# pkuyzy/TLC-GNN

Hardware: AMD Instinct MI355X
Metric: persistence-images/sec + LP-forward edges/sec, PubMed-scale, 1/2/4/8 GPU (higher is better)
Workload: dtype f64

## Files before the change

include/tlcgnn.h:

```cpp
#ifndef TLCGNN_H
#define TLCGNN_H

#include <stdint.h>

#ifdef __cplusplus
extern "C" {
#endif

#define TLC_OK                 0
#define TLC_ERR_INVALID_ARG    1
#define TLC_ERR_HIP            2
#define TLC_ERR_NO_DEVICE      3
#define TLC_ERR_UNSUPPORTED    4
#define TLC_ERR_OUT_OF_MEMORY  5

#define TLC_ST_OK              0
#define TLC_ST_MISSING_NODE    1
#define TLC_ST_DISCONNECTED    2
#define TLC_ST_ZERO_RANGE      3
#define TLC_ST_NO_TREE_EDGE    4
#define TLC_ST_TOO_LARGE       5
#define TLC_ST_NOT_CONVERGED   6
#define TLC_ST_BAD_INPUT       7

#define TLC_KEEP_ZERO_PERS   0x01u
#define TLC_INCLUDE_ROOTS    0x02u
#define TLC_NORM_EPS         0x04u
#define TLC_PI_ORD0_EXT1     0x08u
#define TLC_NO_EXT1          0x10u
#define TLC_UNREACHABLE_100  0x20u
#define TLC_DESC_MIN         0x40u
#define TLC_DESC_MAX         0x80u
#define TLC_DESC_ROOT1       0xC0u
#define TLC_DESC_MASK        0xC0u
#define TLC_NO_NORM          0x100u

typedef struct tlc_graph tlc_graph;

const char* tlc_version(void);
const char* tlc_last_error(void);
int  tlc_device_count(void);

int tlc_graph_create(int32_t n_nodes, const int32_t* h_rowptr, const int32_t* h_col, const double* h_w,
                     int device, tlc_graph** out);
int tlc_graph_destroy(tlc_graph* g);

int tlc_pd_pi_batch(tlc_graph* g, const int32_t* d_pairs, int64_t n_pairs, int hop, uint32_t flags,
                    int res, double* d_out_pi, uint8_t* d_out_status, void* stream);

int tlc_vicinity_filtration(tlc_graph* g, const int32_t* d_pairs, int64_t n_pairs, int hop, uint32_t flags,
                            const int64_t* d_node_offs, int32_t* d_out_ids, double* d_out_f,
                            int32_t* d_out_n, uint8_t* d_out_status,
                            const int64_t* d_edge_offs, int32_t* d_out_edges, int32_t* d_out_m, void* stream);

int tlc_pd_pi_batch_async(tlc_graph* g, const int32_t* d_pairs, int64_t n_pairs, int hop, uint32_t flags,
                          int res, double* d_out_pi, uint8_t* d_out_status, void* stream);
int tlc_pd_pi_batch_join(tlc_graph* g, void* stream);

int tlc_pd_pi_batch_stats(tlc_graph* g, int64_t* h_out, void* stream);

int tlc_pd_pi_batch_set_timing(tlc_graph* g, int enable);
int tlc_pd_pi_batch_timings(tlc_graph* g, double* h_ms, void* stream);
int tlc_pd_pi_batch_timing_history(tlc_graph* g, int slot, double* h_ms, int32_t cap, int32_t* n_out, void* stream);
int tlc_pd_pi_batch_sizes(tlc_graph* g, int32_t* h_n, int32_t* h_m2, int64_t cap, void* stream);
int tlc_pd_pi_algorithmic_bytes(int32_t n_nodes, const int32_t* h_rowptr, const int32_t* h_col, const int32_t* h_pairs,
                                int64_t n_pairs, int hop, int res, double* h_out_bytes);

int tlc_debug_set_option(tlc_graph* g, const char* name, int value);
int tlc_debug_dc_stats(tlc_graph* g, long long* h_out, void* stream);
int tlc_debug_chunk_counters(tlc_graph* g, long long* h_out, int32_t n, void* stream);
int tlc_debug_tier_counts(tlc_graph* g, long long* h_out, void* stream);
int tlc_debug_phase_profile(tlc_graph* g, int enable, unsigned long long* h_out, int64_t cap_u64, int32_t* n_rows);
int tlc_debug_pair_times(tlc_graph* g, unsigned long long* h_out, int64_t n_pairs);

int tlc_pd_from_filtration(int32_t n_graphs, const int64_t* d_node_offs, const int64_t* d_edge_offs,
                           const int32_t* d_edges, const double* d_f, uint32_t flags,
                           double* d_pd_up, double* d_pd_down, double* d_pd_one, double* d_ext0,
                           int32_t* d_counts, int32_t* d_edge_rank, void* stream);

int tlc_pi_raster(int32_t n_dgms, const int64_t* d_offs, const double* d_pts, int res, double* d_out,
                  void* stream);
int tlc_pi_raster_wgrad(int32_t n_dgms, int64_t n_pts, const int64_t* d_offs, const double* d_pts, int res,
                        const double* d_grad_img, double* d_grad_pts, void* stream);


int tlc_gcn_norm_csr(int32_t n_nodes, int64_t n_edges, const int64_t* d_edge_index,
                     int32_t* d_rowptr, int32_t* d_col, float* d_val, int32_t* d_nnz, void* stream);

int tlc_gemm_f32(int32_t M, int32_t N, int32_t K, const float* d_A, const float* d_B, const float* d_bias,
                 int relu, float* d_C, void* stream);

int tlc_spgemm_csr_dense_f32(int32_t M, int32_t K, int32_t N, const int32_t* d_rowptr, const int32_t* d_col, const float* d_val,
                             const float* d_B, const float* d_bias, int relu, float* d_C, void* stream);

int tlc_spmm_csr_f32(int32_t n_rows, const int32_t* d_rowptr, const int32_t* d_col, const float* d_val,
                     const float* d_X, int32_t k, const float* d_bias, int relu, float* d_Y, void* stream);

int tlc_renorm_rows_f32(int32_t n_rows, int32_t k, float* d_emb, void* stream);

int tlc_gcn2_encode_f32(int32_t n_nodes, const int32_t* d_rowptr, const int32_t* d_col, const float* d_val,
                        const float* d_x, int32_t f_in, const float* d_w1, const float* d_b1, int32_t hidden,
                        const float* d_w2, const float* d_b2, int32_t out_dim, int flags, float* d_ws, float* d_emb, void* stream);

int tlc_gcn2_encode_csr_f32(int32_t n_nodes, const int32_t* d_rowptr, const int32_t* d_col, const float* d_val,
                            const int32_t* d_xs_rowptr, const int32_t* d_xs_col, const float* d_xs_val, int32_t f_in,
                            const float* d_w1, const float* d_b1, int32_t hidden, const float* d_w2, const float* d_b2,
                            int32_t out_dim, int flags, float* d_ws, float* d_emb, void* stream);

int tlc_lp_decode_fused(int64_t n_pairs, const int32_t* d_pairs, const float* d_emb, int32_t emb_dim,
                        const double* d_pi, int32_t pi_dim, const float* d_W1, const float* d_b1,
                        const float* d_W2, const float* d_b2, float* d_prob, void* stream);
int tlc_lp_decode_fused_f32(int64_t n_pairs, const int32_t* d_pairs, const float* d_emb, int32_t emb_dim,
                            const float* d_pi, int32_t pi_dim, const float* d_W1, const float* d_b1,
                            const float* d_W2, const float* d_b2, float* d_prob, void* stream);


int tlc_gcn_norm_csr_t(int32_t n_nodes, int64_t n_edges, const int64_t* d_edge_index, const int32_t* d_rowptr,
                       int32_t* d_rowptr_t, int32_t* d_col_t, float* d_val_t, int32_t* d_nnz, void* stream);

int tlc_gemm_tn_f32(int32_t M, int32_t N, int64_t K, const float* d_A, const float* d_B, float* d_C, float* d_work, void* stream);

int tlc_lp_decode_bwd_f32(int64_t n_pairs, const int32_t* d_pairs, const float* d_emb_pre, const float* d_emb, int32_t n_nodes,
                          int32_t emb_dim, const float* d_pi, int32_t pi_dim, const float* d_W1, const float* d_b1,
                          const float* d_W2, const float* d_b2, const float* d_gprob, const int32_t* d_node_ptr,
                          const int32_t* d_node_slots, float* d_gemb, float* d_gw, float* d_work, void* stream);


int64_t tlc_nc_group_work_ints(int32_t n_nodes, int64_t n_edges);

int tlc_nc_group(int32_t n_nodes, int64_t n_edges, const int64_t* d_edge_index, int32_t* d_groups, int32_t* d_work, int32_t* d_bad,
                 void* stream);

int tlc_nc_linear_f32(int32_t M, int32_t N, int32_t K, const float* d_x, const float* d_w, const float* d_b, float* d_y, void* stream);

int tlc_nc_linear_bwd_f32(int32_t M, int32_t N, int32_t K, const float* d_x, const float* d_w, const float* d_gy, float* d_gx,
                          float* d_gw, float* d_gb, float* d_work, void* stream);

int64_t tlc_nc_curv_work_bytes(int32_t n_nodes, int64_t n_edges, int32_t C, int32_t D);

int tlc_nc_curv_fwd_f32(int32_t n_nodes, int64_t n_edges, int32_t C, int32_t D, const int32_t* d_groups, const float* d_xl,
                        const float* d_wmul, const float* d_w1, const float* d_prelu, const float* d_w2, const float* d_b2, float* d_alpha,
                        float* d_out, void* stream);

int tlc_nc_curv_bwd_f32(int32_t n_nodes, int64_t n_edges, int32_t C, int32_t D, const int32_t* d_groups, const float* d_xl,
                        const float* d_wmul, const float* d_w1, const float* d_prelu, const float* d_w2, const float* d_alpha,
                        const float* d_gout, float* d_gxl, float* d_gw1, float* d_gprelu, float* d_gw2, float* d_gb2, void* d_work,
                        int64_t work_bytes, void* stream);

#define TLC_SCORE_F32          0
#define TLC_SCORE_F64          1
#define TLC_LABEL_U8           0
#define TLC_LABEL_I64          1
#define TLC_LABEL_F32          2
#define TLC_RANK_FORCE_RADIX   0x1u
// ... 101 lines not shown
```

tlc-gnn_amd/_lib.py:

```python
import ctypes as C
import os
import subprocess

HERE = os.path.dirname(os.path.abspath(__file__))
LIB_PATH = os.path.join(HERE, "libtlcgnn_hip.so")
CSRC = os.path.join(HERE, "csrc")

OK = 0
ERRORS = {1: "TLC_ERR_INVALID_ARG", 2: "TLC_ERR_HIP", 3: "TLC_ERR_NO_DEVICE", 4: "TLC_ERR_UNSUPPORTED",
          5: "TLC_ERR_OUT_OF_MEMORY"}

ST_OK, ST_MISSING_NODE, ST_DISCONNECTED, ST_ZERO_RANGE, ST_NO_TREE_EDGE, ST_TOO_LARGE = range(6)
ST_NOT_CONVERGED, ST_BAD_INPUT = 6, 7
HKS_NMAX, HKS_LDS_NMAX, HKS_TMAX, HKS_NORMALISE = 256, 96, 8, 0x1
KEEP_ZERO_PERS, INCLUDE_ROOTS, NORM_EPS, PI_ORD0_EXT1, NO_EXT1, UNREACHABLE_100 = 0x1, 0x2, 0x4, 0x8, 0x10, 0x20
DESC_MIN, DESC_MAX, DESC_ROOT1, NO_NORM = 0x40, 0x80, 0xC0, 0x100
DESCRIPTOR_FLAG = {"sum": 0, "min": DESC_MIN, "max": DESC_MAX}

SYMBOLS = [
    "tlc_version", "tlc_last_error", "tlc_device_count", "tlc_graph_create", "tlc_graph_destroy",
    "tlc_pd_pi_batch", "tlc_pd_pi_batch_async", "tlc_pd_pi_batch_join", "tlc_vicinity_filtration", "tlc_pd_pi_batch_stats", "tlc_pd_pi_batch_set_timing",
    "tlc_pd_pi_batch_timings", "tlc_pd_pi_batch_timing_history", "tlc_pd_pi_batch_sizes", "tlc_pd_pi_algorithmic_bytes", "tlc_pd_from_filtration",
    "tlc_pi_raster", "tlc_pi_raster_wgrad", "tlc_gcn_norm_csr", "tlc_gcn_norm_csr_t", "tlc_gemm_f32", "tlc_gemm_tn_f32", "tlc_lp_decode_bwd_f32", "tlc_binary_rank_metrics", "tlc_binary_rank_metrics_work_bytes",
    "tlc_nc_group_work_ints", "tlc_nc_group", "tlc_nc_linear_f32", "tlc_nc_linear_bwd_f32", "tlc_nc_curv_work_bytes", "tlc_nc_curv_fwd_f32",
    "tlc_nc_curv_bwd_f32", "tlc_spgemm_csr_dense_f32", "tlc_spmm_csr_f32", "tlc_renorm_rows_f32", "tlc_gcn2_encode_f32", "tlc_gcn2_encode_csr_f32",
    "tlc_lp_decode_fused", "tlc_lp_decode_fused_f32", "tlc_gat_layer_fwd", "tlc_gat_layer_tiled_fwd", "tlc_gat_tile_cut", "tlc_csr_by_target", "tlc_pdgnn_forward", "tlc_pdgnn_forward_work_bytes", "tlc_scatter_f32", "tlc_edge_head_fwd",
    "tlc_complement_rows", "tlc_complement_pairs", "tlc_select_rows", "tlc_pack_vicinities", "tlc_stack_batch", "tlc_ollivier_ricci_sinkhorn",
    "tlc_near_pairs", "tlc_w2_partial_matching", "tlc_w2_inference_matching", "tlc_gat_layer_bwd", "tlc_edge_head_bwd", "tlc_pack_offsets", "tlc_vicinity_sizes", "tlc_debug_dc_stats", "tlc_debug_tier_counts", "tlc_debug_chunk_counters", "tlc_debug_phase_profile", "tlc_debug_set_option", "tlc_debug_pair_times",
    "tlc_hks_batch", "tlc_hks_batch_work_bytes",
]


class TlcError(RuntimeError):
    pass


def build(verbose=False, force=False):
    if force:
        subprocess.run(["make", "-C", CSRC, "clean"], stdout=subprocess.PIPE, stderr=subprocess.STDOUT, text=True)
    cmd = ["make", "-C", CSRC, "-j", str(min(8, os.cpu_count() or 1))]
    res = subprocess.run(cmd, stdout=subprocess.PIPE, stderr=subprocess.STDOUT, text=True)
    if verbose or res.returncode != 0:
        print(res.stdout)
    if res.returncode != 0:
        raise TlcError("building libtlcgnn_hip.so failed")
    return LIB_PATH


_lib = None


def lib():
    global _lib
    if _lib is None:
        if not os.path.exists(LIB_PATH):
            raise TlcError("libtlcgnn_hip.so is missing: run `python -c 'import __graft_entry__ as g; g.build()'` "
                           "(there is no CPU fallback for the product path)")
        try:
            import torch
        except ImportError:
            pass
        L = C.CDLL(LIB_PATH)
        L.tlc_version.restype = C.c_char_p
        L.tlc_last_error.restype = C.c_char_p
        L.tlc_graph_create.argtypes = [C.c_int32, C.c_void_p, C.c_void_p, C.c_void_p, C.c_int, C.POINTER(C.c_void_p)]
        L.tlc_graph_destroy.argtypes = [C.c_void_p]
        L.tlc_pd_pi_batch.argtypes = [C.c_void_p, C.c_void_p, C.c_int64, C.c_int, C.c_uint32, C.c_int, C.c_void_p,
                                      C.c_void_p, C.c_void_p]
        L.tlc_pd_pi_batch_async.argtypes = L.tlc_pd_pi_batch.argtypes
        L.tlc_pd_pi_batch_join.argtypes = [C.c_void_p, C.c_void_p]
        L.tlc_vicinity_filtration.argtypes = [C.c_void_p, C.c_void_p, C.c_int64, C.c_int, C.c_uint32, C.c_void_p,
                                              C.c_void_p, C.c_void_p, C.c_void_p, C.c_void_p, C.c_void_p, C.c_void_p,
                                              C.c_void_p, C.c_void_p]
        L.tlc_pd_pi_batch_stats.argtypes = [C.c_void_p, C.c_void_p, C.c_void_p]
        L.tlc_pd_pi_batch_set_timing.argtypes = [C.c_void_p, C.c_int]
        L.tlc_pd_pi_batch_timings.argtypes = [C.c_void_p, C.c_void_p, C.c_void_p]
        L.tlc_pd_pi_batch_timing_history.argtypes = [C.c_void_p, C.c_int, C.c_void_p, C.c_int32, C.c_void_p, C.c_void_p]
        L.tlc_pd_pi_batch_sizes.argtypes = [C.c_void_p, C.c_void_p, C.c_void_p, C.c_int64, C.c_void_p]
        L.tlc_pd_pi_algorithmic_bytes.argtypes = [C.c_int32, C.c_void_p, C.c_void_p, C.c_void_p, C.c_int64, C.c_int, C.c_int, C.c_void_p]
        L.tlc_pd_from_filtration.argtypes = [C.c_int32] + [C.c_void_p] * 4 + [C.c_uint32] + [C.c_void_p] * 7
        L.tlc_pi_raster.argtypes = [C.c_int32, C.c_void_p, C.c_void_p, C.c_int, C.c_void_p, C.c_void_p]
        L.tlc_pi_raster_wgrad.argtypes = [C.c_int32, C.c_int64, C.c_void_p, C.c_void_p, C.c_int, C.c_void_p, C.c_void_p, C.c_void_p]
        if hasattr(L, "tlc_gcn_norm_csr"):
            L.tlc_gcn_norm_csr.argtypes = [C.c_int32, C.c_int64] + [C.c_void_p] * 6
            L.tlc_gemm_f32.argtypes = [C.c_int32, C.c_int32, C.c_int32, C.c_void_p, C.c_void_p, C.c_void_p, C.c_int,
                                       C.c_void_p, C.c_void_p]
            L.tlc_spgemm_csr_dense_f32.argtypes = [C.c_int32, C.c_int32, C.c_int32] + [C.c_void_p] * 5 + [C.c_int, C.c_void_p, C.c_void_p]
            L.tlc_spmm_csr_f32.argtypes = [C.c_int32] + [C.c_void_p] * 4 + [C.c_int32, C.c_void_p, C.c_int, C.c_void_p,
                                                                            C.c_void_p]
            L.tlc_renorm_rows_f32.argtypes = [C.c_int32, C.c_int32, C.c_void_p, C.c_void_p]
            L.tlc_gcn2_encode_f32.argtypes = ([C.c_int32] + [C.c_void_p] * 4 + [C.c_int32, C.c_void_p, C.c_void_p, C.c_int32, C.c_void_p,
                                              C.c_void_p, C.c_int32, C.c_int, C.c_void_p, C.c_void_p, C.c_void_p])
            L.tlc_gcn2_encode_csr_f32.argtypes = ([C.c_int32] + [C.c_void_p] * 6 + [C.c_int32, C.c_void_p, C.c_void_p, C.c_int32, C.c_void_p,
                                                  C.c_void_p, C.c_int32, C.c_int, C.c_void_p, C.c_void_p, C.c_void_p])
            L.tlc_lp_decode_fused.argtypes = [C.c_int64, C.c_void_p, C.c_void_p, C.c_int32, C.c_void_p, C.c_int32,
                                              C.c_void_p, C.c_void_p, C.c_void_p, C.c_void_p, C.c_void_p, C.c_void_p]
            L.tlc_lp_decode_fused_f32.argtypes = L.tlc_lp_decode_fused.argtypes
        if hasattr(L, "tlc_gemm_tn_f32"):
            L.tlc_gcn_norm_csr_t.argtypes = [C.c_int32, C.c_int64] + [C.c_void_p] * 7
            L.tlc_gemm_tn_f32.argtypes = [C.c_int32, C.c_int32, C.c_int64] + [C.c_void_p] * 5
            L.tlc_lp_decode_bwd_f32.argtypes = ([C.c_int64, C.c_void_p, C.c_void_p, C.c_void_p, C.c_int32, C.c_int32, C.c_void_p, C.c_int32]
                                                + [C.c_void_p] * 10)
        if hasattr(L, "tlc_binary_rank_metrics"):
            L.tlc_binary_rank_metrics_work_bytes.argtypes = [C.c_void_p, C.c_int32, C.c_int, C.c_uint32]
            L.tlc_binary_rank_metrics_work_bytes.restype = C.c_int64
            L.tlc_binary_rank_metrics.argtypes = ([C.c_void_p, C.c_int, C.c_void_p, C.c_int, C.c_void_p, C.c_int32, C.c_uint32]
                                                  + [C.c_void_p] * 6 + [C.c_int64, C.c_void_p])
        if hasattr(L, "tlc_nc_group"):
            L.tlc_nc_group_work_ints.argtypes = [C.c_int32, C.c_int64]
            L.tlc_nc_group_work_ints.restype = C.c_int64
            L.tlc_nc_group.argtypes = [C.c_int32, C.c_int64] + [C.c_void_p] * 5
            L.tlc_nc_linear_f32.argtypes = [C.c_int32] * 3 + [C.c_void_p] * 5
            L.tlc_nc_linear_bwd_f32.argtypes = [C.c_int32] * 3 + [C.c_void_p] * 8
            L.tlc_nc_curv_work_bytes.argtypes = [C.c_int32, C.c_int64, C.c_int32, C.c_int32]
            L.tlc_nc_curv_work_bytes.restype = C.c_int64
            L.tlc_nc_curv_fwd_f32.argtypes = [C.c_int32, C.c_int64, C.c_int32, C.c_int32] + [C.c_void_p] * 10
            L.tlc_nc_curv_bwd_f32.argtypes = [C.c_int32, C.c_int64, C.c_int32, C.c_int32] + [C.c_void_p] * 14 + [C.c_int64, C.c_void_p]
        if hasattr(L, "tlc_gat_layer_fwd"):
            L.tlc_gat_layer_fwd.argtypes = [C.c_int32, C.c_void_p, C.c_void_p, C.c_void_p, C.c_int32, C.c_int32,
                                            C.c_void_p, C.c_void_p, C.c_void_p, C.c_void_p, C.c_float, C.c_void_p,
                                            C.c_void_p, C.c_void_p]
            L.tlc_csr_by_target.argtypes = [C.c_int32, C.c_int64] + [C.c_void_p] * 6
            L.tlc_pdgnn_forward_work_bytes.argtypes = [C.c_int32, C.c_int64, C.c_int32]
            L.tlc_pdgnn_forward_work_bytes.restype = C.c_int64
            L.tlc_pdgnn_forward.argtypes = [C.c_int32, C.c_int64, C.c_void_p, C.c_void_p, C.c_int32, C.c_void_p, C.c_int64, C.c_void_p, C.c_int32,
                                            C.c_void_p, C.c_void_p, C.c_void_p, C.c_int32, C.c_void_p, C.c_int64, C.c_void_p, C.c_void_p, C.c_void_p]
            L.tlc_gat_tile_cut.argtypes = [C.c_int32, C.c_void_p, C.c_void_p, C.c_int32, C.c_void_p, C.c_void_p, C.POINTER(C.c_int32), C.c_void_p]
            L.tlc_gat_layer_tiled_fwd.argtypes = [C.c_int32, C.c_void_p, C.c_void_p, C.c_int32, C.c_void_p, C.c_void_p, C.c_int32, C.c_int32,
                                                  C.c_void_p, C.c_void_p, C.c_void_p, C.c_void_p, C.c_float, C.c_void_p,
                                                  C.c_void_p, C.c_void_p]
            L.tlc_scatter_f32.argtypes = [C.c_int64, C.c_void_p, C.c_void_p, C.c_int32, C.c_int, C.c_int32, C.c_void_p,
                                          C.c_void_p, C.c_void_p]
            L.tlc_edge_head_fwd.argtypes = [C.c_int64, C.c_void_p, C.c_void_p, C.c_void_p, C.c_int32, C.c_void_p,
                                            C.c_void_p, C.c_int32, C.c_float, C.c_void_p, C.c_void_p, C.c_void_p,
                                            C.c_int32, C.c_void_p, C.c_void_p]
        L.tlc_complement_rows.argtypes = [C.c_int32, C.c_void_p, C.c_void_p, C.c_void_p, C.c_void_p]
        L.tlc_complement_pairs.argtypes = [C.c_int32, C.c_void_p, C.c_void_p, C.c_void_p, C.c_void_p, C.c_int64, C.c_int64,
                                           C.c_void_p, C.c_void_p]
        L.tlc_select_rows.argtypes = [C.c_int64, C.c_int32, C.c_void_p, C.c_void_p, C.c_int64, C.c_int64, C.c_uint32, C.c_void_p,
                                      C.c_void_p, C.c_void_p, C.c_void_p, C.c_void_p, C.c_void_p]
        L.tlc_pack_vicinities.argtypes = [C.c_int64] + [C.c_void_p] * 14
        L.tlc_pack_offsets.argtypes = [C.c_int64] + [C.c_void_p] * 6
        L.tlc_stack_batch.argtypes = [C.c_int64] + [C.c_void_p] * 4 + [C.c_int64, C.c_int64] + [C.c_void_p] * 3
        L.tlc_vicinity_sizes.argtypes = [C.c_void_p, C.c_void_p, C.c_int64, C.c_int, C.c_uint32, C.c_void_p, C.c_void_p, C.c_void_p]
        L.tlc_ollivier_ricci_sinkhorn.argtypes = [C.c_int32, C.c_void_p, C.c_void_p, C.c_int64, C.c_void_p, C.c_double, C.c_double,
                                                  C.c_int32, C.c_double, C.c_void_p, C.c_void_p, C.c_void_p, C.c_int64, C.c_int32,
                                                  C.c_int64, C.c_void_p]
        L.tlc_near_pairs.argtypes = [C.c_int32, C.c_void_p, C.c_void_p, C.c_void_p, C.c_int, C.c_int64, C.c_void_p, C.c_void_p,
                                     C.c_void_p, C.c_void_p]
        L.tlc_w2_partial_matching.argtypes = [C.c_int32, C.c_void_p, C.c_void_p, C.c_void_p, C.c_void_p, C.c_int, C.c_int32] + [C.c_void_p] * 7
        L.tlc_w2_inference_matching.argtypes = [C.c_int32, C.c_void_p, C.c_void_p, C.c_void_p, C.c_void_p, C.c_int, C.c_int32] + [C.c_void_p] * 9
        L.tlc_gat_layer_bwd.argtypes = [C.c_int32, C.c_void_p, C.c_void_p, C.c_void_p, C.c_int32, C.c_int32, C.c_void_p, C.c_void_p,
                                        C.c_void_p, C.c_float] + [C.c_void_p] * 9
        L.tlc_edge_head_bwd.argtypes = [C.c_int64, C.c_void_p, C.c_void_p, C.c_void_p, C.c_int32, C.c_void_p, C.c_void_p, C.c_int32,
                                        C.c_float] + [C.c_void_p] * 9
        L.tlc_hks_batch_work_bytes.argtypes = [C.c_int64, C.c_int64, C.c_int64, C.c_int32, C.POINTER(C.c_int64)]
        L.tlc_hks_batch.argtypes = ([C.c_void_p] * 3 + [C.c_int64] * 3 + [C.POINTER(C.c_double), C.c_int32, C.c_uint32, C.c_void_p, C.c_void_p,
                                    C.c_void_p, C.c_int64, C.c_void_p])
        L.tlc_debug_set_option.argtypes = [C.c_void_p, C.c_char_p, C.c_int]
        L.tlc_debug_dc_stats.argtypes = [C.c_void_p, C.c_void_p, C.c_void_p]
        L.tlc_debug_tier_counts.argtypes = [C.c_void_p, C.c_void_p, C.c_void_p]
        L.tlc_debug_chunk_counters.argtypes = [C.c_void_p, C.c_void_p, C.c_int32, C.c_void_p]
        L.tlc_debug_phase_profile.argtypes = [C.c_void_p, C.c_int, C.c_void_p, C.c_int64, C.c_void_p]
        _lib = L
    return _lib


def check(rc, what=""):
    if rc != OK:
        msg = lib().tlc_last_error().decode("utf-8", "replace")
        raise TlcError("%s: %s (%s)" % (what or "libtlcgnn_hip", ERRORS.get(rc, rc), msg))


def require_gpu():
    import torch
    if not torch.cuda.is_available():
        raise TlcError("no MI355X/HIP device visible: the TLC-GNN hot path has no CPU fallback")
    return torch


def stream_ptr(device=None):
    import torch
    return C.c_void_p(torch.cuda.current_stream(device).cuda_stream)


def on_device_of(fn):
    import functools

    @functools.wraps(fn)
    def wrapped(*args, **kwargs):
        import torch
        for a in list(args) + list(kwargs.values()):
            if isinstance(a, torch.Tensor) and a.is_cuda:
                if a.device.index != torch.cuda.current_device():
                    with torch.cuda.device(a.device):
                        return fn(*args, **kwargs)
                break
        return fn(*args, **kwargs)
    return wrapped


def ptr(t):
    if t is None:
        return None
    assert t.is_contiguous()
    return C.c_void_p(t.data_ptr())
```

tlc-gnn_amd/csrc/api.hip:

```cpp
#include <stdarg.h>
#include <stdlib.h>

#include <algorithm>
#include <new>
#include <vector>

#include "tlc_common.h"
#include <atomic>
#include <chrono>
#include "tlc_kernels.h"

static thread_local char g_err[512] = "";
void tlc_set_error(const char* fmt, ...) {
    va_list ap;
    va_start(ap, fmt);
    vsnprintf(g_err, sizeof(g_err), fmt, ap);
    va_end(ap);
}
extern "C" const char* tlc_last_error(void) { return g_err; }
extern "C" const char* tlc_version(void) { return "tlcgnn-hip 0.1.0 (gfx950)"; }
extern "C" int tlc_device_count(void) {
    int n = 0;
    if (hipGetDeviceCount(&n) != hipSuccess) return 0;
    return n;
}

#define TLC_CHUNK_PAIRS (1 << 20)
#define TLC_N_SIDE 8
#define TLC_EARLY_CAND 512
#define TLC_EARLY_SLOTS 256
#define TLC_EARLY_WG 256
#ifndef TLC_EARLY_MIN_PAIRS
#define TLC_EARLY_MIN_PAIRS 4096
#endif
#define TLC_TIMING_RING 64
#define TLC_X_REGION 4096

#define TLC_CTL_INTS (64 + TLC_SCAN_MAX_BLOCKS + 8 + 8 * 64)
struct HostSync {
    long long total_entries;
    int tier_count[TLC_N_TIERS];
    int pad[2];
    unsigned long long stats[2];
    volatile long long pub_total;
    volatile int pub_tier[TLC_N_TIERS];
    volatile int pub_tiny[TLC_TINY_BINS];
    volatile int pub_dcm;
    volatile int pub_early;
    volatile int pub_overflow;
    volatile unsigned pub_seq;
};

#define TLC_POISON 7.25

#define TLC_N_WS 4

struct ChunkCtx {
    TlcVicParams vp;
    TlcPdParams pp;
    hipStream_t s;
    int n_pairs, hop, pi_enabled;
    bool bump, use_x, early, spec, count_only, tiny_bins, pipelined;
    bool mh_front;
    bool plain, fsplit;
    int xfgrid;
    long long bump_base;
    int xgrid, vgrid, tmask;
    unsigned seq;
    size_t spec_base[TLC_N_TIERS];
    int spec_cap[TLC_N_TIERS];
    bool used[TLC_N_SIDE];
    hipEvent_t* ev_t;
    unsigned char* ev_used;
    std::chrono::steady_clock::time_point ht0;
    double ht_front;
    unsigned long long call_seq;
};

struct Workspace {
    size_t cap_pairs;
    int *hdr_n, *hdr_m2, *hdr_lu, *hdr_lv, *tier_list;
    int* dc_lists;
    int* tiny_bins;
    int* big_lists;
    hipEvent_t ev_cls;
    int prev_dcm;
    long long* edge_off;
    int* d_ctl;
    long long* d_block_sums;
    long long* d_totals;
    unsigned long long* d_stats;
    HostSync* h_sync;
    HostSync* h_sync_dev;
    unsigned pub_seq;
    size_t cap_entries;
    unsigned* A_dir;
    double* A_lw;
    size_t cap_small;
    unsigned* S_dir;
    double* S_lw;
    int vic_hop_cap;
    int* vic_scratch;
    long long vic_stride;
    int huge_slots;
    unsigned char* huge_scratch;
    size_t huge_stride;
    int* d_cand_list;
    int* d_early_list;
    unsigned* E_dir;
    double* E_lw;
    unsigned char* handoff;
    size_t cap_handoff;
    unsigned char* handoff_large;
    size_t cap_handoff_large;
    hipStream_t main;
    hipStream_t side[TLC_N_SIDE];
    hipEvent_t ev_in, ev_done;
    hipEvent_t ev_fork, ev_join[TLC_N_SIDE], ev_early, ev_scan;
    int prev_tc[TLC_N_TIERS];
    size_t x_entries_hint;
    int busy;
    int in_call;
    int n_pairs;
    ChunkCtx ctx;
    int own_early;
    int back_pending;
};

struct tlc_graph {
    int device;
    int n_nodes;
    long long nnz;
    int nw;
    int *d_rowptr, *d_col;
    double* d_w;
    Workspace ws[TLC_N_WS];
    unsigned long long next_ws;
    Workspace* last_ws;
    unsigned long long call_seq;
    Workspace* pending;
    int vic_slots;
    size_t vic_lds;
    int lds_attr_set;
    int ball_hop;
    int* d_ball_ub[2];
    long long last_stats[10];
    long long last_tc[TLC_N_TIERS];
    long long acc_tie, acc_entries;
    unsigned long long* d_phase;
    unsigned long long* d_pair_t;
    size_t cap_pair_t;
    int timing;
    hipEvent_t ev_ring[TLC_TIMING_RING][16];
    unsigned char ev_ring_used[TLC_TIMING_RING][8];
    int ev_ring_ready;
    unsigned long long ring_pos;
    hipEvent_t* ev_t;
    unsigned char* ev_used;
    int last_n_pairs;
    int ball_list_hop;
    int* d_bptr;
    int* d_bcol;
    unsigned* d_bbits;
    int* d_be_ptr;
    unsigned* d_be_pos;
    double* d_be_w;
    long long be_entries;
    long long ball_entries;
    TlcNodeRec* d_nrec;
    double* d_hh_w;
    int hh_k;
    int hh_diag;
    size_t x_lds64, x_lds512, x_lds64f, x_lds64fb;
    int opt_extract, opt_heavy, opt_tiny;
    int opt_fast_split;
    int opt_dc_inplace;
    int opt_ball_edges;
    int opt_ball_bits;
    int opt_dc_force_fail;
    int opt_plain_kernels;
    int count_only;
    int opt_n_ws;
    int opt_spec_cap;
    int opt_timing_every;
    unsigned timing_seq;
    int opt_tier_mask;
    int opt_x_region, opt_x_bump_min;
    int opt_mh_front_pos;
    int opt_main_beside_early;
    int opt_poison;
    long long last_n_hi;
    long long cnt_n_hi, cnt_pipelined, cnt_early, cnt_beyond_spec, cnt_poisoned, cnt_poison_bytes;
    long long cnt_deferred;
    long long max_busy;
    long long poison_region[3];
};

static int finish_pending(tlc_graph* g);
static int quiesce(tlc_graph* g) {
    { const int rp = finish_pending(g); if (rp != TLC_OK) return rp; }
    for (int k = 0; k < TLC_N_WS; ++k)
        if (g->ws[k].busy) { TLC_HIP_CHECK(hipEventSynchronize(g->ws[k].ev_done)); g->ws[k].busy = 0; }
    return TLC_OK;
}

static int ensure_pairs(tlc_graph* g, Workspace* ws, size_t n) {
    if (n <= ws->cap_pairs) return TLC_OK;
    hipFree(ws->hdr_n); hipFree(ws->hdr_m2); hipFree(ws->hdr_lu); hipFree(ws->hdr_lv); hipFree(ws->tier_list); hipFree(ws->edge_off);
    hipFree(ws->dc_lists); hipFree(ws->big_lists); hipFree(ws->tiny_bins);
    ws->hdr_n = ws->hdr_m2 = ws->hdr_lu = ws->hdr_lv = ws->tier_list = ws->dc_lists = ws->big_lists = ws->tiny_bins = nullptr;
    ws->edge_off = nullptr;
    ws->cap_pairs = 0;
    TLC_HIP_CHECK(hipMalloc(&ws->hdr_n, n * sizeof(int)));
    TLC_HIP_CHECK(hipMalloc(&ws->hdr_m2, n * sizeof(int)));
    TLC_HIP_CHECK(hipMalloc(&ws->hdr_lu, n * sizeof(int)));
    TLC_HIP_CHECK(hipMalloc(&ws->hdr_lv, n * sizeof(int)));
    TLC_HIP_CHECK(hipMalloc(&ws->tier_list, n * TLC_N_TIERS * sizeof(int)));
    TLC_HIP_CHECK(hipMalloc(&ws->edge_off, (n + 1) * sizeof(long long)));
    TLC_HIP_CHECK(hipMalloc(&ws->dc_lists, 3 * (n + TLC_EARLY_SLOTS) * sizeof(int)));
    TLC_HIP_CHECK(hipMalloc(&ws->big_lists, 4 * n * sizeof(int)));
    TLC_HIP_CHECK(hipMalloc(&ws->tiny_bins, (size_t)TLC_TINY_BINS * n * sizeof(int)));
    ws->cap_pairs = n;
    return TLC_OK;
}

static int ensure_arena(tlc_graph* g, Workspace* ws, size_t entries, size_t keep = 0, hipStream_t s = nullptr) {
    if (entries <= ws->cap_entries) return TLC_OK;
    size_t want = std::max(entries + entries / 4, (size_t)1 << 16);
    unsigned* old_dir = ws->A_dir;
    double* old_lw = ws->A_lw;
    ws->A_dir = nullptr; ws->A_lw = nullptr; ws->cap_entries = 0;
    if (keep == 0) { hipFree(old_dir); hipFree(old_lw); old_dir = nullptr; old_lw = nullptr; }
    TLC_HIP_CHECK(hipMalloc(&ws->A_dir, want * sizeof(unsigned)));
    TLC_HIP_CHECK(hipMalloc(&ws->A_lw, want * sizeof(double)));
    if (keep > 0) {
        TLC_HIP_CHECK(hipMemcpyAsync(ws->A_dir, old_dir, keep * sizeof(unsigned), hipMemcpyDeviceToDevice, s));
        TLC_HIP_CHECK(hipMemcpyAsync(ws->A_lw, old_lw, keep * sizeof(double), hipMemcpyDeviceToDevice, s));
        TLC_HIP_CHECK(hipDeviceSynchronize());
        hipFree(old_dir); hipFree(old_lw);
    }
    ws->cap_entries = want;
    return TLC_OK;
}


static int ensure_handoff(tlc_graph* g, Workspace* ws, size_t bytes) {
    if (bytes <= ws->cap_handoff) return TLC_OK;
    const size_t want = std::max(bytes + bytes / 4, (size_t)1 << 20);
    hipFree(ws->handoff);
    ws->handoff = nullptr; ws->cap_handoff = 0;
    TLC_HIP_CHECK(hipMalloc(&ws->handoff, want));
    ws->cap_handoff = want;
    return TLC_OK;
}

static int ensure_handoff_large(tlc_graph* g, Workspace* ws, size_t slots) {
    if (slots * tlc_handoff_slot_bytes(TLC_TIER_LARGE) <= ws->cap_handoff_large) return TLC_OK;
    const size_t bytes = (slots + slots / 4) * tlc_handoff_slot_bytes(TLC_TIER_LARGE);
    hipFree(ws->handoff_large);
    ws->handoff_large = nullptr; ws->cap_handoff_large = 0;
    TLC_HIP_CHECK(hipMalloc(&ws->handoff_large, bytes));
    ws->cap_handoff_large = bytes;
    return TLC_OK;
}

static int ensure_small(tlc_graph* g, Workspace* ws, size_t n_pairs) {
    if (n_pairs <= ws->cap_small) return TLC_OK;
    hipFree(ws->S_dir); hipFree(ws->S_lw);
    ws->S_dir = nullptr; ws->S_lw = nullptr; ws->cap_small = 0;
    TLC_HIP_CHECK(hipMalloc(&ws->S_dir, n_pairs * (2 * TLC_S_MMAX) * sizeof(unsigned)));
    TLC_HIP_CHECK(hipMalloc(&ws->S_lw, n_pairs * (2 * TLC_S_MMAX) * sizeof(double)));
    ws->cap_small = n_pairs;
// ... 141 lines not shown
    TLC_HIP_CHECK(hipMemcpyAsync(g->d_bptr, sz.data(), ((size_t)n + 1) * sizeof(int), hipMemcpyHostToDevice, s));
    if ((rc = tlc_launch_ball_list(true, n, g->nw, g->d_rowptr, g->d_col, hop, nullptr, g->d_bptr, g->d_bcol, grid, s)) != TLC_OK) return rc;
    TLC_HIP_CHECK(hipStreamSynchronize(s));
    g->ball_list_hop = hop; g->ball_entries = tot;
    {
        int* d_es = nullptr;
        int* d_bp = nullptr;
        unsigned* d_pos = nullptr;
        double* d_bw = nullptr;
        std::vector<int> es((size_t)n + 1, 0);
        bool ok = hipMalloc(&d_es, (size_t)n * sizeof(int)) == hipSuccess;
        ok = ok && tlc_launch_ball_edges(false, n, g->nw, g->d_rowptr, g->d_col, g->d_w, g->d_bptr, g->d_bcol, d_es, nullptr, nullptr, nullptr, grid, s) == TLC_OK;
        ok = ok && hipMemcpyAsync(es.data(), d_es, (size_t)n * sizeof(int), hipMemcpyDeviceToHost, s) == hipSuccess;
        ok = ok && hipStreamSynchronize(s) == hipSuccess;
        long long et = 0;
        if (ok) for (int x = 0; x < n; ++x) { const int c = es[x]; es[x] = (int)et; et += c; if (et > 0x7fffffffll) { ok = false; break; } }
        if (ok) {
            es[n] = (int)et;
            size_t fb = 0, tb = 0;
            ok = hipMemGetInfo(&fb, &tb) == hipSuccess && (size_t)et * 12 <= fb / 8;
        }
        ok = ok && hipMalloc(&d_bp, ((size_t)n + 1) * sizeof(int)) == hipSuccess;
        ok = ok && hipMalloc(&d_pos, ((size_t)et + 64) * sizeof(unsigned)) == hipSuccess;
        ok = ok && hipMalloc(&d_bw, ((size_t)et + 64) * sizeof(double)) == hipSuccess;
        ok = ok && hipMemcpyAsync(d_bp, es.data(), ((size_t)n + 1) * sizeof(int), hipMemcpyHostToDevice, s) == hipSuccess;
        ok = ok && tlc_launch_ball_edges(true, n, g->nw, g->d_rowptr, g->d_col, g->d_w, g->d_bptr, g->d_bcol, nullptr, d_bp, d_pos, d_bw, grid, s) == TLC_OK;
        ok = ok && hipStreamSynchronize(s) == hipSuccess;
        hipFree(d_es);
        if (ok) { g->d_be_ptr = d_bp; g->d_be_pos = d_pos; g->d_be_w = d_bw; g->be_entries = et; }
        else { hipFree(d_bp); hipFree(d_pos); hipFree(d_bw); (void)hipGetLastError(); }
    }
    if (g->d_be_ptr) {
        const size_t bytes = (size_t)n * (size_t)g->nw * sizeof(unsigned);
        size_t fb = 0, tb = 0;
        unsigned* d_bb = nullptr;
        bool ok = bytes <= ((size_t)1 << 30) && hipMemGetInfo(&fb, &tb) == hipSuccess && bytes <= fb / 8;
        ok = ok && hipMalloc(&d_bb, bytes) == hipSuccess;
        ok = ok && hipMemsetAsync(d_bb, 0, bytes, s) == hipSuccess;
        ok = ok && tlc_launch_ball_bits(n, g->nw, g->d_bptr, g->d_bcol, d_bb, s) == TLC_OK;
        ok = ok && hipStreamSynchronize(s) == hipSuccess;
        if (ok) g->d_bbits = d_bb;
        else { hipFree(d_bb); (void)hipGetLastError(); }
    }
    return TLC_OK;
}

extern "C" int tlc_graph_create(int32_t n_nodes, const int32_t* h_rowptr, const int32_t* h_col, const double* h_w,
                                int device, tlc_graph** out) {
    TLC_REQUIRE(out != nullptr, "out is null");
    *out = nullptr;
    TLC_REQUIRE(n_nodes > 0 && h_rowptr && h_col && h_w, "null graph arrays or n_nodes <= 0");
    int ndev = 0;
    if (hipGetDeviceCount(&ndev) != hipSuccess || ndev == 0) {
        tlc_set_error("no HIP device visible");
        return TLC_ERR_NO_DEVICE;
    }
    TLC_REQUIRE(device >= 0 && device < ndev, "device index out of range");
    const long long nnz = h_rowptr[n_nodes];
    TLC_REQUIRE(h_rowptr[0] == 0 && nnz >= 0, "rowptr must start at 0");
    for (int i = 0; i < n_nodes; ++i) TLC_REQUIRE(h_rowptr[i + 1] >= h_rowptr[i], "rowptr not monotone");
    for (long long j = 0; j < nnz; ++j) {
        TLC_REQUIRE(h_col[j] >= 0 && h_col[j] < n_nodes, "column index out of range");
        TLC_REQUIRE(h_w[j] > 0.0, "edge weights (kappa+1) must be > 0");
    }
    const int nw = (n_nodes + 31) / 32;
    const size_t lds = ((size_t)5 * ((nw + 3) & ~3) / 2 + 4 + 16) * 4;
    if (lds > 160 * 1024) {
        tlc_set_error("graph has %d nodes: the vicinity bitmaps (%zu B) exceed the 160 KiB LDS of a CU", n_nodes, lds);
        return TLC_ERR_UNSUPPORTED;
    }
    TLC_ON_DEVICE(device);
    tlc_graph* g = new (std::nothrow) tlc_graph();
    if (!g) return TLC_ERR_OUT_OF_MEMORY;
    memset(g, 0, sizeof(*g));
    g->device = device; g->n_nodes = n_nodes; g->nnz = nnz; g->nw = nw; g->vic_lds = lds;
    auto env_on = [](const char* name) { const char* v = getenv(name); return !(v && v[0] == '0'); };
    g->opt_extract = env_on("TLC_EXTRACT"); g->opt_heavy = env_on("TLC_HEAVY"); g->opt_tiny = env_on("TLC_TINY");
    g->opt_ball_edges = env_on("TLC_BALL_EDGES"); g->opt_dc_inplace = env_on("TLC_DC_INPLACE") ? 1 : 0;
    g->opt_fast_split = env_on("TLC_FAST_SPLIT") ? 1 : 0;
    g->opt_ball_bits = env_on("TLC_BALL_BITS") ? 1 : 0;
    g->opt_plain_kernels = env_on("TLC_PLAIN_KERNELS") ? 1 : 0;
    g->opt_n_ws = 3;
    g->opt_x_region = TLC_X_REGION; g->opt_x_bump_min = 1 << 20; g->opt_tier_mask = (1 << TLC_N_TIERS) - 1; g->opt_timing_every = 1;
    g->opt_mh_front_pos = 64; g->opt_main_beside_early = 1;
    int rc = TLC_OK;
    auto fail = [&](int code) { tlc_graph_destroy(g); return code; };
#define CK(e) do { if ((e) != hipSuccess) { tlc_set_error("%s failed: %s", #e, hipGetErrorString(hipGetLastError())); return fail(TLC_ERR_HIP); } } while (0)
    CK(hipMalloc(&g->d_rowptr, (size_t)(n_nodes + 1) * sizeof(int)));
    CK(hipMalloc(&g->d_col, ((size_t)nnz + 8) * sizeof(int)));
    CK(hipMalloc(&g->d_w, ((size_t)nnz + 8) * sizeof(double)));
    CK(hipMemset(g->d_col + nnz, 0, 8 * sizeof(int)));
    CK(hipMemset(g->d_w + nnz, 0, 8 * sizeof(double)));
    CK(hipMemcpy(g->d_rowptr, h_rowptr, (size_t)(n_nodes + 1) * sizeof(int), hipMemcpyHostToDevice));
    CK(hipMemcpy(g->d_col, h_col, (size_t)nnz * sizeof(int), hipMemcpyHostToDevice));
    CK(hipMemcpy(g->d_w, h_w, (size_t)nnz * sizeof(double), hipMemcpyHostToDevice));
    int prio_lo = 0, prio_hi = 0;
    hipDeviceGetStreamPriorityRange(&prio_lo, &prio_hi);
    const int prio_mid = (prio_lo + prio_hi) / 2;
    const bool eager_streams = getenv("TLC_LAZY_STREAMS") == nullptr;
    const int n_eager = 3;
    for (int i = 0; i < TLC_N_WS; ++i) {
        Workspace* ws = &g->ws[i];
        CK(hipMalloc(&ws->d_ctl, TLC_CTL_INTS * sizeof(int)));
        ws->d_stats = reinterpret_cast<unsigned long long*>(ws->d_ctl + 64 + TLC_SCAN_MAX_BLOCKS);
        CK(hipMalloc(&ws->d_block_sums, TLC_SCAN_MAX_BLOCKS * sizeof(long long)));
        CK(hipMalloc(&ws->d_totals, 2 * sizeof(long long)));
        CK(hipHostMalloc((void**)&ws->h_sync, sizeof(HostSync), hipHostMallocMapped | hipHostMallocCoherent));
        memset(ws->h_sync, 0, sizeof(HostSync));
        CK(hipHostGetDevicePointer((void**)&ws->h_sync_dev, ws->h_sync, 0));
        if (i == 0 || (eager_streams && i < n_eager)) CK(hipStreamCreateWithPriority(&ws->main, hipStreamNonBlocking, prio_mid));
        for (int k = 0; k < TLC_N_SIDE; ++k) {
            if (k == 4) {
                if (i == 0 || (eager_streams && i < n_eager)) { CK(hipStreamCreateWithPriority(&ws->side[k], hipStreamNonBlocking, prio_hi)); ws->own_early = 1; }
            }
            else if (i > 0) {
                ws->side[k] = g->ws[0].side[k];
                if (i == 2 && k == 7) ws->side[k] = g->ws[0].side[1];
            }
            else if (k == 2) ws->side[k] = nullptr;
            else {
                const int pr = k == 1 ? prio_hi : ((k == 6 || k == 7) ? prio_mid : prio_lo);
                CK(hipStreamCreateWithPriority(&ws->side[k], hipStreamNonBlocking, pr));
            }
            CK(hipEventCreateWithFlags(&ws->ev_join[k], hipEventDisableTiming));
        }
        if (i == 0) ws->side[2] = ws->side[6];
        CK(hipEventCreateWithFlags(&ws->ev_fork, hipEventDisableTiming));
        CK(hipEventCreateWithFlags(&ws->ev_early, hipEventDisableTiming));
        CK(hipEventCreateWithFlags(&ws->ev_scan, hipEventDisableTiming));
        CK(hipEventCreateWithFlags(&ws->ev_cls, hipEventDisableTiming));
        CK(hipEventCreateWithFlags(&ws->ev_in, hipEventDisableTiming));
        CK(hipEventCreateWithFlags(&ws->ev_done, hipEventDisableTiming));
    }
#undef CK
    hipDeviceProp_t prop;
    int cus = 256;
    if (hipGetDeviceProperties(&prop, device) == hipSuccess && prop.multiProcessorCount > 0) cus = prop.multiProcessorCount;
    int per_cu = (int)std::min<size_t>(28, (160 * 1024) / std::max<size_t>(lds + 64, 1));
    if (per_cu < 1) per_cu = 1;
    g->x_lds64 = tlc_extract_lds_bytes(nw, 64);
    g->x_lds512 = tlc_extract_lds_bytes(nw, 512);
    g->x_lds64f = tlc_extract_lds_bytes(nw, 64, true);
    g->x_lds64fb = tlc_extract_lds_bytes(0, 64, true);
    per_cu = std::max(per_cu, (int)std::min<size_t>(32, (160 * 1024) / std::max<size_t>(g->x_lds64 + 64, 1)));
    g->vic_slots = cus * per_cu;
    {
        std::vector<int> hidx;
        if ((rc = build_heavy_set(g, h_rowptr, h_col, h_w, &hidx)) != TLC_OK) return fail(rc);
        if ((rc = build_node_records(g, h_rowptr, h_col, h_w, hidx)) != TLC_OK) return fail(rc);
    }
    *out = g;
    return TLC_OK;
}

extern "C" int tlc_graph_destroy(tlc_graph* g) {
    if (!g) return TLC_OK;
    TlcDeviceScope scope(g->device);
    hipDeviceSynchronize();
    hipFree(g->d_rowptr); hipFree(g->d_col); hipFree(g->d_w);
    for (int i = 0; i < TLC_N_WS; ++i) {
        Workspace* ws = &g->ws[i];
        hipFree(ws->hdr_n); hipFree(ws->hdr_m2); hipFree(ws->hdr_lu); hipFree(ws->hdr_lv); hipFree(ws->tier_list); hipFree(ws->edge_off);
        hipFree(ws->dc_lists); hipFree(ws->big_lists); hipFree(ws->tiny_bins);
        hipFree(ws->d_ctl); hipFree(ws->d_block_sums); hipFree(ws->d_totals);
        if (ws->h_sync) hipHostFree(ws->h_sync);
        hipFree(ws->A_dir); hipFree(ws->A_lw); hipFree(ws->S_dir); hipFree(ws->S_lw); hipFree(ws->vic_scratch); hipFree(ws->huge_scratch);
        hipFree(ws->handoff); hipFree(ws->handoff_large);
        hipFree(ws->d_cand_list); hipFree(ws->d_early_list); hipFree(ws->E_dir); hipFree(ws->E_lw);
        if (ws->main) hipStreamDestroy(ws->main);
        for (int k = 0; k < TLC_N_SIDE; ++k) {
            const bool own = (k == 4 && ws->own_early) || (i == 0 && k != 2);
            if (own && ws->side[k]) hipStreamDestroy(ws->side[k]);
            if (ws->ev_join[k]) hipEventDestroy(ws->ev_join[k]);
        }
        for (hipEvent_t e : {ws->ev_fork, ws->ev_early, ws->ev_scan, ws->ev_in, ws->ev_done, ws->ev_cls}) if (e) hipEventDestroy(e);
    }
    hipFree(g->d_phase); hipFree(g->d_pair_t);
    hipFree(g->d_bptr); hipFree(g->d_bcol); hipFree(g->d_nrec); hipFree(g->d_hh_w);
    hipFree(g->d_be_ptr); hipFree(g->d_be_pos); hipFree(g->d_be_w); hipFree(g->d_bbits);
    hipFree(g->d_ball_ub[0]); hipFree(g->d_ball_ub[1]);
    if (g->ev_ring_ready)
        for (int r = 0; r < TLC_TIMING_RING; ++r)
            for (int k = 0; k < 16; ++k) if (g->ev_ring[r][k]) hipEventDestroy(g->ev_ring[r][k]);
    delete g;
    return TLC_OK;
}

__global__ void tlc_wait_started(const int* counter, int target, long long max_ticks) {
    if (threadIdx.x != 0) return;
    const long long t0 = wall_clock64();
    while (__hip_atomic_load(counter, __ATOMIC_RELAXED, __HIP_MEMORY_SCOPE_AGENT) < target && wall_clock64() - t0 < max_ticks)
        __builtin_amdgcn_s_sleep(8);
}

__global__ void tlc_wait_started_dev(const int* counter, const int* target, int cap, long long max_ticks) {
    if (threadIdx.x != 0) return;
    int tg = *target;
    tg = tg < cap ? tg : cap;
    const long long t0 = wall_clock64();
    while (__hip_atomic_load(counter, __ATOMIC_RELAXED, __HIP_MEMORY_SCOPE_AGENT) < tg && wall_clock64() - t0 < max_ticks)
        __builtin_amdgcn_s_sleep(8);
}

#define T0(k, st) do { if ((c.tmask >> (k)) & 1) { TLC_HIP_CHECK(hipEventRecord(c.ev_t[2 * (k)], st)); } } while (0)
#define T1(k, st) do { if ((c.tmask >> (k)) & 1) { TLC_HIP_CHECK(hipEventRecord(c.ev_t[2 * (k) + 1], st)); c.ev_used[k] = 1; } } while (0)
static inline void dc_lists_for(Workspace* ws, TlcPdParams& q, int k) {
    const size_t cap = ws->cap_pairs + TLC_EARLY_SLOTS;
    q.dc_count = ws->d_ctl + 26 + 2 * k;
    q.dc_list = ws->dc_lists + (size_t)k * cap;
}
static const int tslot[TLC_N_TIERS] = {3, 4, 5, 6, 7, 3, 4, 4};

static int front_prepare(tlc_graph* g, Workspace* ws, const int32_t* d_pairs, int n_pairs, int hop, uint32_t flags, int res,
                         double* d_out_pi, uint8_t* d_out_status, const int64_t* d_ids_off, int32_t* d_out_ids,
                         double* d_out_f, int32_t* d_out_n, const int64_t* d_edge_offs, int32_t* d_out_edges, int32_t* d_out_m,
                         int pi_enabled, hipStream_t s, bool pipelined) {
    int rc;
    ChunkCtx& c = ws->ctx;
    c.ht0 = std::chrono::steady_clock::now();
    c.s = s; c.n_pairs = n_pairs; c.hop = hop; c.pi_enabled = pi_enabled; c.call_seq = g->call_seq;
    if ((rc = ensure_pairs(g, ws, (size_t)n_pairs)) != TLC_OK) return rc;
    if ((rc = ensure_vic_scratch(g, ws, hop)) != TLC_OK) return rc;
    TLC_HIP_CHECK(hipMemsetAsync(ws->d_ctl, 0, TLC_CTL_INTS * sizeof(int), s));

    TlcVicParams& vp = c.vp;
    memset(&vp, 0, sizeof(vp));
    vp.n_nodes = g->n_nodes; vp.nw = g->nw; vp.rowptr = g->d_rowptr; vp.col = g->d_col; vp.w = g->d_w;
    vp.dbg = g->d_phase ? g->d_phase + 32 * TLC_TIER_HUGE : nullptr;
    if (g->d_phase) {
        if (g->cap_pair_t < (size_t)n_pairs) {
            hipFree(g->d_pair_t); g->d_pair_t = nullptr; g->cap_pair_t = 0;
            TLC_HIP_CHECK(hipMalloc(&g->d_pair_t, (size_t)n_pairs * 16 * sizeof(unsigned long long)));
            g->cap_pair_t = (size_t)n_pairs;
        }
        TLC_HIP_CHECK(hipMemsetAsync(g->d_pair_t, 0, (size_t)n_pairs * 16 * sizeof(unsigned long long), s));
        vp.dbg_pair_t = g->d_pair_t;
    }
    vp.pairs = d_pairs; vp.n_pairs = n_pairs; vp.hop = hop; vp.flags = flags; vp.res = res;
    vp.scratch = ws->vic_scratch; vp.scratch_stride = ws->vic_stride;
    vp.hdr_n = ws->hdr_n; vp.hdr_m2 = ws->hdr_m2; vp.hdr_lu = ws->hdr_lu; vp.hdr_lv = ws->hdr_lv;
    vp.out_pi = d_out_pi; vp.out_status = d_out_status; vp.out_n = d_out_n; vp.out_m = d_out_m;
    vp.edge_off = ws->edge_off; vp.A_dir = nullptr; vp.A_lw = nullptr;
    vp.ids_off = (const long long*)d_ids_off; vp.out_ids = d_out_ids;

    if (!g->lds_attr_set && g->vic_lds > 64 * 1024) {
        TLC_HIP_CHECK(hipFuncSetAttribute((const void*)tlc_vicinity_kernel<false, 64>, hipFuncAttributeMaxDynamicSharedMemorySize, (int)g->vic_lds));
        TLC_HIP_CHECK(hipFuncSetAttribute((const void*)tlc_vicinity_kernel<true, 64>, hipFuncAttributeMaxDynamicSharedMemorySize, (int)g->vic_lds));
        TLC_HIP_CHECK(hipFuncSetAttribute((const void*)tlc_vicinity_kernel<true, 512>, hipFuncAttributeMaxDynamicSharedMemorySize, (int)g->vic_lds));
        TLC_HIP_CHECK(hipFuncSetAttribute((const void*)tlc_vicinity_kernel<false, 512>, hipFuncAttributeMaxDynamicSharedMemorySize, (int)g->vic_lds));
        g->lds_attr_set = 1;
    }
    const int vgrid = std::min(n_pairs, g->vic_slots);
    const int tmask = (g->timing && (g->timing_seq++ % (unsigned)std::max(g->opt_timing_every, 1)) == 0) ? g->timing : 0;
    if (tmask) {
        if (!g->ev_ring_ready) {
            for (int r = 0; r < TLC_TIMING_RING; ++r)
                for (int k = 0; k < 16; ++k) TLC_HIP_CHECK(hipEventCreate(&g->ev_ring[r][k]));
            g->ev_ring_ready = 1;
        }
        const int set = (int)(g->ring_pos++ % TLC_TIMING_RING);
        g->ev_t = g->ev_ring[set];
        g->ev_used = g->ev_ring_used[set];
        memset(g->ev_used, 0, 8);
        c.ev_t = g->ev_t; c.ev_used = g->ev_used;
    }
    c.tmask = tmask; c.vgrid = vgrid;
    g->last_n_pairs = n_pairs;
    const bool plain = pi_enabled && !d_out_ids && !d_out_f && !d_out_edges;
    const bool bump = true;
    unsigned long long* d_bump_top = reinterpret_cast<unsigned long long*>(ws->d_ctl + 20);
    int* d_bump_overflow = ws->d_ctl + 22;
    bool use_x = g->opt_extract && g->x_lds512 <= (size_t)160 * 1024 && g->x_lds64 <= (size_t)160 * 1024 &&
                 (hop <= 2 || (size_t)g->nw * 12 + 16 <= (size_t)160 * 1024);
    if (use_x) {
        if ((rc = ensure_ball_lists(g, hop, s)) != TLC_OK) return rc;
        use_x = g->ball_list_hop == hop;
    }
    const bool early = pi_enabled && !d_out_ids && !d_out_f && !d_out_edges && (hop <= 2 || use_x) && n_pairs >= TLC_EARLY_MIN_PAIRS;
    const int xgrid = std::min(n_pairs, g->vic_slots);
    const bool fsplit = use_x && g->opt_fast_split && g->opt_ball_edges && g->d_be_ptr != nullptr && !(flags & TLC_INCLUDE_ROOTS);
    const int xfgrid = fsplit ? std::min(n_pairs, 8192) : 0;
    long long bump_base = 0;
    if (use_x) {
        const long long regions = (long long)xgrid + TLC_EARLY_WG + xfgrid;
        bump_base = regions * g->opt_x_region;
        const size_t want = (size_t)bump_base + std::max<size_t>(std::max<size_t>((size_t)n_pairs * 32, (size_t)g->opt_x_bump_min), ws->x_entries_hint + ws->x_entries_hint / 2);
        if (ws->cap_entries < want && (rc = ensure_arena(g, ws, want)) != TLC_OK) return rc;
        vp.small_dir = nullptr; vp.small_lw = nullptr;
        vp.bptr = g->d_bptr; vp.bcol = g->d_bcol;
        if (g->opt_ball_edges) { vp.be_ptr = g->d_be_ptr; vp.be_pos = g->d_be_pos; vp.be_w = g->d_be_w; }
        vp.nrec = g->d_nrec;
        if (g->hh_k > 0 && g->opt_heavy) { vp.hh_w = g->d_hh_w; vp.hh_k = g->hh_k; }
        vp.region_entries = g->opt_x_region; vp.bump_base = bump_base; vp.region_base_wg = 0;
    } else {
        if ((rc = ensure_small(g, ws, (size_t)n_pairs)) != TLC_OK) return rc;
        vp.small_dir = ws->S_dir; vp.small_lw = ws->S_lw;
    }
    if (bump) {
        if (ws->cap_entries == 0 &&
            (rc = ensure_arena(g, ws, std::min<size_t>((size_t)n_pairs * 128, (size_t)1 << 23))) != TLC_OK) return rc;
        vp.A_dir = ws->A_dir; vp.A_lw = ws->A_lw;
        vp.bump_top = d_bump_top; vp.bump_cap = (long long)ws->cap_entries; vp.bump_overflow = d_bump_overflow;
    }
    TlcPdParams& pp = c.pp;
    memset(&pp, 0, sizeof(pp));
    pp.hdr_n = ws->hdr_n; pp.hdr_m2 = ws->hdr_m2; pp.hdr_lu = ws->hdr_lu; pp.hdr_lv = ws->hdr_lv;
    pp.edge_off = ws->edge_off;
    pp.small_dir = use_x ? nullptr : ws->S_dir; pp.small_lw = use_x ? nullptr : ws->S_lw;
    pp.flags = flags; pp.res = res; pp.out_pi = d_out_pi; pp.out_status = d_out_status;
    pp.ids_off = (const long long*)d_ids_off; pp.out_f = d_out_f; pp.out_n = d_out_n; pp.pi_enabled = pi_enabled;
    pp.edges_off = (const long long*)d_edge_offs; pp.out_edges = d_out_edges; pp.out_m = d_out_m;
    pp.stats = ws->d_stats;
    pp.dc_force_fail = g->opt_dc_force_fail;
    pp.no_plain = g->opt_plain_kernels ? 0 : 1;
    c.bump = bump; c.use_x = use_x; c.early = early; c.bump_base = bump_base; c.xgrid = xgrid;
    c.plain = plain; c.fsplit = fsplit; c.xfgrid = xfgrid; c.pipelined = pipelined; c.spec = false;
    c.count_only = g->count_only != 0;
    return TLC_OK;
}

__global__ void tlc_fill_f64(double* p, long long n, double v) {
    for (long long i = (long long)blockIdx.x * blockDim.x + threadIdx.x; i < n; i += (long long)gridDim.x * blockDim.x) p[i] = v;
}

static int poison_chunk(tlc_graph* g, Workspace* ws, hipStream_t s) {
    const struct { double* p; size_t n; } reg[3] = {
        {ws->A_lw, ws->cap_entries},
        {ws->E_lw, ws->E_lw ? (size_t)TLC_EARLY_SLOTS * 2 * TLC_L_MMAX : 0},
        {ws->S_lw, ws->cap_small * (2 * TLC_S_MMAX)}};
    long long bytes = 0;
    for (int r = 0; r < 3; ++r) {
        const long long n = reg[r].p ? (long long)reg[r].n : 0;
        g->poison_region[r] = n * (long long)sizeof(double);
        if (n == 0) continue;
        const int grid = (int)std::min<long long>((n + 255) / 256, 4096);
        hipLaunchKernelGGL(tlc_fill_f64, dim3(grid), dim3(256), 0, s, reg[r].p, n, (double)TLC_POISON);
        TLC_HIP_CHECK(hipGetLastError());
        bytes += n * (long long)sizeof(double);
    }
    g->cnt_poisoned += 1;
    g->cnt_poison_bytes += bytes;
    return TLC_OK;
}

static int front_fast(tlc_graph* g, Workspace* ws) {
    int rc;
    ChunkCtx& c = ws->ctx;
    TlcVicParams& vp = c.vp;
    hipStream_t s = c.s;
    const int hop = c.hop, xgrid = c.xgrid, xfgrid = c.xfgrid;
    const bool early = c.early, use_x = c.use_x, fsplit = c.fsplit;
    if (early && (rc = ensure_early(g, ws, hop, s)) != TLC_OK) return rc;
    if (g->opt_poison && (rc = poison_chunk(g, ws, s)) != TLC_OK) return rc;
    g->cnt_pipelined += c.pipelined ? 1 : 0;
    g->cnt_early += early ? 1 : 0;
    if (early) {
        TLC_HIP_CHECK(hipEventRecord(ws->ev_fork, s));
        TLC_HIP_CHECK(hipStreamWaitEvent(ws->side[4], ws->ev_fork, 0));
    }
    vp.early_min_ball = (early && use_x) ? TLC_M_NMAX - 1 : 0;
    if (fsplit) {
        TlcVicParams fp = vp;
        fp.region_base_wg = xgrid + TLC_EARLY_WG;
        fp.scratch_base_slot = 0;
        fp.work_counter = nullptr;
        size_t flds = g->x_lds64f;
        if (g->opt_ball_bits && g->d_bbits) {
            fp.bbits = g->d_bbits; fp.bb_nw = g->nw; fp.nw = 0;
            flds = g->x_lds64fb;
        }
        if ((rc = tlc_launch_extract(64, xfgrid, flds, fp, s, true)) != TLC_OK) return rc;
        vp.fast_split = 1;
    }
    return TLC_OK;
}

static int front_early_chain(tlc_graph* g, Workspace* ws) {
    int rc;
    ChunkCtx& c = ws->ctx;
    TlcVicParams& vp = c.vp;
    TlcPdParams& pp = c.pp;
    hipStream_t s = c.s;
    const int n_pairs = c.n_pairs, hop = c.hop, xgrid = c.xgrid;
    const bool early = c.early, use_x = c.use_x;
    const int32_t* d_pairs = vp.pairs;
    int* d_cand_count = ws->d_ctl + 16;
    int* d_early_count = ws->d_ctl + 17;
    int* d_early_started = ws->d_ctl + 18;
    int* d_cand_started = ws->d_ctl + 19;
    if (early) {
        if ((rc = ensure_early(g, ws, hop, s)) != TLC_OK) return rc;
        hipStream_t es = ws->side[4];
        if (use_x) {
            if ((rc = tlc_launch_classify(n_pairs, d_pairs, g->n_nodes, g->d_bptr, TLC_M_NMAX - 1, TLC_EARLY_CAND, d_cand_count,
                                          ws->d_cand_list, ws->d_ctl + 32, ws->big_lists, es)) != TLC_OK) return rc;
            TLC_HIP_CHECK(hipEventRecord(ws->ev_cls, es));
        } else if ((rc = tlc_launch_select_heavy(n_pairs, d_pairs, g->n_nodes, g->d_ball_ub[(hop - 1) & 1], TLC_M_NMAX - 1, TLC_EARLY_CAND,
                                                 d_cand_count, ws->d_cand_list, es)) != TLC_OK) return rc;
        TlcVicParams ep = vp;
        ep.fill_mode = 1; ep.fill_list = ws->d_cand_list; ep.fill_count = TLC_EARLY_CAND; ep.work_count_dev = d_cand_count;
        ep.scratch_base_slot = g->vic_slots;
        ep.dbg = g->d_phase ? g->d_phase + 32 * TLC_N_TIERS : nullptr;
        ep.early_list = ws->d_early_list; ep.early_count = d_early_count; ep.early_cap = TLC_EARLY_SLOTS;
        ep.early_dir = ws->E_dir; ep.early_lw = ws->E_lw;
        ep.started = d_cand_started;
        if (use_x) {
            ep.region_base_wg = xgrid;
            if ((rc = tlc_launch_extract(512, TLC_EARLY_WG, g->x_lds512, ep, es)) != TLC_OK) return rc;
            vp.skip_threshold = TLC_M_NMAX - 1; vp.skip_count = d_cand_count; vp.skip_cap = TLC_EARLY_CAND;
            vp.big_count = ws->d_ctl + 32; vp.big_list = ws->big_lists;
        } else {
            ep.bump_top = nullptr;
            ep.out_pi = nullptr; ep.out_status = nullptr; ep.out_n = nullptr; ep.out_m = nullptr;
            ep.small_dir = nullptr; ep.small_lw = nullptr;
            hipLaunchKernelGGL((tlc_vicinity_kernel<false, 512>), dim3(TLC_EARLY_WG), dim3(512), g->vic_lds, es, ep);
            TLC_HIP_CHECK(hipGetLastError());
        }
        TLC_HIP_CHECK(hipEventRecord(ws->ev_early, es));
        TlcPdParams lp = pp;
        lp.tier_list = ws->d_early_list; lp.tier_count = TLC_EARLY_SLOTS; lp.tier_count_dev = d_early_count;
        lp.slot_entries = 2 * TLC_L_MMAX; lp.A_dir = ws->E_dir; lp.A_lw = ws->E_lw;
        lp.started = d_early_started;
        if (tlc_handoff_slot_bytes(TLC_TIER_LARGE) != 0) {
            if ((rc = ensure_handoff_large(g, ws, TLC_EARLY_SLOTS)) != TLC_OK) return rc;
            lp.handoff = ws->handoff_large; lp.handoff_stride = (long long)tlc_handoff_slot_bytes(TLC_TIER_LARGE);
            lp.handoff_cap = TLC_EARLY_SLOTS;
            dc_lists_for(ws, lp, 2);
            lp.dc_inplace = g->opt_dc_inplace;
        }
        lp.phase_cycles = g->d_phase ? g->d_phase + 32 * TLC_TIER_LARGE : nullptr;
        T0(5, es);
        if (((g->opt_tier_mask >> TLC_TIER_LARGE) & 1) && (rc = tlc_launch_pd_tier(TLC_TIER_LARGE, lp, es)) != TLC_OK) return rc;
        T1(5, es);
        TLC_HIP_CHECK(hipEventRecord(ws->ev_join[4], es));
    }
    return TLC_OK;
}

static int front_join_early(tlc_graph* g, Workspace* ws) {
    ChunkCtx& c = ws->ctx;
    hipStream_t s = c.s;
    const bool use_x = c.use_x;
    int* d_early_count = ws->d_ctl + 17;
    int* d_early_started = ws->d_ctl + 18;
    if (c.early) {
        if (g->opt_main_beside_early && c.pipelined && use_x) { TLC_HIP_CHECK(hipStreamWaitEvent(s, ws->ev_cls, 0)); }
        else TLC_HIP_CHECK(hipStreamWaitEvent(s, ws->ev_early, 0));
        if (!c.pipelined)
            hipLaunchKernelGGL(tlc_wait_started_dev, dim3(1), dim3(TLC_WAVE), 0, s, (const int*)d_early_started, (const int*)d_early_count,
                               192, 5000ll);
        TLC_HIP_CHECK(hipGetLastError());
    }
    return TLC_OK;
}

static int front_main_scan(tlc_graph* g, Workspace* ws) {
    int rc;
    ChunkCtx& c = ws->ctx;
    TlcVicParams& vp = c.vp;
    hipStream_t s = c.s;
    const int n_pairs = c.n_pairs, xgrid = c.xgrid, vgrid = c.vgrid;
    const bool early = c.early, use_x = c.use_x, fsplit = c.fsplit, plain = c.plain, pipelined = c.pipelined, bump = c.bump;
    const long long bump_base = c.bump_base;
    int* d_early_count = ws->d_ctl + 17;
    unsigned long long* d_bump_top = reinterpret_cast<unsigned long long*>(ws->d_ctl + 20);
    int* d_bump_overflow = ws->d_ctl + 22;
    vp.work_counter = ws->d_ctl + 64 + TLC_SCAN_MAX_BLOCKS + 8;
    vp.work_chunk = std::max(2, n_pairs / (pipelined ? 4096 : 8192));
    if (fsplit && early) vp.work_chunk = 1;
    T0(0, s);
    if (use_x) {
        if ((rc = tlc_launch_extract(64, xgrid, g->x_lds64, vp, s)) != TLC_OK) return rc;
    } else {
        hipLaunchKernelGGL((tlc_vicinity_kernel<false, 64>), dim3(vgrid), dim3(TLC_WAVE), g->vic_lds, s, vp);
    }
    T1(0, s);
    vp.work_counter = nullptr;
    vp.skip_count = nullptr; vp.big_count = nullptr;
    TLC_HIP_CHECK(hipGetLastError());
    if (early) TLC_HIP_CHECK(hipStreamWaitEvent(s, ws->ev_early, 0));

    const int nb = (n_pairs + TLC_SCAN_BLOCK - 1) / TLC_SCAN_BLOCK;
    T0(1, s);
    const unsigned seq = ++ws->pub_seq;
    TlcScanParams sp;
    memset(&sp, 0, sizeof(sp));
    sp.n_pairs = n_pairs; sp.hdr_n = ws->hdr_n; sp.hdr_m2 = ws->hdr_m2;
    sp.block_agg = ws->d_block_sums; sp.block_flag = ws->d_ctl + 64; sp.sync = ws->d_ctl + 10; sp.totals = ws->d_totals;
    sp.edge_off = ws->edge_off; sp.tier_count = ws->d_ctl; sp.tier_list = ws->tier_list; sp.small_arena = use_x ? 0 : 1;
    const bool mh_split = !pipelined;
    sp.mh_min_pos = mh_split ? TLC_MH_MIN_POS : 0x7fffffff;
    c.mh_front = !mh_split && plain && g->opt_mh_front_pos > 0;
    if (c.mh_front) { sp.mh_min_pos = g->opt_mh_front_pos; sp.mh_compact_only = 1; }
    sp.tiny_ok = (g->opt_tiny && plain && vp.flags == 0u && vp.res == 5) ? 1 : 0;
    sp.dcm_count = ws->d_ctl + 44; sp.h_dcm = const_cast<int*>(&ws->h_sync_dev->pub_dcm);
    static_assert(TLC_TINY_BINS <= 16, "the size-class counters of the TINY list live in d_ctl[48..63]");
    if (sp.tiny_ok) { sp.tiny_bin_count = ws->d_ctl + 48; sp.tiny_bin_list = ws->tiny_bins; sp.h_tiny_bins = const_cast<int*>(ws->h_sync_dev->pub_tiny); }
    sp.early_list = early ? ws->d_early_list : nullptr; sp.early_count = d_early_count; sp.early_cap = TLC_EARLY_SLOTS;
    sp.h_early = const_cast<int*>(&ws->h_sync_dev->pub_early);
    sp.bump_top = bump ? d_bump_top : nullptr; sp.bump_overflow = d_bump_overflow; sp.bump_base = bump_base;
    sp.h_overflow = const_cast<int*>(&ws->h_sync_dev->pub_overflow);
    sp.h_total = const_cast<long long*>(&ws->h_sync_dev->pub_total);
    sp.h_tier = const_cast<int*>(ws->h_sync_dev->pub_tier);
    sp.h_seq = const_cast<unsigned*>(&ws->h_sync_dev->pub_seq);
    sp.seq = seq;
    hipLaunchKernelGGL(tlc_scan_bin, dim3(nb), dim3(TLC_SCAN_BLOCK), 0, s, sp);
    T1(1, s);
    TLC_HIP_CHECK(hipGetLastError());
    c.seq = seq;
    c.tiny_bins = sp.tiny_bin_count != nullptr;
    return TLC_OK;
}

static int front_speculative(tlc_graph* g, Workspace* ws) {
    int rc;
    ChunkCtx& c = ws->ctx;
    TlcPdParams& pp = c.pp;
    hipStream_t s = c.s;
    const int n_pairs = c.n_pairs;
    const bool early = c.early, plain = c.plain, pipelined = c.pipelined;
    int* d_bump_overflow = ws->d_ctl + 22;
    bool (&used)[TLC_N_SIDE] = c.used;
    for (int k = 0; k < TLC_N_SIDE; ++k) used[k] = (k == 4) && early;
    TLC_HIP_CHECK(hipEventRecord(ws->ev_scan, s));
    const bool mh_split = !pipelined;
    const bool spec = plain && mh_split;
    size_t (&spec_base)[TLC_N_TIERS] = c.spec_base;
    int (&spec_cap)[TLC_N_TIERS] = c.spec_cap;
    for (int t = 0; t < TLC_N_TIERS; ++t) { spec_base[t] = 0; spec_cap[t] = 0; }
    if (spec) {
        spec_cap[TLC_TIER_MID] = std::min(n_pairs, std::max(4096, ws->prev_tc[TLC_TIER_MID] + ws->prev_tc[TLC_TIER_MID] / 4));
        spec_cap[TLC_TIER_MEDIUM] = std::min(n_pairs, std::max(2048, ws->prev_tc[TLC_TIER_MEDIUM] + ws->prev_tc[TLC_TIER_MEDIUM] / 4));
        spec_cap[TLC_TIER_MEDHI] = std::min(n_pairs, std::max(1024, ws->prev_tc[TLC_TIER_MEDHI] + ws->prev_tc[TLC_TIER_MEDHI] / 4));
        spec_cap[TLC_TIER_MEDWIDE] = 0;
        if (g->opt_spec_cap > 0)
            for (int t : {TLC_TIER_MID, TLC_TIER_MEDIUM, TLC_TIER_MEDHI}) spec_cap[t] = std::min(spec_cap[t], g->opt_spec_cap);
        spec_base[TLC_TIER_MEDHI] = (size_t)spec_cap[TLC_TIER_MID] * tlc_handoff_slot_bytes(TLC_TIER_MID);
        spec_base[TLC_TIER_MEDIUM] = spec_base[TLC_TIER_MEDHI] + (size_t)spec_cap[TLC_TIER_MEDHI] * tlc_handoff_slot_bytes(TLC_TIER_MEDHI);
        spec_base[TLC_TIER_MEDWIDE] = spec_base[TLC_TIER_MEDIUM] + (size_t)spec_cap[TLC_TIER_MEDIUM] * tlc_handoff_slot_bytes(TLC_TIER_MEDIUM);
        if ((rc = ensure_handoff(g, ws, spec_base[TLC_TIER_MEDWIDE] +
                                        (size_t)spec_cap[TLC_TIER_MEDWIDE] * tlc_handoff_slot_bytes(TLC_TIER_MEDWIDE))) != TLC_OK) return rc;
        pp.A_dir = ws->A_dir; pp.A_lw = ws->A_lw;
        {
            const int t = TLC_TIER_MEDHI;
            pp.tier_list = ws->tier_list + (size_t)t * n_pairs; pp.tier_count = n_pairs; pp.tier_count_dev = ws->d_ctl + t;
            pp.grid = spec_cap[t]; pp.handoff_cap = spec_cap[t]; pp.phase = 0;
            pp.handoff = ws->handoff + spec_base[t]; pp.handoff_stride = (long long)tlc_handoff_slot_bytes(t);
            pp.abort_flag = d_bump_overflow;
            pp.phase_cycles = g->d_phase ? g->d_phase + 32 * t : nullptr;
            pp.dc_count = nullptr; pp.dc_list = nullptr;
            if (ws->prev_dcm > 0) dc_lists_for(ws, pp, 0);
            T0(tslot[t], s);
            if (((g->opt_tier_mask >> t) & 1) && (rc = tlc_launch_pd_tier(t, pp, s)) != TLC_OK) return rc;
            T1(tslot[t], s);
            pp.dc_count = nullptr; pp.dc_list = nullptr;
        }
        pp.phase = 0;
        pp.grid = 0; pp.tier_count_dev = nullptr; pp.abort_flag = nullptr; pp.handoff = nullptr; pp.handoff_cap = 0;
    }
    c.spec = spec;
    return TLC_OK;
}

static int run_chunk_front(tlc_graph* g, Workspace* ws, const int32_t* d_pairs, int n_pairs, int hop, uint32_t flags, int res,
                     double* d_out_pi, uint8_t* d_out_status, const int64_t* d_ids_off, int32_t* d_out_ids,
                     double* d_out_f, int32_t* d_out_n, const int64_t* d_edge_offs, int32_t* d_out_edges, int32_t* d_out_m,
                     int pi_enabled, hipStream_t s, bool pipelined) {
    int rc;
    ChunkCtx& c = ws->ctx;
    if ((rc = front_prepare(g, ws, d_pairs, n_pairs, hop, flags, res, d_out_pi, d_out_status, d_ids_off, d_out_ids, d_out_f, d_out_n,
                            d_edge_offs, d_out_edges, d_out_m, pi_enabled, s, pipelined)) != TLC_OK) return rc;
    if ((rc = front_fast(g, ws)) != TLC_OK) return rc;
    if ((rc = front_early_chain(g, ws)) != TLC_OK) return rc;
    if ((rc = front_join_early(g, ws)) != TLC_OK) return rc;
    if ((rc = front_main_scan(g, ws)) != TLC_OK) return rc;
    if ((rc = front_speculative(g, ws)) != TLC_OK) return rc;
    c.ht_front = (double)std::chrono::duration_cast<std::chrono::nanoseconds>(std::chrono::steady_clock::now() - c.ht0).count() * 1e-3;
    ws->back_pending = 1;
    return TLC_OK;
}

static inline bool sizes_published(const Workspace* ws) { return ws->h_sync->pub_seq == ws->ctx.seq; }

static void account_chunk(tlc_graph* g, const int (&tc)[TLC_N_TIERS], int n_early) {
    for (int t = 0; t <= TLC_TIER_HUGE; ++t) g->last_stats[t] += tc[t];
    for (int t = 0; t < TLC_N_TIERS; ++t) g->last_tc[t] += tc[t];
    g->last_stats[TLC_TIER_MEDIUM] += tc[TLC_TIER_MEDWIDE];
    g->last_stats[TLC_TIER_MEDIUM] += tc[TLC_TIER_MEDHI];
    g->last_stats[9] += tc[TLC_TIER_MEDHI];
    g->last_stats[TLC_TIER_SMALL] += tc[TLC_TIER_TINY];
    g->last_stats[8] += tc[TLC_TIER_TINY];
    g->last_stats[TLC_TIER_LARGE] += n_early;
    g->last_stats[7] += tc[TLC_TIER_MID];
    g->last_stats[6] += 1;
}

static int wait_for_sizes(const Workspace* ws, hipStream_t s, unsigned seq) {
    const auto t0 = std::chrono::steady_clock::now();
    bool seen = false;
    for (unsigned it = 1; !(seen = (ws->h_sync->pub_seq == seq)); ++it) {
        if ((it & 0x3ff) != 0) continue;
        const auto el = std::chrono::steady_clock::now() - t0;
        if (el < std::chrono::microseconds(300)) continue;
        const hipError_t q = hipStreamQuery(s);
        if (q == hipSuccess) { seen = (ws->h_sync->pub_seq == seq); break; }
        if (q != hipErrorNotReady) { tlc_set_error(hipGetErrorString(q)); return TLC_ERR_HIP; }
        if (el > std::chrono::seconds(20)) break;
    }
    TLC_REQUIRE(seen, "size publication did not arrive");
    return TLC_OK;
}

static int run_chunk_back(tlc_graph* g, Workspace* ws) {
    int rc;
    ChunkCtx& c = ws->ctx;
    static const bool host_trace = getenv("TLC_HOST_TRACE") != nullptr;
    const auto ht0 = c.ht0;
    auto ht_us = [&]() { return (double)std::chrono::duration_cast<std::chrono::nanoseconds>(std::chrono::steady_clock::now() - ht0).count() * 1e-3; };
    const double ht_front = c.ht_front;
    double ht_seen = 0;
    TlcVicParams& vp = c.vp;
    TlcPdParams& pp = c.pp;
    hipStream_t s = c.s;
    const int n_pairs = c.n_pairs, hop = c.hop, pi_enabled = c.pi_enabled, xgrid = c.xgrid, vgrid = c.vgrid;
    const bool bump = c.bump, use_x = c.use_x, early = c.early, spec = c.spec;
    const long long bump_base = c.bump_base;
    const unsigned seq = c.seq;
    size_t (&spec_base)[TLC_N_TIERS] = c.spec_base;
    int (&spec_cap)[TLC_N_TIERS] = c.spec_cap;
    bool (&used)[TLC_N_SIDE] = c.used;
    ws->back_pending = 0;
    if ((rc = wait_for_sizes(ws, s, seq)) != TLC_OK) return rc;
    ht_seen = ht_us();
    std::atomic_thread_fence(std::memory_order_acquire);
    const long long total = ws->h_sync->pub_total;
    int tc[TLC_N_TIERS];
    for (int t = 0; t < TLC_N_TIERS; ++t) tc[t] = ws->h_sync->pub_tier[t];
    int n_hi = 0;
    if (c.mh_front) { n_hi = tc[TLC_TIER_MEDHI]; tc[TLC_TIER_MEDIUM] += n_hi; tc[TLC_TIER_MEDHI] = 0; }
    g->cnt_n_hi += n_hi;
    const bool bumped = bump && ws->h_sync->pub_overflow == 0;
    if (use_x) ws->x_entries_hint = std::max(ws->x_entries_hint, (size_t)std::max<long long>(total - (bumped ? bump_base : 0), 0));
    if ((rc = ensure_arena(g, ws, (size_t)total, bumped ? (size_t)std::min<long long>(total, (long long)ws->cap_entries) : 0, s)) != TLC_OK) return rc;
    if (tc[TLC_TIER_HUGE] > 0 && (rc = ensure_huge(g, ws)) != TLC_OK) return rc;

    const int n_early = early ? ws->h_sync->pub_early : 0;
    const int n_dcm = ws->h_sync->pub_dcm;
    ws->prev_dcm = n_dcm;
    int todo = tc[0] + tc[1] + tc[2] + tc[3] + tc[4] + tc[5] + tc[6] + tc[7];
    if (c.count_only) {
        if ((rc = tlc_launch_copy_sizes(n_pairs, ws->hdr_n, ws->hdr_m2, pp.out_n, pp.out_m, s)) != TLC_OK) return rc;
        todo = 0;
    }
    const bool spec_done = spec && bumped;
    if (spec_done)
        for (int t : {TLC_TIER_MID, TLC_TIER_MEDIUM, TLC_TIER_MEDHI}) g->cnt_beyond_spec += std::max(tc[t] - spec_cap[t], 0);
    ws->prev_tc[TLC_TIER_MID] = tc[TLC_TIER_MID]; ws->prev_tc[TLC_TIER_MEDIUM] = tc[TLC_TIER_MEDIUM]; ws->prev_tc[TLC_TIER_MEDHI] = tc[TLC_TIER_MEDHI];
    ws->prev_tc[TLC_TIER_MEDWIDE] = tc[TLC_TIER_MEDWIDE];
    if (todo > 0) {
        vp.A_dir = ws->A_dir; vp.A_lw = ws->A_lw;
        pp.A_dir = ws->A_dir; pp.A_lw = ws->A_lw;
        pp.huge_scratch = ws->huge_scratch; pp.huge_stride = (long long)ws->huge_stride;
        pp.huge_nmax = std::min(g->n_nodes, TLC_MAX_SUBGRAPH_NODES); pp.huge_mmax = (int)std::min<long long>(g->nnz / 2 + 1, TLC_MAX_SUBGRAPH_EDGES); pp.huge_slots = ws->huge_slots;
        pp.started = (int*)(ws->d_stats + 2);
        bool filled_all = false;
        if (use_x && !bumped && tc[0] + tc[1] + tc[4] + tc[5] + tc[6] + tc[7] > 0) {
            vp.fill_mode = (tc[TLC_TIER_LARGE] + tc[TLC_TIER_HUGE] > 0 || n_early > 0) ? 2 : 0; vp.fill_list = nullptr; vp.fill_count = 0;
            vp.x_fill = 1; vp.bump_top = nullptr; vp.work_count_dev = nullptr;
            if ((rc = tlc_launch_extract(64, xgrid, g->x_lds64, vp, s)) != TLC_OK) return rc;
            filled_all = true;
        }
        size_t hand_base[TLC_N_TIERS] = {0, 0, 0, 0, 0, 0, 0, 0};
        if (pi_enabled && !spec_done) {
            size_t hand_total = 0;
            for (int t = 0; t < TLC_N_TIERS; ++t) {
                if (t == TLC_TIER_LARGE) continue;
                hand_base[t] = hand_total;
                hand_total += (size_t)tc[t] * tlc_handoff_slot_bytes(t);
            }
            if ((rc = ensure_handoff(g, ws, hand_total)) != TLC_OK) return rc;
        } else if (pi_enabled) {
            hand_base[TLC_TIER_MID] = 0;
            hand_base[TLC_TIER_MEDIUM] = spec_base[TLC_TIER_MEDIUM];
            hand_base[TLC_TIER_MEDWIDE] = spec_base[TLC_TIER_MEDWIDE];
        }
        if (spec_done && tc[TLC_TIER_MEDHI] > spec_cap[TLC_TIER_MEDHI]) {
            const int t = TLC_TIER_MEDHI;
            pp.tier_list = ws->tier_list + (size_t)t * n_pairs; pp.tier_count = tc[t]; pp.tier_count_dev = nullptr;
            pp.wi_base = spec_cap[t]; pp.grid = tc[t] - spec_cap[t]; pp.handoff_cap = spec_cap[t]; pp.phase = 1;
            pp.handoff = ws->handoff + spec_base[t]; pp.handoff_stride = (long long)tlc_handoff_slot_bytes(t);
            pp.abort_flag = nullptr; pp.dc_count = nullptr; pp.dc_list = nullptr;
            pp.tier_list_hi = nullptr; pp.n_hi = 0;
            pp.phase_cycles = g->d_phase ? g->d_phase + 32 * t : nullptr;
            if (((g->opt_tier_mask >> t) & 1) && (rc = tlc_launch_pd_tier(t, pp, s)) != TLC_OK) return rc;
            pp.wi_base = 0; pp.grid = 0; pp.phase = 0; pp.handoff = nullptr; pp.handoff_cap = 0;
        }
        struct PendingSwap { bool on; int k; bool timed; TlcPdParams pp; };
        PendingSwap pend[TLC_N_TIERS];
        for (int t = 0; t < TLC_N_TIERS; ++t) pend[t].on = false;
        auto finish_pending_swaps = [&]() -> int {
            for (int t = 0; t < TLC_N_TIERS; ++t) {
                if (!pend[t].on) continue;
                pend[t].on = false;
                const int k = pend[t].k;
                hipStream_t ss = ws->side[k];
                int r = ((g->opt_tier_mask >> t) & 1) ? tlc_launch_pd_tier(t, pend[t].pp, ss) : TLC_OK;
                if (r != TLC_OK) return r;
                if (pend[t].timed) T1(tslot[t], ss);
                TLC_HIP_CHECK(hipEventRecord(ws->ev_join[k], ss));
            }
            return TLC_OK;
        };
        auto launch_side = [&](int k, int t, bool behind_s = true) -> int {
            if (bumped && !behind_s) {
                TLC_HIP_CHECK(hipStreamWaitEvent(ws->side[k], ws->ev_scan, 0));
            } else {
                TLC_HIP_CHECK(hipEventRecord(ws->ev_fork, s));
                TLC_HIP_CHECK(hipStreamWaitEvent(ws->side[k], ws->ev_fork, 0));
            }
            pp.tier_list = ws->tier_list + (size_t)t * n_pairs; pp.tier_count = tc[t];
            pp.tier_list_hi = nullptr; pp.n_hi = 0;
            if (t == TLC_TIER_MEDIUM && n_hi > 0) { pp.tier_list_hi = ws->tier_list + (size_t)TLC_TIER_MEDHI * n_pairs; pp.n_hi = n_hi; }
            const size_t hs = pi_enabled ? tlc_handoff_slot_bytes(t) : 0;
            pp.handoff = hs ? ws->handoff + hand_base[t] : nullptr;
            pp.handoff_stride = (long long)hs;
            pp.handoff_cap = (spec_done && (t == TLC_TIER_MID || t == TLC_TIER_MEDIUM || t == TLC_TIER_MEDWIDE)) ? std::min(tc[t], spec_cap[t]) : tc[t];
            pp.dc_count = nullptr; pp.dc_list = nullptr; pp.dc_inplace = 0;
            if (t == TLC_TIER_LARGE) { dc_lists_for(ws, pp, 1); pp.dc_inplace = g->opt_dc_inplace; }
            if ((t == TLC_TIER_MEDHI || t == TLC_TIER_MEDWIDE) && n_dcm > 0) dc_lists_for(ws, pp, 0);
            if (hs && t == TLC_TIER_LARGE) {
                int r2 = ensure_handoff_large(g, ws, (size_t)TLC_EARLY_SLOTS + (size_t)tc[t]);
                if (r2 != TLC_OK) return r2;
                pp.handoff = ws->handoff_large + (size_t)TLC_EARLY_SLOTS * hs;
            }
            pp.grid = 0; pp.phase = 0; pp.tier_count_dev = nullptr; pp.abort_flag = nullptr;
            pp.phase_cycles = g->d_phase ? g->d_phase + 32 * t : nullptr;
            const bool timed = !(early && t == TLC_TIER_LARGE) && !(t == TLC_TIER_MEDIUM && spec) && t != TLC_TIER_MEDWIDE;
            if (timed) T0(tslot[t], ws->side[k]);
            const bool two = hs && !(pp.flags & TLC_NO_EXT1) &&
                             (t == TLC_TIER_MEDIUM || t == TLC_TIER_MID || t == TLC_TIER_MEDHI || t == TLC_TIER_MEDWIDE);
            if (two) pp.phase = 1;
            int r = ((g->opt_tier_mask >> t) & 1) ? tlc_launch_pd_tier(t, pp, ws->side[k]) : TLC_OK;
            pp.phase = 0;
            if (r != TLC_OK) return r;
            used[k] = true;
            if (two) {
                pend[t].on = true; pend[t].k = k; pend[t].timed = timed; pend[t].pp = pp; pend[t].pp.phase = 2;
                return TLC_OK;
            }
            if (timed) T1(tslot[t], ws->side[k]);
            TLC_HIP_CHECK(hipEventRecord(ws->ev_join[k], ws->side[k]));
            return TLC_OK;
        };
        const int heavy = tc[TLC_TIER_LARGE] + tc[TLC_TIER_HUGE];
        if (pi_enabled && tc[TLC_TIER_LARGE] > 0 && (rc = ensure_handoff_large(g, ws, (size_t)TLC_EARLY_SLOTS + (size_t)tc[TLC_TIER_LARGE])) != TLC_OK) return rc;
        T0(2, s);
        for (int t = TLC_TIER_HUGE; t >= TLC_TIER_LARGE; --t) {
            if (tc[t] <= 0) continue;
            vp.fill_mode = 1; vp.fill_list = ws->tier_list + (size_t)t * n_pairs; vp.fill_count = tc[t];
            if (use_x) {
                vp.x_fill = 1; vp.bump_top = nullptr; vp.work_count_dev = nullptr;
                if ((rc = tlc_launch_extract(512, std::min(tc[t], TLC_EARLY_WG), g->x_lds512, vp, s)) != TLC_OK) return rc;
            } else if (hop <= 2)
                hipLaunchKernelGGL((tlc_vicinity_kernel<true, 512>), dim3(std::min(tc[t], g->vic_slots)), dim3(512), g->vic_lds, s, vp);
            else
                hipLaunchKernelGGL((tlc_vicinity_kernel<true, 64>), dim3(std::min(tc[t], g->vic_slots)), dim3(TLC_WAVE), g->vic_lds, s, vp);
            TLC_HIP_CHECK(hipGetLastError());
            if ((rc = launch_side(1, t)) != TLC_OK) return rc;
        }
        if (tc[TLC_TIER_LARGE] > 0) {
            hipLaunchKernelGGL(tlc_wait_started, dim3(1), dim3(TLC_WAVE), 0, s, (const int*)pp.started,
                               std::min(tc[TLC_TIER_LARGE], 192), 5000ll);
            TLC_HIP_CHECK(hipGetLastError());
        }
        auto launch_tiny_small = [&]() -> int {
            if (tc[TLC_TIER_TINY] > 0) {
                if (bumped) { TLC_HIP_CHECK(hipStreamWaitEvent(ws->side[5], ws->ev_scan, 0)); }
                else { TLC_HIP_CHECK(hipEventRecord(ws->ev_fork, s)); TLC_HIP_CHECK(hipStreamWaitEvent(ws->side[5], ws->ev_fork, 0)); }
                pp.tier_list = ws->tier_list + (size_t)TLC_TIER_TINY * n_pairs; pp.tier_count = tc[TLC_TIER_TINY];
                pp.tiny_bin_list = nullptr;
                if (c.tiny_bins) {
                    pp.tiny_bin_list = ws->tiny_bins; pp.tiny_bin_stride = n_pairs;
                    for (int b = 0; b < TLC_TINY_BINS; ++b) pp.tiny_bin_cnt[b] = ws->h_sync->pub_tiny[b];
                }
                pp.handoff = nullptr; pp.handoff_stride = 0; pp.handoff_cap = 0; pp.grid = 0; pp.phase = 0;
                pp.tier_count_dev = nullptr; pp.abort_flag = nullptr;
                pp.dc_count = nullptr; pp.dc_list = nullptr;
                pp.tier_list_hi = nullptr; pp.n_hi = 0;
                pp.phase_cycles = g->d_phase ? g->d_phase + 32 * TLC_TIER_TINY : nullptr;
                int r = ((g->opt_tier_mask >> TLC_TIER_TINY) & 1) ? tlc_launch_pd_tiny(pp, ws->side[5]) : TLC_OK;
                if (r != TLC_OK) return r;
                TLC_HIP_CHECK(hipEventRecord(ws->ev_join[5], ws->side[5]));
                used[5] = true;
            }
            if (tc[TLC_TIER_SMALL] > 0) return launch_side(0, TLC_TIER_SMALL, false);
            return TLC_OK;
        };
        auto launch_medium_mid = [&]() -> int {
            int r;
            if (tc[TLC_TIER_MEDIUM] + tc[TLC_TIER_MEDHI] + tc[TLC_TIER_MEDWIDE] + tc[TLC_TIER_MID] > 0) {
                if (!bumped && !filled_all) {
                    vp.fill_mode = (heavy > 0 || n_early > 0) ? 2 : 0; vp.fill_list = nullptr; vp.fill_count = 0;
                    hipLaunchKernelGGL((tlc_vicinity_kernel<true, 64>), dim3(vgrid), dim3(TLC_WAVE), g->vic_lds, s, vp);
                    TLC_HIP_CHECK(hipGetLastError());
                }
                T1(2, s);
                if (tc[TLC_TIER_MEDWIDE] > 0 && (r = launch_side(7, TLC_TIER_MEDWIDE, !bumped)) != TLC_OK) return r;
                if (!spec_done && tc[TLC_TIER_MEDHI] > 0 && (r = launch_side(2, TLC_TIER_MEDHI)) != TLC_OK) return r;
                if (tc[TLC_TIER_MEDIUM] > 0 && (r = launch_side(6, TLC_TIER_MEDIUM, !bumped)) != TLC_OK) return r;
                if (tc[TLC_TIER_MID] > 0 && (r = launch_side(3, TLC_TIER_MID, !bumped)) != TLC_OK) return r;
            } else {
                T1(2, s);
            }
            return TLC_OK;
        };
        if (!c.pipelined && c.tiny_bins) {
            if ((rc = launch_medium_mid()) != TLC_OK) return rc;
            if ((rc = launch_tiny_small()) != TLC_OK) return rc;
        } else {
            if ((rc = launch_tiny_small()) != TLC_OK) return rc;
            if ((rc = launch_medium_mid()) != TLC_OK) return rc;
        }
        if ((rc = finish_pending_swaps()) != TLC_OK) return rc;
    }
    for (int k = 0; k < TLC_N_SIDE; ++k)
        if (used[k]) TLC_HIP_CHECK(hipStreamWaitEvent(s, ws->ev_join[k], 0));
#undef T0
#undef T1
    if (c.call_seq == g->call_seq) { account_chunk(g, tc, n_early); g->last_n_hi += n_hi; }
    if (host_trace) {
        static std::chrono::steady_clock::time_point last_end;
        const double gap = (double)std::chrono::duration_cast<std::chrono::nanoseconds>(ht0 - last_end).count() * 1e-3;
        fprintf(stderr, "[tlc host] ws%d since-last-chunk %.0f us | front submitted %.0f | sizes seen %.0f | tiers submitted %.0f\n",
                (int)(ws - g->ws), gap, ht_front, ht_seen, ht_us());
        last_end = std::chrono::steady_clock::now();
    }
    return TLC_OK;
}

static int chunk_entries(Workspace* ws, long long* out) {
    std::vector<int> n((size_t)ws->n_pairs), m2((size_t)ws->n_pairs);
    *out = 0;
    if (ws->n_pairs <= 0) return TLC_OK;
    TLC_HIP_CHECK(hipMemcpy(n.data(), ws->hdr_n, n.size() * sizeof(int), hipMemcpyDeviceToHost));
    TLC_HIP_CHECK(hipMemcpy(m2.data(), ws->hdr_m2, m2.size() * sizeof(int), hipMemcpyDeviceToHost));
    long long e = 0;
    for (size_t k = 0; k < n.size(); ++k) if (n[k] > 0) e += m2[k];
    *out = e;
    return TLC_OK;
}

static int finish_pending(tlc_graph* g) {
    Workspace* ws = g->pending;
    if (!ws) return TLC_OK;
    g->pending = nullptr;
    int rc = run_chunk_back(g, ws);
    if (rc != TLC_OK) return rc;
    TLC_HIP_CHECK(hipEventRecord(ws->ev_done, ws->ctx.s));
    return TLC_OK;
}
// ... 211 lines not shown
    } while (0);
    if (rc == TLC_ERR_HIP) tlc_set_error("tlc_pd_from_filtration: HIP runtime call failed: %s", hipGetErrorString(hipGetLastError()));
    hipStreamSynchronize(s);
    hipFree(d_tier);
    if (huge) hipFree(huge);
    return rc;
}

extern "C" int tlc_pi_raster(int32_t n_dgms, const int64_t* d_offs, const double* d_pts, int res, double* d_out,
                             void* stream) {
    TLC_REQUIRE(n_dgms >= 0, "n_dgms < 0");
    TLC_REQUIRE(res >= 1 && res <= 8, "res must be in 1..8");
    if (n_dgms == 0) return TLC_OK;
    TLC_REQUIRE(d_offs && d_out, "null pointer");
    return tlc_launch_pi_raster(n_dgms, (const long long*)d_offs, d_pts, res, d_out, stream);
}

extern "C" int tlc_vicinity_sizes(tlc_graph* g, const int32_t* d_pairs, int64_t n_pairs, int hop, uint32_t flags, int32_t* d_n, int32_t* d_m,
                                  void* stream) {
    TLC_REQUIRE(g != nullptr, "graph handle is null");
    TLC_REQUIRE(n_pairs == 0 || (d_n && d_m), "null output");
    g->count_only = 1;
    const int rc = run_batch(g, d_pairs, n_pairs, hop, flags, 5, nullptr, nullptr, nullptr, nullptr, nullptr, d_n, nullptr, nullptr, d_m,
                             0, stream, true);
    g->count_only = 0;
    return rc;
}

extern "C" int tlc_pi_raster_wgrad(int32_t n_dgms, int64_t n_pts, const int64_t* d_offs, const double* d_pts, int res,
                                   const double* d_grad_img, double* d_grad_pts, void* stream) {
    TLC_REQUIRE(n_dgms >= 0 && n_pts >= 0, "negative count");
    TLC_REQUIRE(res >= 1 && res <= 8, "res must be in 1..8");
    if (n_pts == 0) return TLC_OK;
    TLC_REQUIRE(n_dgms > 0 && d_offs && d_pts && d_grad_img && d_grad_pts, "null pointer");
    return tlc_launch_pi_raster_wgrad(n_dgms, (long long)n_pts, (const long long*)d_offs, d_pts, res, d_grad_img, d_grad_pts, stream);
}

extern "C" int tlc_debug_phase_profile(tlc_graph* g, int enable, unsigned long long* h_out, int64_t cap_u64, int32_t* n_rows) {
    TLC_REQUIRE(g != nullptr, "null graph");
    TLC_REQUIRE(h_out == nullptr || cap_u64 >= 0, "cap_u64 < 0");
    TLC_ON_DEVICE(g->device);
    { int rc_p = finish_pending(g); if (rc_p != TLC_OK) return rc_p; }
    const size_t rows = (size_t)TLC_N_TIERS + 2;
    if (n_rows) *n_rows = (int32_t)rows;
    TLC_HIP_CHECK(hipDeviceSynchronize());
    if (h_out && g->d_phase) {
        const size_t k = std::min<size_t>(rows * 32, (size_t)cap_u64);
        TLC_HIP_CHECK(hipMemcpy(h_out, g->d_phase, k * sizeof(unsigned long long), hipMemcpyDeviceToHost));
    }
    if (enable && !g->d_phase) TLC_HIP_CHECK(hipMalloc(&g->d_phase, rows * 32 * sizeof(unsigned long long)));
    if (g->d_phase) TLC_HIP_CHECK(hipMemset(g->d_phase, 0, rows * 32 * sizeof(unsigned long long)));
    if (!enable && g->d_phase) { hipFree(g->d_phase); g->d_phase = nullptr; }
    return TLC_OK;
}

extern "C" int tlc_debug_pair_times(tlc_graph* g, unsigned long long* h_out, int64_t n_pairs) {
    TLC_REQUIRE(g && h_out, "null argument");
    TLC_ON_DEVICE(g->device);
    { int rc_p = finish_pending(g); if (rc_p != TLC_OK) return rc_p; }
    TLC_HIP_CHECK(hipDeviceSynchronize());
    const size_t k = std::min<size_t>((size_t)std::max<int64_t>(n_pairs, 0), g->d_pair_t ? g->cap_pair_t : 0);
    if (k) TLC_HIP_CHECK(hipMemcpy(h_out, g->d_pair_t, k * 16 * sizeof(unsigned long long), hipMemcpyDeviceToHost));
    return TLC_OK;
}

extern "C" int tlc_debug_set_option(tlc_graph* g, const char* name, int value) {
    TLC_REQUIRE(g && name, "null argument");
    if (!strcmp(name, "extract")) g->opt_extract = value != 0;
    else if (!strcmp(name, "heavy")) g->opt_heavy = value != 0;
    else if (!strcmp(name, "tiny")) g->opt_tiny = value != 0;
    else if (!strcmp(name, "ball_edges")) g->opt_ball_edges = value != 0;
    else if (!strcmp(name, "dc_inplace")) g->opt_dc_inplace = value != 0;
    else if (!strcmp(name, "fast_split")) g->opt_fast_split = value != 0;
    else if (!strcmp(name, "ball_bits")) g->opt_ball_bits = value != 0;
    else if (!strcmp(name, "plain_kernels")) g->opt_plain_kernels = value != 0;
    else if (!strcmp(name, "tier_mask")) g->opt_tier_mask = value;
    else if (!strcmp(name, "spec_cap")) g->opt_spec_cap = std::max(value, 0);
    else if (!strcmp(name, "n_ws")) { int rc_p = finish_pending(g); if (rc_p != TLC_OK) return rc_p; g->opt_n_ws = std::min(std::max(value, 2), TLC_N_WS); }
    else if (!strcmp(name, "timing_every")) { g->opt_timing_every = std::max(value, 1); g->timing_seq = 0; }
    else if (!strcmp(name, "dc_force_fail")) g->opt_dc_force_fail = value != 0;
    else if (!strcmp(name, "x_arena")) { g->opt_x_region = value > 0 ? value : TLC_X_REGION; g->opt_x_bump_min = value > 0 ? value : (1 << 20); }
    else if (!strcmp(name, "mh_front_pos")) g->opt_mh_front_pos = std::max(value, 0);
    else if (!strcmp(name, "main_beside_early")) g->opt_main_beside_early = value != 0;
    else if (!strcmp(name, "poison")) g->opt_poison = value != 0;
    else { tlc_set_error("tlc_debug_set_option: unknown option '%s'", name); return TLC_ERR_INVALID_ARG; }
    return TLC_OK;
}

extern "C" int tlc_debug_dc_stats(tlc_graph* g, long long* h_out, void* stream) {
    TLC_REQUIRE(g && h_out, "null argument");
    TLC_ON_DEVICE(g->device);
    { int rc_p = finish_pending(g); if (rc_p != TLC_OK) return rc_p; }
    TLC_HIP_CHECK(hipStreamSynchronize((hipStream_t)stream));
    unsigned long long v[4] = {0, 0, 0, 0};
    if (g->last_ws) {
        if (g->last_ws->busy) { TLC_HIP_CHECK(hipEventSynchronize(g->last_ws->ev_done)); g->last_ws->busy = 0; }
        TLC_HIP_CHECK(hipMemcpy(v, g->last_ws->d_stats, sizeof(v), hipMemcpyDeviceToHost));
    }
    h_out[0] = (long long)v[1];
    h_out[1] = (long long)v[3];
    return TLC_OK;
}

extern "C" int tlc_debug_chunk_counters(tlc_graph* g, long long* h_out, int32_t n, void* stream) {
    TLC_REQUIRE(g && h_out && n >= 0, "null argument");
    TLC_ON_DEVICE(g->device);
    { int rc_p = finish_pending(g); if (rc_p != TLC_OK) return rc_p; }
    TLC_HIP_CHECK(hipStreamSynchronize((hipStream_t)stream));
    const long long v[12] = {g->last_n_hi, g->cnt_n_hi, g->cnt_pipelined, g->cnt_early, g->cnt_beyond_spec, g->cnt_poisoned,
                             g->cnt_poison_bytes, g->poison_region[0], g->poison_region[1], g->poison_region[2], g->cnt_deferred,
                             g->max_busy};
    for (int k = 0; k < n && k < 12; ++k) h_out[k] = v[k];
    return TLC_OK;
}

extern "C" int tlc_debug_tier_counts(tlc_graph* g, long long* h_out, void* stream) {
    TLC_REQUIRE(g && h_out, "null argument");
    TLC_ON_DEVICE(g->device);
    { int rc_p = finish_pending(g); if (rc_p != TLC_OK) return rc_p; }
    TLC_HIP_CHECK(hipStreamSynchronize((hipStream_t)stream));
    for (int t = 0; t < TLC_N_TIERS; ++t) h_out[t] = g->last_tc[t];
    return TLC_OK;
}


extern "C" int tlc_pd_pi_batch_set_timing(tlc_graph* g, int enable) {
    TLC_REQUIRE(g != nullptr, "null graph");
    g->timing = enable == 1 ? 0xff : (enable > 1 ? (enable >> 1) & 0xff : 0);
    return TLC_OK;
}

extern "C" int tlc_pd_pi_batch_timings(tlc_graph* g, double* h_ms, void* stream) {
    TLC_REQUIRE(g && h_ms, "null argument");
    TLC_ON_DEVICE(g->device);
    { int rc_p = finish_pending(g); if (rc_p != TLC_OK) return rc_p; }
    TLC_HIP_CHECK(hipStreamSynchronize((hipStream_t)stream));
    for (int k = 0; k < 8; ++k) {
        h_ms[k] = -1.0;
        if (g->timing && g->ev_used && g->ev_used[k]) {
            TLC_HIP_CHECK(hipEventSynchronize(g->ev_t[2 * k + 1]));
            float ms = 0.f;
            TLC_HIP_CHECK(hipEventElapsedTime(&ms, g->ev_t[2 * k], g->ev_t[2 * k + 1]));
            h_ms[k] = (double)ms;
        }
    }
    return TLC_OK;
}

extern "C" int tlc_pd_pi_batch_timing_history(tlc_graph* g, int slot, double* h_ms, int32_t cap, int32_t* n_out, void* stream) {
    TLC_REQUIRE(g && h_ms && n_out, "null argument");
    TLC_REQUIRE(slot >= 0 && slot < 8 && cap >= 0, "slot must be in 0..7");
    TLC_ON_DEVICE(g->device);
    { int rc_p = finish_pending(g); if (rc_p != TLC_OK) return rc_p; }
    TLC_HIP_CHECK(hipStreamSynchronize((hipStream_t)stream));
    const unsigned long long have = std::min<unsigned long long>(g->ring_pos, TLC_TIMING_RING);
    const int n = (int)std::min<unsigned long long>(have, (unsigned long long)cap);
    for (int i = 0; i < n; ++i) {
        const int set = (int)((g->ring_pos - n + i) % TLC_TIMING_RING);
        h_ms[i] = -1.0;
        if (g->ev_ring_ready && g->ev_ring_used[set][slot]) {
            TLC_HIP_CHECK(hipEventSynchronize(g->ev_ring[set][2 * slot + 1]));
            float ms = 0.f;
            TLC_HIP_CHECK(hipEventElapsedTime(&ms, g->ev_ring[set][2 * slot], g->ev_ring[set][2 * slot + 1]));
            h_ms[i] = (double)ms;
        }
    }
    *n_out = n;
    return TLC_OK;
}

extern "C" int tlc_pd_pi_batch_sizes(tlc_graph* g, int32_t* h_n, int32_t* h_m2, int64_t cap, void* stream) {
    TLC_REQUIRE(g && h_n && h_m2, "null argument");
    TLC_ON_DEVICE(g->device);
    { int rc_p = finish_pending(g); if (rc_p != TLC_OK) return rc_p; }
    TLC_HIP_CHECK(hipStreamSynchronize((hipStream_t)stream));
    const size_t k = (size_t)std::min<int64_t>(cap, g->last_n_pairs);
    if (k && g->last_ws) {
        if (g->last_ws->busy) { TLC_HIP_CHECK(hipEventSynchronize(g->last_ws->ev_done)); g->last_ws->busy = 0; }
        TLC_HIP_CHECK(hipMemcpy(h_n, g->last_ws->hdr_n, k * sizeof(int), hipMemcpyDeviceToHost));
        TLC_HIP_CHECK(hipMemcpy(h_m2, g->last_ws->hdr_m2, k * sizeof(int), hipMemcpyDeviceToHost));
    }
    return TLC_OK;
}

extern "C" int tlc_pd_pi_algorithmic_bytes(int32_t n_nodes, const int32_t* h_rowptr, const int32_t* h_col, const int32_t* h_pairs,
                                           int64_t n_pairs, int hop, int res, double* h_out_bytes) {
    TLC_REQUIRE(n_nodes > 0 && h_rowptr && h_col && h_out_bytes && (n_pairs == 0 || h_pairs), "null argument");
    std::vector<int> su(n_nodes, 0), sv(n_nodes, 0), sx(n_nodes, 0), fr(n_nodes), nx(n_nodes), ball(n_nodes);
    int ep = 0;
    for (int64_t i = 0; i < n_pairs; ++i) {
        const int u = h_pairs[2 * i], v = h_pairs[2 * i + 1];
        double b = 8.0 + 8.0 * res * res;
        if (u < 0 || v < 0 || u >= n_nodes || v >= n_nodes || h_rowptr[u + 1] == h_rowptr[u] || h_rowptr[v + 1] == h_rowptr[v]) {
            h_out_bytes[i] = b;
            continue;
        }
        ++ep;
        int n_ball = 0;
        for (int side = 0; side < 2; ++side) {
            const int root = side ? v : u;
            std::vector<int>& st = side ? sv : su;
            int nf = 1;
            fr[0] = root; st[root] = ep;
            if (side == 0) ball[n_ball++] = root;
// ... 23 lines not shown
```

tlc-gnn_amd/csrc/extract.hip:

```cpp
#include "vicinity_dev.h"

#define TLC_X_HV_CAP 2048
#define TLC_X_H_CAP 128
#define TLC_X_BLOCK 4096
#define TLC_X_BIN_MIN 64
#define TLC_X_COUNTERS 8
#define TLC_X_COUNTER_STRIDE 64

namespace {

template <int BW>
struct XCfg {
    static constexpr int SID_CAP = (BW == 64) ? 256 : 2048;
};

#define TLC_X_UNITS (1024 + TLC_X_H_CAP * TLC_X_H_CAP / 64)
constexpr int X_STAGE = 128;
struct XLayout {
    size_t o_pref, o_sid, o_hvy, o_hl, o_ctl, o_ucnt, o_stage, o_mt, total;
};
#define TLC_X_MT_BYTES ((TLC_BE_CAP / 64) * 16)
__host__ __device__ __forceinline__ constexpr XLayout x_layout(int nw, int sid_cap, int bw, bool fast = false) {
    XLayout L{};
    const size_t nw4 = (size_t)((nw + 3) & ~3);
    if (fast) {
        L.o_pref = nw4 * 4;
        L.o_sid = (L.o_pref + 15) & ~(size_t)15;
        L.o_hvy = L.o_hl = L.o_ctl = L.o_sid + (size_t)sid_cap * 4;
        L.o_ucnt = L.o_ctl + 64 + 4 + 16;
        L.o_stage = (L.o_ucnt + 15) & ~(size_t)15;
        L.o_mt = L.o_stage;
        L.total = L.o_mt + TLC_X_MT_BYTES;
        return L;
    }
    L.o_pref = nw4 * 4;
    L.o_sid = (L.o_pref + nw4 * 2 + 15) & ~(size_t)15;
    L.o_hvy = L.o_sid + (size_t)sid_cap * 4;
    L.o_hl = L.o_hvy + TLC_X_HV_CAP / 8;
    L.o_ctl = L.o_hl + (size_t)TLC_X_H_CAP * 4;
    L.o_ucnt = L.o_ctl + 64 + (size_t)(bw / 64) * 4 + 16;
    L.o_stage = (L.o_ucnt + (bw > 64 ? (size_t)TLC_X_UNITS * 4 : 0) + 15) & ~(size_t)15;
    L.o_mt = L.o_stage + (size_t)(bw / 64) * X_STAGE * 12;
    L.total = L.o_mt + TLC_X_MT_BYTES;
    return L;
}

struct XState {
    unsigned* bits;
    unsigned short* pref;
    unsigned* hvy;
    unsigned* hl;
    int* ucnt;
    unsigned char* stage;
    int* ctl;
    int* xw;
};

__device__ __forceinline__ bool x_member(const XState& X, int y, int& ly) {
    const unsigned word = X.bits[y >> 5];
    const unsigned bit = 1u << (y & 31);
    if (!(word & bit)) return false;
    ly = (int)X.pref[y >> 5] + __popc(word & (bit - 1u));
    return true;
}
struct XRec {
    int rb, deg, hidx, n_in;
    int c0, c1, c2, c3;
    double w0, w1, w2, w3;
    __device__ __forceinline__ int c(int q) const { return q == 0 ? c0 : (q == 1 ? c1 : (q == 2 ? c2 : c3)); }
    __device__ __forceinline__ double w(int q) const { return q == 0 ? w0 : (q == 1 ? w1 : (q == 2 ? w2 : w3)); }
};
__device__ __forceinline__ XRec x_empty_rec() {
    XRec R;
    R.rb = R.deg = R.n_in = 0; R.hidx = -1;
    R.c0 = R.c1 = R.c2 = R.c3 = 0;
    R.w0 = R.w1 = R.w2 = R.w3 = 0.0;
    return R;
}
__device__ __forceinline__ XRec x_load_rec(const TlcNodeRec* r) {
    XRec R;
    const TlcI4 h = *reinterpret_cast<const TlcI4*>(r), c = *reinterpret_cast<const TlcI4*>(&r->col[0]);
    const TlcD2 wa = *reinterpret_cast<const TlcD2*>(&r->w[0]), wb = *reinterpret_cast<const TlcD2*>(&r->w[2]);
    R.rb = h.v[0]; R.deg = h.v[1]; R.hidx = h.v[2]; R.n_in = h.v[3];
    R.c0 = c.v[0]; R.c1 = c.v[1]; R.c2 = c.v[2]; R.c3 = c.v[3];
    R.w0 = wa.v[0]; R.w1 = wa.v[1]; R.w2 = wb.v[0]; R.w3 = wb.v[1];
    return R;
}

template <int BW>
__device__ __forceinline__ void x_sync() {
    if (BW == 64) {
        __builtin_amdgcn_fence(__ATOMIC_ACQ_REL, "wavefront");
        __builtin_amdgcn_wave_barrier();
    } else {
        __syncthreads();
    }
}
template <typename T>
__device__ __forceinline__ void x_store(T* p, T v) { *p = v; }
__device__ __forceinline__ bool x_heavy(const XState& X, int ly) { return (X.hvy[ly >> 5] >> (ly & 31)) & 1u; }

template <int BW, bool WR, class PB>
__device__ __forceinline__ int x_sweep_wave(const PB& p, const int* ids, int n, const XState& X, bool use_hvy, int nH,
                                            unsigned* dir, double* lw, int cap, int* ucnt, const XRec pre, bool has_pre, int dbg_i = -1) {
    const int lane = tlc_lane(), wv = (int)(threadIdx.x >> 6);
    constexpr int NW = BW / 64;
    int run = 0, counted = 0;
#ifdef TLC_PAIR_TIMES
#define SSTAMP(k) do { if (WR && dbg_i >= 0 && p.dbg_pair_t && threadIdx.x == 0) p.dbg_pair_t[16 * (size_t)dbg_i + (k)] = wall_clock64(); } while (0)
#else
#define SSTAMP(k) do { } while (0)
#endif
    SSTAMP(8);
    double* const st_w = reinterpret_cast<double*>(X.stage + (size_t)wv * X_STAGE * 12);
    unsigned* const st_d = reinterpret_cast<unsigned*>(st_w + X_STAGE);
    int st_fb = 0, st_fill = 0;
    auto st_flush = [&]() {
        if (!WR || st_fill == 0) return;
        x_sync<64>();
        for (int k = lane; k < st_fill; k += TLC_WAVE) {
            const int e = st_fb + k;
            if (e < cap) { x_store(&dir[e], st_d[k]); x_store(&lw[e], st_w[k]); }
        }
        x_sync<64>();
        st_fill = 0;
    };
    auto st_round = [&](int r0, int tot) -> bool {
        if (!WR) return false;
        if (st_fill && (r0 != st_fb + st_fill || st_fill + tot > X_STAGE)) st_flush();
        if (tot > X_STAGE) return false;
        if (!st_fill) st_fb = r0;
        st_fill += tot;
        return true;
    };
    auto st_put = [&](bool staged, int off, unsigned d, double w) {
        if (staged) { st_d[off - st_fb] = d; st_w[off - st_fb] = w; }
        else if (off < cap) { x_store(&dir[off], d); x_store(&lw[off], w); }
    };
// ... 204 lines not shown
            const int j = j0 + u * TLC_WAVE + lane;
            const bool in = j < e1;
            pos_[u] = in ? be_pos[j] : 0u;
            w_[u] = (in && dir) ? be_w[j] : 0.0;
        }
#pragma unroll
        for (int u = 0; u < UN; ++u) {
            if (j0 + u * TLC_WAVE >= e1) break;
            const bool in = j0 + u * TLC_WAVE + lane < e1;
            const unsigned pos = pos_[u];
            bool ma, mb;
            unsigned ra, rb;
            look(pos >> 16, ma, ra);
            look(pos & 0xffffu, mb, rb);
            const bool keep = in && ma && mb;
            const unsigned long long K = __ballot(keep);
            if (dir && keep) {
                const int o = run + __popcll(K & tlc_lanemask_lt());
                if (o < cap) { x_store(&dir[o], (ra << 16) | rb); x_store(&lw[o], w_[u]); }
            }
            run += __popcll(K);
        }
    }
    return run;
}

template <int BW, class PB>
__device__ __forceinline__ int x_sweep(const PB& p, const int* ids, int n, const XState& X, bool use_hvy, int nH,
                                       unsigned* dir, double* lw, int cap, const XRec pre, bool has_pre, int dbg_i = -1) {
    if (BW == 64) {
        if (dir) return x_sweep_wave<BW, true>(p, ids, n, X, use_hvy, nH, dir, lw, cap, nullptr, pre, has_pre, dbg_i);
        return x_sweep_wave<BW, false>(p, ids, n, X, use_hvy, nH, nullptr, nullptr, 0, nullptr, pre, has_pre);
    }
    int* ucnt = X.ucnt;
    x_sweep_wave<BW, false>(p, ids, n, X, use_hvy, nH, nullptr, nullptr, 0, ucnt, pre, false);
    x_sync<BW>();
    const int nu = ((n + 63) >> 6) + ((use_hvy && nH > 0) ? ((nH * nH + 63) >> 6) : 0);
    const int per = (nu + BW - 1) / BW;
    const int u0 = (int)threadIdx.x * per;
    int mine = 0;
    for (int q = 0; q < per; ++q) if (u0 + q < nu) mine += ucnt[u0 + q];
    int total = 0;
    int off = block_escan_i32<BW>(mine, X.xw, &total);
    for (int q = 0; q < per; ++q) if (u0 + q < nu) { const int c = ucnt[u0 + q]; ucnt[u0 + q] = off; off += c; }
    x_sync<BW>();
    if (dir) x_sweep_wave<BW, true>(p, ids, n, X, use_hvy, nH, dir, lw, cap, ucnt, pre, false);
    x_sync<BW>();
    return total;
}

template <int BW, class PB>
__device__ __forceinline__ void x_zero_row(const PB& p, int i, int status, int n_report, int lu, int lv) {
    const int tid = threadIdx.x, res2 = p.res * p.res;
    if (tid == 0) {
        p.hdr_n[i] = 0; p.hdr_m2[i] = 0; p.hdr_lu[i] = lu; p.hdr_lv[i] = lv;
        if (p.out_status) p.out_status[i] = (unsigned char)status;
        if (p.out_n) p.out_n[i] = n_report;
        if (p.out_m) p.out_m[i] = 0;
    }
    if (p.out_pi) for (int c = tid; c < res2; c += BW) p.out_pi[(size_t)i * res2 + c] = 0.0;
}

struct XHead {
    int u, v;
    int ru0, ru1, rv0, rv1, a0, a1, b0, b1;
    int eu0, eu1, ev0, ev1;
};
template <int BW, bool FAST = false, class PB>
__device__ __forceinline__ void extract_pair(const PB& p, int i, bool from_rest, const XHead& H, unsigned char* lds, int* slot) {
    static_assert(!FAST || BW == 64, "the FAST launch is one wavefront per pair");
    constexpr int SID_CAP = FAST ? TLC_BE_CAP + 8 : XCfg<BW>::SID_CAP;
    const XLayout L = x_layout(p.nw, SID_CAP, BW, FAST);
    const int nw4 = (p.nw + 3) & ~3;
    XState X;
    X.bits = (unsigned*)lds;
    X.pref = (unsigned short*)(lds + L.o_pref);
    int* sid = (int*)(lds + L.o_sid);
    X.hvy = (unsigned*)(lds + L.o_hvy);
    X.hl = (unsigned*)(lds + L.o_hl);
    X.ctl = (int*)(lds + L.o_ctl);
    X.xw = X.ctl + 16;
    X.ucnt = (int*)(lds + L.o_ucnt);
    X.stage = lds + L.o_stage;
    int tid_ = threadIdx.x;
    asm volatile("" : "+v"(tid_));
    const int tid = tid_;
#ifdef TLC_PAIR_TIMES
#define XSTAMP(k) do { if (p.dbg_pair_t && tid == 0) p.dbg_pair_t[16 * (size_t)i + (k)] = wall_clock64(); } while (0)
#else
#define XSTAMP(k) do { } while (0)
#endif
#ifdef TLC_PAIR_TIMES
    const unsigned long long t_start = wall_clock64();
#endif
    if constexpr (FAST) {
        __builtin_assume(p.x_fill == 0); __builtin_assume(p.fill_mode == 0); __builtin_assume(p.early_list == nullptr);
        __builtin_assume(p.skip_count == nullptr); __builtin_assume(p.big_count == nullptr); __builtin_assume(p.be_ptr != nullptr);
        __builtin_assume((p.flags & TLC_INCLUDE_ROOTS) == 0u); __builtin_assume(p.bump_top != nullptr);
    }
    const int u = H.u, v = H.v;
    bool missing = u < 0 || v < 0 || u >= p.n_nodes || v >= p.n_nodes;
    int a0 = 0, a1 = 0, b0 = 0, b1 = 0;
    if (!missing) {
        a0 = H.a0; a1 = H.a1; b0 = H.b0; b1 = H.b1;
        missing = (H.ru1 == H.ru0) || (H.rv1 == H.rv0);
        if (!missing && from_rest && !FAST) {
            const int na = a1 - a0, nb = b1 - b0, mn = na < nb ? na : nb;
            if (p.skip_count && mn >= p.skip_threshold) {
                if (*p.skip_count <= p.skip_cap) return;
            } else if (p.big_count && mn >= TLC_X_BIN_MIN) return;
        }
    }
    int fill_m2 = 0;
    if (p.x_fill) {
        const int hn = p.hdr_n[i];
        if (hn <= 0) return;
        fill_m2 = p.hdr_m2[i];
        if (p.fill_mode == 2 && (hn > TLC_M_NMAX || (fill_m2 >> 1) > TLC_M_MMAX)) return;
    }
    if (missing) {
        if (FAST || !p.fast_split || p.x_fill) x_zero_row<BW>(p, i, TLC_ST_MISSING_NODE, 0, -1, -1);
        return;
    }
#ifdef TLC_PAIR_TIMES
    if (p.dbg_pair_t && tid == 0) { p.dbg_pair_t[16 * (size_t)i] = t_start; p.dbg_pair_t[16 * (size_t)i + 1] = wall_clock64(); p.dbg_pair_t[16 * (size_t)i + 14] = blockIdx.x; }
#endif
    if (a1 - a0 < b1 - b0) { int t = a0; a0 = b0; b0 = t; t = a1; a1 = b1; b1 = t; }
    const int nA = a1 - a0, nB = b1 - b0;
    int be0 = 0, be1 = 0;
    bool fast = false;
    if constexpr (BW == 64) {
        if (p.be_ptr && nB <= TLC_BE_CAP && !(p.flags & TLC_INCLUDE_ROOTS) && !(p.early_min_ball > 0 && nB >= p.early_min_ball)) {
            const bool b_is_u = (H.a1 - H.a0) < (H.b1 - H.b0);
            be0 = b_is_u ? H.eu0 : H.ev0; be1 = b_is_u ? H.eu1 : H.ev1;
            fast = true;
        }
    }
    if constexpr (FAST) { if (!fast) return; }
    else if (fast && p.fast_split && !p.x_fill) return;
    unsigned long long M0 = 0ull, M1 = 0ull;
    uint4* const mtab = reinterpret_cast<uint4*>(lds + L.o_mt);
    int bv[4];
#pragma unroll
    for (int r = 0; r < 4; ++r) {
        const int j = r * BW + tid;
        bv[r] = j < nB ? p.bcol[b0 + j] : -1;
    }
    const unsigned* bbrow = nullptr;
    if constexpr (FAST) {
        if (p.bbits) bbrow = p.bbits + (size_t)(((H.a1 - H.a0) < (H.b1 - H.b0)) ? v : u) * (size_t)p.bb_nw;
    }
    for (int j = tid; j < (bbrow ? 0 : nA); j += 4 * BW) {
        int av[4];
#pragma unroll
        for (int r = 0; r < 4; ++r) av[r] = (j + r * BW < nA) ? p.bcol[a0 + j + r * BW] : -1;
#pragma unroll
        for (int r = 0; r < 4; ++r) if (av[r] >= 0) atomicOr(&X.bits[av[r] >> 5], 1u << (av[r] & 31));
    }
    if (tid == 0) { X.ctl[0] = -1; X.ctl[1] = -1; }
    x_sync<BW>();
    XSTAMP(2);
    const int capg = p.n_nodes < TLC_MAX_SUBGRAPH_NODES + 1 ? p.n_nodes : TLC_MAX_SUBGRAPH_NODES + 1;
    const bool incl = (p.flags & TLC_INCLUDE_ROOTS) != 0u;
    const bool in_lds = nB + (incl ? 2 : 0) <= SID_CAP;
    int* ids = in_lds ? sid : slot;
    const int cap_ids = in_lds ? SID_CAP : capg;
// ... 93 lines not shown
            if (BW == 64 && base == 0) {
                rec0 = x_load_rec(p.nrec + x);
                if (heavy_ok && x != u && x != v) hi = rec0.hidx;
            } else if (heavy_ok && x != u && x != v) hi = p.nrec[x].hidx;
            const int w = x >> 5;
            atomicOr(&X.bits[w], 1u << (x & 31));
            if (k == 0 || (ids[k - 1] >> 5) != w) X.pref[w] = (unsigned short)k;
        }
        if (heavy_ok) {
            int q, tot;
            if (BW == 64) {
                const unsigned long long mk = __ballot(hi >= 0);
                q = nH + __popcll(mk & tlc_lanemask_lt());
                tot = __popcll(mk);
            } else {
                q = nH + block_escan_i32<BW>(hi >= 0 ? 1 : 0, X.xw, &tot);
            }
            if (hi >= 0) {
                atomicOr(&X.hvy[k >> 5], 1u << (k & 31));
                if (q < TLC_X_H_CAP) X.hl[q] = ((unsigned)k << 16) | (unsigned)hi;
            }
            nH += tot;
        }
    }
    x_sync<BW>();
    const bool use_hvy = heavy_ok && nH <= TLC_X_H_CAP;
    XSTAMP(5);
    auto sweep = [&](unsigned* d_, double* w_, int cap_, int dbg_i) -> int {
        if (FAST || fast) {
            if (nB > TLC_BE_REG_CAP) return x_sweep_ball<true>(p.be_pos, p.be_w, be0, be1, 0ull, 0ull, mtab, d_, w_, cap_);
            return x_sweep_ball<false>(p.be_pos, p.be_w, be0, be1, M0, M1, nullptr, d_, w_, cap_);
        }
        if constexpr (!FAST) return x_sweep<BW>(p, ids, n, X, use_hvy, nH, d_, w_, cap_, rec0, BW == 64, dbg_i);
        return 0;
    };
    if (p.x_fill) {
        const long long eo = p.edge_off[i];
        sweep(p.A_dir + eo, p.A_lw + eo, fill_m2, -1);
        if (fast) return;
        x_sync<BW>();
        for (int k = tid; k < n; k += BW) X.bits[ids[k] >> 5] = 0u;
        x_sync<BW>();
        return;
    }
    long long* cur = (long long*)(X.ctl + 8);
    unsigned* wdir = nullptr;
    double* wlw = nullptr;
    int cap = 0;
    long long at = -1;
    const bool early_large_ok = p.early_list != nullptr && n <= TLC_L_NMAX;
    if (p.bump_top && n <= TLC_M_NMAX) {
        const long long nn = (long long)n * n;
        cap = nn < 2 * TLC_M_MMAX ? (int)nn : 2 * TLC_M_MMAX;
        if (fast && be1 - be0 < cap) cap = be1 - be0;
        if (cur[1] - cur[0] < cap) {
            x_sync<BW>();
            if (tid == 0) {
                long long off = p.bump_base + (long long)atomicAdd(p.bump_top, (unsigned long long)TLC_X_BLOCK);
                if (off + TLC_X_BLOCK > p.bump_cap) { off = -1; atomicAdd(p.bump_overflow, 1); }
                cur[0] = off; cur[1] = off < 0 ? -1 : off + TLC_X_BLOCK;
            }
            x_sync<BW>();
        }
        at = cur[1] - cur[0] >= cap ? cur[0] : -1;
        if (at >= 0) { wdir = p.A_dir + at; wlw = p.A_lw + at; } else cap = 0;
    }
    int es = -1;
    if (!wdir && early_large_ok && n > TLC_M_NMAX) {
        if (tid == 0) X.ctl[4] = atomicAdd(p.early_count, 1);
        x_sync<BW>();
        es = X.ctl[4];
        if (es < p.early_cap) {
            wdir = p.early_dir + (size_t)es * (2 * TLC_L_MMAX);
            wlw = p.early_lw + (size_t)es * (2 * TLC_L_MMAX);
            cap = 2 * TLC_L_MMAX;
        }
    }
    const int m2 = sweep(wdir, wlw, cap, i);
    XSTAMP(6);
    const int m = m2 >> 1;
    if (m > TLC_MAX_SUBGRAPH_EDGES) {
        x_zero_row<BW>(p, i, TLC_ST_TOO_LARGE, -n, lu, lv);
    } else {
        if (tid == 0) { p.hdr_n[i] = n; p.hdr_m2[i] = m2; p.hdr_lu[i] = lu; p.hdr_lv[i] = lv; }
        if (at >= 0 && m <= TLC_M_MMAX) {
            if (tid == 0) { p.edge_off[i] = at; cur[0] = at + m2; }
        } else if (p.bump_top && n <= TLC_M_NMAX && m <= TLC_M_MMAX) {
            if (tid == 0) p.edge_off[i] = -1;
        } else if (n <= TLC_M_NMAX && m > TLC_M_MMAX && early_large_ok && m <= TLC_L_MMAX) {
            if (tid == 0) X.ctl[4] = atomicAdd(p.early_count, 1);
            x_sync<BW>();
            es = X.ctl[4];
            if (es < p.early_cap) {
                sweep(p.early_dir + (size_t)es * (2 * TLC_L_MMAX), p.early_lw + (size_t)es * (2 * TLC_L_MMAX), 2 * TLC_L_MMAX, -1);
                if (tid == 0) p.early_list[es] = i;
            }
        } else if (es >= 0 && es < p.early_cap) {
            if (m <= TLC_L_MMAX) { if (tid == 0) p.early_list[es] = i; }
            else if (tid == 0) p.early_list[es] = -1;
        }
    }
    if (!FAST && !fast) {
        x_sync<BW>();
        for (int k = tid; k < n; k += BW) X.bits[ids[k] >> 5] = 0u;
        x_sync<BW>();
    }
    XSTAMP(7);
#undef XSTAMP
}

}

typedef const __attribute__((address_space(4))) TlcVicParams XParams;
typedef const __attribute__((address_space(4))) int XCInt;
template <int BW, bool FAST>
__global__ __launch_bounds__(BW, BW == 64 ? (FAST ? 8 : 4) : 1) void tlc_extract_kernel(TlcVicParams p) {
    extern __shared__ __attribute__((aligned(16))) unsigned char xlds[];
    int* slot = p.scratch + (size_t)(p.scratch_base_slot + blockIdx.x) * p.scratch_stride;
    {
        const int nw4 = (p.nw + 3) & ~3;
        uint4* z = reinterpret_cast<uint4*>(xlds);
        for (int w = threadIdx.x; w < nw4 / 4; w += BW) z[w] = make_uint4(0u, 0u, 0u, 0u);
        __syncthreads();
    }
    {
        const XLayout L = x_layout(p.nw, FAST ? TLC_BE_CAP + 8 : XCfg<BW>::SID_CAP, BW, FAST);
        long long* cur = (long long*)((int*)(xlds + L.o_ctl) + 8);
        if (threadIdx.x == 0) {
            const long long b = p.region_base_entries + (long long)(p.region_base_wg + (int)blockIdx.x) * p.region_entries;
            cur[0] = b; cur[1] = b + p.region_entries;
            if (!p.bump_top) cur[1] = cur[0] = 0;
        }
        __syncthreads();
    }
    int c0 = 0, c1 = 0, c2 = 0;
    int n_work = p.n_pairs;
    if (p.fill_mode == 1) {
        n_work = p.fill_count;
        if (p.work_count_dev) { const int c = *p.work_count_dev; n_work = c < n_work ? c : n_work; }
    } else if (p.big_count && !FAST) {
        c0 = p.big_count[0]; c1 = p.big_count[1]; c2 = p.big_count[2];
        if (p.fast_split && !p.x_fill && !(p.skip_count && *p.skip_count > p.skip_cap)) { c2 = 0; n_work = 0; }
        n_work += c0 + c1 + c2;
    }
    XParams* kp = (XParams*)__builtin_amdgcn_kernarg_segment_ptr();
    auto idx_of = [&](XParams* q, int w, bool& from_rest) -> int {
        from_rest = false;
        if (q->fill_mode == 1) return ((XCInt*)q->fill_list)[w];
        if (w < c0) return ((XCInt*)q->big_list)[w];
        if (w < c0 + c1) return ((XCInt*)q->big_list)[(size_t)q->n_pairs + (w - c0)];
        if (w < c0 + c1 + c2) return ((XCInt*)q->big_list)[2 * (size_t)q->n_pairs + (w - c0 - c1)];
        from_rest = true;
        return w - c0 - c1 - c2;
    };
    auto pair_of = [&](XParams* q, int i, int& u, int& v) {
        XCInt* pr = (XCInt*)q->pairs + 2 * (size_t)i;
        u = pr[0]; v = pr[1];
    };
    auto bounds_of = [&](XParams* q, XHead& H) {
        H.ru0 = H.ru1 = H.rv0 = H.rv1 = H.a0 = H.a1 = H.b0 = H.b1 = 0;
        H.eu0 = H.eu1 = H.ev0 = H.ev1 = 0;
        if (H.u < 0 || H.v < 0 || H.u >= q->n_nodes || H.v >= q->n_nodes) return;
        XCInt* rp = (XCInt*)q->rowptr;
        XCInt* bp = (XCInt*)q->bptr;
        H.ru0 = rp[H.u]; H.ru1 = rp[H.u + 1]; H.rv0 = rp[H.v]; H.rv1 = rp[H.v + 1];
        H.a0 = bp[H.u]; H.a1 = bp[H.u + 1]; H.b0 = bp[H.v]; H.b1 = bp[H.v + 1];
        if (BW == 64 && q->be_ptr) {
            XCInt* ep = (XCInt*)q->be_ptr;
            H.eu0 = ep[H.u]; H.eu1 = ep[H.u + 1]; H.ev0 = ep[H.v]; H.ev1 = ep[H.v + 1];
        }
    };
    if (p.started && threadIdx.x == 0 && (int)blockIdx.x < n_work) atomicAdd(p.started, 1);
    __shared__ int s_chunk;
    const bool dyn = p.work_counter != nullptr;
    const int n_chunks = dyn ? (n_work + p.work_chunk - 1) / p.work_chunk : n_work;
    int ck = (int)(blockIdx.x % TLC_X_COUNTERS), dry = 0;
    for (int c = blockIdx.x; c < n_chunks;) {
        int nxt = 0;
        if (dyn && BW == 64 && threadIdx.x == 0) nxt = atomicAdd(p.work_counter + ck * TLC_X_COUNTER_STRIDE, 1);
        bool fr0 = false, fr1 = false;
        int i0 = -1, i1 = -1, u0 = -1, v0 = -1;
        {
            XParams* q = kp;
            asm volatile("" : "+s"(q));
            i0 = idx_of(q, c, fr0);
            if (c + n_chunks < n_work) i1 = idx_of(q, c + n_chunks, fr1);
            pair_of(q, i0, u0, v0);
        }
        for (int w = c; w < n_work; w += n_chunks) {
            XParams* q = kp;
            asm volatile("" : "+s"(q));
            bool fr2 = false;
            int i2 = -1, u1 = -1, v1 = -1;
            if (w + 2 * n_chunks < n_work) i2 = idx_of(q, w + 2 * n_chunks, fr2);
            if (w + n_chunks < n_work) pair_of(q, i1, u1, v1);
            XHead H;
            H.u = u0; H.v = v0;
            bounds_of(q, H);
            extract_pair<BW, FAST>(*q, i0, fr0, H, xlds, slot);
            i0 = i1; fr0 = fr1; u0 = u1; v0 = v1;
            i1 = i2; fr1 = fr2;
        }
        if (!dyn) { c += gridDim.x; continue; }
        if (BW == 64) {
            c = (int)gridDim.x + TLC_X_COUNTERS * __builtin_amdgcn_readfirstlane(nxt) + ck;
            while (c >= n_chunks && ++dry < TLC_X_COUNTERS) {
                ck = (ck + 1) % TLC_X_COUNTERS;
                int* cnt = p.work_counter + ck * TLC_X_COUNTER_STRIDE;
                int t = 0;
                if (threadIdx.x == 0) t = __atomic_load_n(cnt, __ATOMIC_RELAXED);
                if ((int)gridDim.x + TLC_X_COUNTERS * __builtin_amdgcn_readfirstlane(t) + ck >= n_chunks) continue;
                if (threadIdx.x == 0) t = atomicAdd(cnt, 1);
                c = (int)gridDim.x + TLC_X_COUNTERS * __builtin_amdgcn_readfirstlane(t) + ck;
            }
        } else {
            if (threadIdx.x == 0) s_chunk = (int)gridDim.x + atomicAdd(p.work_counter, 1);
            __syncthreads();
            c = __builtin_amdgcn_readfirstlane(s_chunk);
            __syncthreads();
        }
    }
}

template __global__ void tlc_extract_kernel<64, false>(TlcVicParams);
template __global__ void tlc_extract_kernel<64, true>(TlcVicParams);
template __global__ void tlc_extract_kernel<512, false>(TlcVicParams);

size_t tlc_extract_lds_bytes(int nw, int bw, bool fast) { return x_layout(nw, fast ? TLC_BE_CAP + 8 : (bw == 64 ? XCfg<64>::SID_CAP : XCfg<512>::SID_CAP), bw, fast).total; }

int tlc_launch_extract(int bw, int grid, size_t lds, const TlcVicParams& p, void* stream, bool fast) {
    if (grid <= 0) return TLC_OK;
    if (fast) {
        if (lds > 64 * 1024) TLC_HIP_CHECK(hipFuncSetAttribute((const void*)tlc_extract_kernel<64, true>, hipFuncAttributeMaxDynamicSharedMemorySize, (int)lds));
        hipLaunchKernelGGL((tlc_extract_kernel<64, true>), dim3(grid), dim3(64), lds, (hipStream_t)stream, p);
    } else if (bw == 64) {
        if (lds > 64 * 1024) TLC_HIP_CHECK(hipFuncSetAttribute((const void*)tlc_extract_kernel<64, false>, hipFuncAttributeMaxDynamicSharedMemorySize, (int)lds));
        hipLaunchKernelGGL((tlc_extract_kernel<64, false>), dim3(grid), dim3(64), lds, (hipStream_t)stream, p);
    } else {
        if (lds > 64 * 1024) TLC_HIP_CHECK(hipFuncSetAttribute((const void*)tlc_extract_kernel<512, false>, hipFuncAttributeMaxDynamicSharedMemorySize, (int)lds));
        hipLaunchKernelGGL((tlc_extract_kernel<512, false>), dim3(grid), dim3(512), lds, (hipStream_t)stream, p);
    }
    TLC_HIP_CHECK(hipGetLastError());
    return TLC_OK;
}

__global__ void tlc_classify_kernel(int n_pairs, const int* __restrict__ pairs, int n_nodes, const int* __restrict__ bptr,
                                    int cand_threshold, int cand_cap, int* __restrict__ cand_count, int* __restrict__ cand_list,
                                    int* __restrict__ big_count, int* __restrict__ big_list) {
    const int i = blockIdx.x * blockDim.x + threadIdx.x;
    int cls = -1;
    if (i < n_pairs) {
        const int u = pairs[2 * (size_t)i], v = pairs[2 * (size_t)i + 1];
        if (u >= 0 && v >= 0 && u < n_nodes && v < n_nodes) {
            int a0, a1, b0, b1;
            row_bounds(bptr, u, a0, a1);
            row_bounds(bptr, v, b0, b1);
            const int a = a1 - a0, b = b1 - b0;
            const int k = a < b ? a : b;
            if (cand_list && k >= cand_threshold) cls = 3;
            else if (k >= 256) cls = 0;
            else if (k >= 128) cls = 1;
            else if (k >= TLC_X_BIN_MIN) cls = 2;
        }
    }
    unsigned long long mk[4];
#pragma unroll
    for (int c = 0; c < 4; ++c) mk[c] = __ballot(cls == c);
    const int lane = tlc_lane();
    int base = 0;
    if (lane < 4) {
        const unsigned long long m = lane == 0 ? mk[0] : (lane == 1 ? mk[1] : (lane == 2 ? mk[2] : mk[3]));
        if (m) base = atomicAdd(lane == 3 ? cand_count : &big_count[lane], __popcll(m));
    }
#pragma unroll
    for (int c = 0; c < 4; ++c) {
        const int bc = __builtin_amdgcn_readlane(base, c);
        if (cls == c) {
            const int pos = bc + __popcll(mk[c] & tlc_lanemask_lt());
            if (c == 3) { if (pos < cand_cap) cand_list[pos] = i; }
            else big_list[(size_t)c * n_pairs + pos] = i;
        }
    }
}
int tlc_launch_classify(int n_pairs, const int* pairs, int n_nodes, const int* bptr, int cand_threshold, int cand_cap,
                        int* cand_count, int* cand_list, int* big_count, int* big_list, void* stream) {
    if (n_pairs <= 0) return TLC_OK;
    hipLaunchKernelGGL(tlc_classify_kernel, dim3((n_pairs + 255) / 256), dim3(256), 0, (hipStream_t)stream, n_pairs, pairs, n_nodes,
                       bptr, cand_threshold, cand_cap, cand_count, cand_list, big_count, big_list);
    TLC_HIP_CHECK(hipGetLastError());
    return TLC_OK;
}

template <bool FILL>
__global__ __launch_bounds__(64) void tlc_ball_list_kernel(int n_nodes, int nw, const int* __restrict__ rowptr, const int* __restrict__ col,
                                                           int hop, int* __restrict__ bsize, const int* __restrict__ bptr, int* __restrict__ bcol) {
    extern __shared__ __attribute__((aligned(16))) unsigned bbits[];
    const int lane = tlc_lane();
    const int wpl = (nw + 63) / 64;
    const int w0 = lane * wpl < nw ? lane * wpl : nw, w1 = (w0 + wpl) < nw ? (w0 + wpl) : nw;
    for (int w = w0; w < w1; ++w) bbits[w] = 0u;
    __syncthreads();
    unsigned* cur = bbits + nw;
    unsigned* nxt = cur + nw;
// ... 158 lines not shown
```

tlc-gnn_amd/csrc/tlc_kernels.h:

```cpp
#pragma once
#include <stdint.h>

#ifndef TLC_ST_TOO_LARGE
#define TLC_ST_TOO_LARGE 5
#endif

#define TLC_TIER_SMALL 0
#define TLC_TIER_MEDIUM 1
#define TLC_TIER_LARGE 2
#define TLC_TIER_HUGE 3
#define TLC_TIER_MID 4
#define TLC_TIER_MEDHI 6
#ifndef TLC_MH_MIN_POS
#define TLC_MH_MIN_POS 120
#endif
#define TLC_TIER_TINY 5
#define TLC_TIER_MEDWIDE 7
#define TLC_MAX_SUBGRAPH_NODES 65535
#define TLC_MAX_SUBGRAPH_EDGES ((1 << 24) - 2)
#define TLC_N_TIERS 8
#ifndef TLC_SCAN_BLOCK
#define TLC_SCAN_BLOCK 1024
#endif
#define TLC_SCAN_MAX_BLOCKS ((1 << 20) / TLC_SCAN_BLOCK)
#ifndef TLC_DC_MIN_POS_SHARED
#define TLC_DC_MIN_POS_SHARED 320
#endif
#ifndef TLC_TINY_BINS
#define TLC_TINY_BINS 8
#define TLC_TINY_BIN_W 5
#endif

#ifndef TLC_T_NMAX
#define TLC_T_NMAX 16
#define TLC_T_MMAX 24
#endif
#ifndef TLC_T_NCUT
#define TLC_T_NCUT TLC_T_NMAX
#endif
#ifndef TLC_T_MCUT
#define TLC_T_MCUT TLC_T_MMAX
#endif
#define TLC_S_NMAX 64
#define TLC_S_MMAX 128
#define TLC_D_NMAX 128
#define TLC_D_MMAX 256
#define TLC_D_THREADS 128
#define TLC_M_NMAX 512
#define TLC_M_MMAX 1024
#ifndef TLC_C_NMAX
#define TLC_C_NMAX 384
#define TLC_C_MMAX 512
#endif
#define TLC_L_NMAX 2048
#define TLC_L_MMAX 4096
#define TLC_L_THREADS 512
#define TLC_HUGE_MIN_TABLE 16384

struct __attribute__((aligned(64))) TlcNodeRec {
    int row_start, deg, hidx, n_in;
    int col[4];
    double w[4];
};

struct TlcVicParams {
    int n_nodes;
    int nw;
    const int* rowptr;
    const int* col;
    const double* w;
    const int* pairs;
    int n_pairs;
    int hop;
    unsigned flags;
    int res;
    int* scratch;
    long long scratch_stride;
    int* hdr_n;
    int* hdr_m2;
    int* hdr_lu;
    int* hdr_lv;
    double* out_pi;
    unsigned char* out_status;
    int* out_n;
    int* out_m;
    long long* edge_off;
    unsigned* A_dir;
    double* A_lw;
    unsigned long long* bump_top;
    long long bump_cap;
    int* bump_overflow;
    const long long* ids_off;
    int* out_ids;
    int fill_mode;
    const int* fill_list;
    int fill_count;
    const int* work_count_dev;
    int scratch_base_slot;
    int* work_counter;
    int work_chunk;
    int* early_list;
    int* early_count;
    int early_cap;
    unsigned* early_dir;
    double* early_lw;
    int* started;
    unsigned* small_dir;
    double* small_lw;
    unsigned long long* dbg;
    unsigned long long* dbg_pair_t;
    const int* bptr;
    const int* bcol;
    const TlcNodeRec* nrec;
    const double* hh_w;
    int hh_k;
    int skip_threshold;
    const int* skip_count;
    int skip_cap;
    const int* big_count;
    const int* big_list;
    int x_fill;
    int region_base_wg;
    long long region_entries;
    long long region_base_entries;
    long long bump_base;
    const int* be_ptr;
    const unsigned* be_pos;
    const double* be_w;
    const unsigned* bbits;
    int bb_nw;
    int fast_split;
    int early_min_ball;
};
#define TLC_BE_CAP 512
#define TLC_BE_REG_CAP 128

struct TlcScanParams {
    int n_pairs;
    const int* hdr_n;
    const int* hdr_m2;
    long long* block_agg;
    int* block_flag;
    int* sync;
    long long* totals;
    long long* edge_off;
    int* tier_count;
    int* tier_list;
    int small_arena;
    int mh_min_pos;
    int mh_compact_only;
    int tiny_ok;
    int* dcm_count;
    int* h_dcm;
    int* tiny_bin_count;
    int* tiny_bin_list;
    int* h_tiny_bins;
    const unsigned long long* bump_top;
    long long bump_base;
    const int* bump_overflow;
    int* h_overflow;
    const int* early_list;
    const int* early_count;
    int early_cap;
    int* h_early;
    long long* h_total;
    int* h_tier;
    unsigned* h_seq;
    unsigned seq;
};

struct TlcPdParams {
    const int* tier_list;
    int tier_count;
    const int* tier_list_hi;
    int n_hi;
    const int* hdr_n;
    const int* hdr_m2;
    const int* hdr_lu;
    const int* hdr_lv;
    const long long* edge_off;
    const unsigned* A_dir;
    const double* A_lw;
    const unsigned* small_dir;
    const double* small_lw;
    unsigned flags;
    int res;
    double* out_pi;
    unsigned char* out_status;
    const long long* ids_off;
    double* out_f;
    int* out_n;
    const long long* edges_off;
    int* out_edges;
    int* out_m;
    int pi_enabled;
    unsigned char* huge_scratch;
    long long huge_stride;
    int huge_nmax;
    int huge_mmax;
    int huge_slots;
    int huge_lds;
    const int* tiny_bin_list;
    int tiny_bin_stride;
    int tiny_bin_cnt[TLC_TINY_BINS];
    unsigned long long* stats;
    unsigned long long* phase_cycles;
    int* started;
    unsigned char* handoff;
    long long handoff_stride;
    const int* tier_count_dev;
    long long slot_entries;
    int* dc_count;
    int* dc_list;
    int dc_inplace;
// ... 62 lines not shown
```

tlc-gnn_amd/csrc/vicinity.hip:

```cpp
#include "vicinity_dev.h"

template <bool FILL, int BW>
__global__ __launch_bounds__(BW) void tlc_vicinity_kernel(TlcVicParams p) {
    extern __shared__ __attribute__((aligned(16))) unsigned lds[];
    int* slot = p.scratch + (size_t)(p.scratch_base_slot + blockIdx.x) * p.scratch_stride;
    int n_work = p.n_pairs;
    if (p.fill_mode == 1) {
        n_work = p.fill_count;
        if (p.work_count_dev) { const int c = *p.work_count_dev; n_work = c < n_work ? c : n_work; }
    }
    if (p.started && threadIdx.x == 0 && (int)blockIdx.x < n_work) atomicAdd(p.started, 1);
    if (p.work_counter) {
        __shared__ int s_chunk;
        const int n_chunks = (n_work + p.work_chunk - 1) / p.work_chunk;
        for (int c = blockIdx.x;;) {
            if (c >= n_chunks) break;
            for (int wi = c; wi < n_work; wi += n_chunks) vicinity_pair<FILL, BW>(p, p.fill_mode == 1 ? p.fill_list[wi] : wi, lds, slot);
            if (threadIdx.x == 0) s_chunk = (int)gridDim.x + atomicAdd(p.work_counter, 1);
            __syncthreads();
            c = s_chunk;
            __syncthreads();
        }
        return;
    }
    for (int wi = blockIdx.x; wi < n_work; wi += gridDim.x) {
        const int i = p.fill_mode == 1 ? p.fill_list[wi] : wi;
        vicinity_pair<FILL, BW>(p, i, lds, slot);
    }
}

template __global__ void tlc_vicinity_kernel<false, 64>(TlcVicParams);
template __global__ void tlc_vicinity_kernel<false, 512>(TlcVicParams);
template __global__ void tlc_vicinity_kernel<true, 64>(TlcVicParams);
template __global__ void tlc_vicinity_kernel<true, 512>(TlcVicParams);

#define SCAN_BLOCK TLC_SCAN_BLOCK

__device__ __forceinline__ long long arena_entries(int n, int m2, int small_arena, bool bumped) {
    if (n <= 0) return 0;
    if (small_arena && n <= TLC_S_NMAX && (m2 >> 1) <= TLC_S_MMAX) return 0;
    if (bumped && n <= TLC_M_NMAX && (m2 >> 1) <= TLC_M_MMAX) return 0;
    return (long long)m2;
}

__global__ __launch_bounds__(SCAN_BLOCK) void tlc_scan_bin(TlcScanParams p) {
    __shared__ long long s_wave[SCAN_BLOCK / TLC_WAVE];
    __shared__ long long s_prefix;
    __shared__ int s_bid;
    __shared__ unsigned s_pre[SCAN_BLOCK / 32];
    __shared__ int s_tc[TLC_N_TIERS][SCAN_BLOCK / TLC_WAVE];
    __shared__ int s_tbase[TLC_N_TIERS];
    __shared__ int s_bc[TLC_TINY_BINS][SCAN_BLOCK / TLC_WAVE];
    __shared__ int s_bbase[TLC_TINY_BINS];
    const int t = threadIdx.x, lane = t & 63, wave = t >> 6;
    if (t == 0) s_bid = atomicAdd(&p.sync[0], 1);
    if (t < SCAN_BLOCK / 32) s_pre[t] = 0u;
    __syncthreads();
    const int bid = s_bid;
    const int i = bid * SCAN_BLOCK + t;
    int n_early = 0;
    if (p.early_list) {
        n_early = *p.early_count;
        n_early = n_early < p.early_cap ? n_early : p.early_cap;
        for (int k = t; k < n_early; k += SCAN_BLOCK) {
            const int j = p.early_list[k] - bid * SCAN_BLOCK;
            if (j >= 0 && j < SCAN_BLOCK) atomicOr(&s_pre[j >> 5], 1u << (j & 31));
        }
        __syncthreads();
    }
    const bool pre = (s_pre[t >> 5] >> (t & 31)) & 1u;
    int n = i < p.n_pairs ? p.hdr_n[i] : 0;
    const int m2v = i < p.n_pairs ? p.hdr_m2[i] : 0;
    const bool bumped = p.bump_top != nullptr && *p.bump_overflow == 0;
    const long long arena_base = bumped ? p.bump_base + (long long)*p.bump_top : 0;
    const long long own = (i < p.n_pairs && !pre) ? arena_entries(n, m2v, p.small_arena, bumped) : 0;
    long long incl = (long long)(unsigned)tlc_wave_iscan_i32((int)own);
    if (lane == 63) s_wave[wave] = incl;
    __syncthreads();
    long long wbase = 0, btotal = 0;
#pragma unroll
    for (int k = 0; k < SCAN_BLOCK / TLC_WAVE; ++k) {
        const long long v = s_wave[k];
        if (k < wave) wbase += v;
        btotal += v;
    }
    if (t == 0) {
        p.block_agg[bid] = btotal;
        __hip_atomic_store(&p.block_flag[bid], 1, __ATOMIC_RELEASE, __HIP_MEMORY_SCOPE_AGENT);
    }
    if (wave == 0) {
        long long acc = 0;
        for (int base = 0; base < bid; base += TLC_WAVE) {
            const int j = base + lane;
            long long v = 0;
            if (j < bid) {
                while (__hip_atomic_load(&p.block_flag[j], __ATOMIC_ACQUIRE, __HIP_MEMORY_SCOPE_AGENT) == 0) __builtin_amdgcn_s_sleep(1);
                v = __hip_atomic_load(&p.block_agg[j], __ATOMIC_RELAXED, __HIP_MEMORY_SCOPE_AGENT);
            }
            acc += tlc_wave_sum_i64(v);
        }
        if (lane == 0) s_prefix = acc;
    }
    __syncthreads();
    int tier = -1;
    if (i < p.n_pairs) {
        if (own > 0 || !bumped) p.edge_off[i] = arena_base + s_prefix + wbase + incl - own;
        if (n > 0 && !pre) {
            const int m = m2v >> 1;
            tier = TLC_TIER_HUGE;
            if (p.tiny_ok && n <= TLC_T_NCUT && m <= TLC_T_MCUT) tier = TLC_TIER_TINY;
            else if (n <= TLC_S_NMAX && m <= TLC_S_MMAX) tier = TLC_TIER_SMALL;
            else if (n <= TLC_D_NMAX && m <= TLC_D_MMAX) tier = TLC_TIER_MID;
            else if (n <= TLC_M_NMAX && m <= TLC_M_MMAX) {
                const bool wide = n > TLC_C_NMAX || m > TLC_C_MMAX || m - n + 1 >= TLC_DC_MIN_POS_SHARED;
                const bool split = p.mh_min_pos != 0x7fffffff;
                if (split && !p.mh_compact_only && (wide || m - n + 1 >= p.mh_min_pos)) tier = TLC_TIER_MEDHI;
                else if (split && p.mh_compact_only && !wide && m - n + 1 >= p.mh_min_pos) tier = TLC_TIER_MEDHI;
                else tier = wide ? TLC_TIER_MEDWIDE : TLC_TIER_MEDIUM;
            }
            else if (n <= TLC_L_NMAX && m <= TLC_L_MMAX) tier = TLC_TIER_LARGE;
        }
    }
    int my_rank = 0;
#pragma unroll
    for (int tt = 0; tt < TLC_N_TIERS; ++tt) {
        const unsigned long long mk = __ballot(tier == tt);
        if (lane == 0) s_tc[tt][wave] = __popcll(mk);
        if (tier == tt) my_rank = __popcll(mk & tlc_lanemask_lt());
    }
    __syncthreads();
    if (t < TLC_N_TIERS) {
        int tot = 0;
        for (int k = 0; k < SCAN_BLOCK / TLC_WAVE; ++k) { const int c = s_tc[t][k]; s_tc[t][k] = tot; tot += c; }
        s_tbase[t] = tot > 0 ? atomicAdd(&p.tier_count[t], tot) : 0;
    }
    __syncthreads();
    if (tier >= 0) p.tier_list[(size_t)tier * p.n_pairs + s_tbase[tier] + s_tc[tier][wave] + my_rank] = i;
    if (p.dcm_count) {
        const int mm = m2v >> 1;
        const bool big = (tier == TLC_TIER_MEDHI || tier == TLC_TIER_MEDWIDE) && mm - n + 1 >= TLC_DC_MIN_POS_SHARED && mm <= 8 * 256;
        const unsigned long long mk = __ballot(big);
        if (lane == 0 && mk) atomicAdd(p.dcm_count, __popcll(mk));
    }
    if (p.tiny_bin_count) {
        int bin = -1;
        if (tier == TLC_TIER_TINY) {
            const int c = (n + (m2v >> 1)) / TLC_TINY_BIN_W;
            bin = TLC_TINY_BINS - 1 - (c < TLC_TINY_BINS - 1 ? c : TLC_TINY_BINS - 1);
        }
        int brank = 0;
#pragma unroll
        for (int b = 0; b < TLC_TINY_BINS; ++b) {
            const unsigned long long mk = __ballot(bin == b);
            if (lane == 0) s_bc[b][wave] = __popcll(mk);
            if (bin == b) brank = __popcll(mk & tlc_lanemask_lt());
        }
        __syncthreads();
        if (t < TLC_TINY_BINS) {
            int tot = 0;
            for (int k = 0; k < SCAN_BLOCK / TLC_WAVE; ++k) { const int c = s_bc[t][k]; s_bc[t][k] = tot; tot += c; }
            s_bbase[t] = tot > 0 ? atomicAdd(&p.tiny_bin_count[t], tot) : 0;
        }
        __syncthreads();
        if (bin >= 0) p.tiny_bin_list[(size_t)bin * p.n_pairs + s_bbase[bin] + s_bc[bin][wave] + brank] = i;
    }
    __syncthreads();
    if (t == 0) {
        atomicAdd(reinterpret_cast<unsigned long long*>(p.sync + 2), (unsigned long long)btotal);
        __threadfence();
        if (atomicAdd(&p.sync[1], 1) == (int)gridDim.x - 1) {
            const long long total = arena_base + (long long)__hip_atomic_load(reinterpret_cast<unsigned long long*>(p.sync + 2),
                                                                              __ATOMIC_RELAXED, __HIP_MEMORY_SCOPE_AGENT);
            if (p.h_overflow) *p.h_overflow = p.bump_overflow ? *p.bump_overflow : 0;
            p.totals[0] = total;
            *p.h_total = total;
            if (p.h_early) {
                int valid = 0;
                for (int k = 0; k < n_early; ++k) valid += p.early_list[k] >= 0 ? 1 : 0;
                *p.h_early = valid;
            }
            for (int tt = 0; tt < TLC_N_TIERS; ++tt)
                p.h_tier[tt] = __hip_atomic_load(&p.tier_count[tt], __ATOMIC_RELAXED, __HIP_MEMORY_SCOPE_AGENT);
            if (p.dcm_count && p.h_dcm) *p.h_dcm = __hip_atomic_load(p.dcm_count, __ATOMIC_RELAXED, __HIP_MEMORY_SCOPE_AGENT);
            if (p.tiny_bin_count && p.h_tiny_bins)
                for (int b = 0; b < TLC_TINY_BINS; ++b)
                    p.h_tiny_bins[b] = __hip_atomic_load(&p.tiny_bin_count[b], __ATOMIC_RELAXED, __HIP_MEMORY_SCOPE_AGENT);
            __threadfence_system();
            __hip_atomic_store(p.h_seq, p.seq, __ATOMIC_RELEASE, __HIP_MEMORY_SCOPE_SYSTEM);
        }
    }
}

__global__ void tlc_ball_bound_kernel(int n_nodes, const int* __restrict__ rowptr, const int* __restrict__ col,
                                      const int* __restrict__ prev, int* __restrict__ out) {
    const int x = blockIdx.x * blockDim.x + threadIdx.x;
    if (x >= n_nodes) return;
    const int b = rowptr[x], e = rowptr[x + 1];
    long long s = 1;
    if (!prev) s += e - b;
    else for (int j = b; j < e; ++j) s += prev[col[j]];
    out[x] = s > (1 << 30) ? (1 << 30) : (int)s;
}
int tlc_launch_ball_bound(int n_nodes, const int* rowptr, const int* col, const int* prev, int* out, void* stream) {
    if (n_nodes <= 0) return TLC_OK;
    hipLaunchKernelGGL(tlc_ball_bound_kernel, dim3((n_nodes + 255) / 256), dim3(256), 0, (hipStream_t)stream, n_nodes, rowptr, col,
                       prev, out);
    TLC_HIP_CHECK(hipGetLastError());
    return TLC_OK;
}

__global__ void tlc_select_heavy_kernel(int n_pairs, const int* __restrict__ pairs, int n_nodes, const int* __restrict__ ub,
                                        int threshold, int cap, int* __restrict__ count, int* __restrict__ list) {
    const int i = blockIdx.x * blockDim.x + threadIdx.x;
    bool cand = false;
    if (i < n_pairs) {
        const int u = pairs[2 * (size_t)i], v = pairs[2 * (size_t)i + 1];
        if (u >= 0 && v >= 0 && u < n_nodes && v < n_nodes) {
            const int a = ub[u], b = ub[v];
            cand = (a < b ? a : b) >= threshold;
        }
    }
    const unsigned long long mk = __ballot(cand);
    if (mk == 0ull) return;
    int base = 0;
    const int leader = __builtin_ctzll(mk);
    if ((int)(threadIdx.x & 63) == leader) base = atomicAdd(count, __popcll(mk));
    base = __builtin_amdgcn_readlane(base, leader);
    const int pos = base + __popcll(mk & tlc_lanemask_lt());
    if (cand && pos < cap) list[pos] = i;
}
int tlc_launch_select_heavy(int n_pairs, const int* pairs, int n_nodes, const int* ub, int threshold, int cap, int* count,
                            int* list, void* stream) {
// ... 7 lines not shown
```

tlc-gnn_amd/engine.py:

```python
import ctypes as C

import numpy as np

from . import _lib
from ._lib import KEEP_ZERO_PERS, INCLUDE_ROOTS, NORM_EPS, PI_ORD0_EXT1, NO_EXT1, UNREACHABLE_100


class DeviceGraph:

    def __init__(self, rowptr, col, w, device=None):
        torch = _lib.require_gpu()
        self.device = torch.cuda.current_device() if device is None else int(device)
        rowptr = np.ascontiguousarray(rowptr, dtype=np.int32)
        col = np.ascontiguousarray(col, dtype=np.int32)
        w = np.ascontiguousarray(w, dtype=np.float64)
        self.n_nodes = len(rowptr) - 1
        self.nnz = int(rowptr[-1])
        h = C.c_void_p()
        rc = _lib.lib().tlc_graph_create(C.c_int32(self.n_nodes), rowptr.ctypes.data_as(C.c_void_p),
                                         col.ctypes.data_as(C.c_void_p), w.ctypes.data_as(C.c_void_p),
                                         C.c_int(self.device), C.byref(h))
        _lib.check(rc, "tlc_graph_create")
        self._h = h
        self._inflight = []

    def close(self):
        if getattr(self, "_h", None):
            _lib.lib().tlc_graph_destroy(self._h)
            self._h = None

    def __del__(self):
        try:
            self.close()
        except Exception:
            pass

    def pd_pi_batch(self, pairs, hop, flags=0, res=5, out=None, status=None, async_=False):
        import torch
        assert pairs.is_cuda and pairs.dtype == torch.int32 and pairs.dim() == 2 and pairs.shape[1] == 2
        assert pairs.device.index == self.device, "pairs live on cuda:%s, the graph on cuda:%d" % (pairs.device.index, self.device)
        pairs = pairs.contiguous()
        E = pairs.shape[0]
        if out is None:
            out = torch.empty((E, res * res), dtype=torch.float64, device=pairs.device)
        if status is None:
            status = torch.empty((E,), dtype=torch.uint8, device=pairs.device)
        fn = _lib.lib().tlc_pd_pi_batch_async if async_ else _lib.lib().tlc_pd_pi_batch
        rc = fn(self._h, _lib.ptr(pairs), C.c_int64(E), C.c_int(hop), C.c_uint32(flags),
                C.c_int(res), _lib.ptr(out), _lib.ptr(status), _lib.stream_ptr(self.device))
        _lib.check(rc, "tlc_pd_pi_batch")
        if async_:
            self._inflight.append((pairs, out, status))
            del self._inflight[:-6]
        return out, status

    def join(self):
        _lib.check(_lib.lib().tlc_pd_pi_batch_join(self._h, _lib.stream_ptr(self.device)), "tlc_pd_pi_batch_join")

    def stats(self):
        out = (C.c_int64 * 10)()
        rc = _lib.lib().tlc_pd_pi_batch_stats(self._h, C.cast(out, C.c_void_p), _lib.stream_ptr(self.device))
        _lib.check(rc, "tlc_pd_pi_batch_stats")
        v = list(out)
        return {"tier_small": v[0], "tier_medium": v[1], "tier_large": v[2], "tier_huge": v[3],
                "tier_mid": v[7], "tier_tiny": v[8], "tier_medium_many_pos": v[9],
                "induced_entries": v[4], "tie_fallback_sources": v[5], "chunks": v[6]}

    def set_option(self, name, value):
        _lib.check(_lib.lib().tlc_debug_set_option(self._h, name.encode(), C.c_int(int(value))), "tlc_debug_set_option")

    def dc_stats(self):
        out = (C.c_longlong * 2)()
        _lib.check(_lib.lib().tlc_debug_dc_stats(self._h, C.cast(out, C.c_void_p), _lib.stream_ptr(self.device)), "tlc_debug_dc_stats")
        return int(out[0]), int(out[1])

    def tier_counts(self):
        out = (C.c_longlong * 8)()
        _lib.check(_lib.lib().tlc_debug_tier_counts(self._h, C.cast(out, C.c_void_p), _lib.stream_ptr(self.device)), "tlc_debug_tier_counts")
        return dict(zip(("small", "medium", "large", "huge", "mid", "tiny", "medium_many_pos", "medium_wide"), (int(v) for v in out)))

    CHUNK_COUNTERS = ("front_list_last_call", "front_list", "pipelined_chunks", "early_chunks", "beyond_spec_slots", "poisoned_chunks",
                      "poison_bytes", "poison_arena_bytes", "poison_early_bytes", "poison_small_bytes", "deferred_second_halves",
                      "max_busy_workspaces")

    def chunk_counters(self):
        out = (C.c_longlong * len(self.CHUNK_COUNTERS))()
        _lib.check(_lib.lib().tlc_debug_chunk_counters(self._h, C.cast(out, C.c_void_p), C.c_int32(len(out)), _lib.stream_ptr(self.device)),
                   "tlc_debug_chunk_counters")
        return dict(zip(self.CHUNK_COUNTERS, (int(v) for v in out)))

    def front_list_count(self):
        return self.chunk_counters()["front_list_last_call"]

    KERNELS = ["vicinity_count", "scan_bin", "vicinity_fill", "pd_tier_small", "pd_tier_medium", "pd_tier_large", "pd_tier_huge",
               "pd_tier_mid"]

    def set_timing(self, on=True, only=None):
        mask = (1 if on else 0) if only is None else sum(1 << (self.KERNELS.index(k) + 1) for k in only)
        _lib.check(_lib.lib().tlc_pd_pi_batch_set_timing(self._h, C.c_int(mask)), "set_timing")

    def timings(self):
        out = (C.c_double * 8)()
        _lib.check(_lib.lib().tlc_pd_pi_batch_timings(self._h, C.cast(out, C.c_void_p), _lib.stream_ptr(self.device)), "timings")
        return dict(zip(self.KERNELS, list(out)[:8]))

    def timing_history(self, kernel, cap=64):
        out = (C.c_double * cap)()
        n = C.c_int32(0)
        _lib.check(_lib.lib().tlc_pd_pi_batch_timing_history(self._h, C.c_int(self.KERNELS.index(kernel)), C.cast(out, C.c_void_p),
                                                             C.c_int32(cap), C.byref(n), _lib.stream_ptr(self.device)), "timing_history")
        return list(out)[:n.value]

    def sizes(self, n_pairs):
        n = np.zeros(n_pairs, dtype=np.int32)
        m2 = np.zeros(n_pairs, dtype=np.int32)
        _lib.check(_lib.lib().tlc_pd_pi_batch_sizes(self._h, n.ctypes.data_as(C.c_void_p), m2.ctypes.data_as(C.c_void_p),
                                                    C.c_int64(n_pairs), _lib.stream_ptr(self.device)), "sizes")
        return n, m2

    def _capacity_offsets(self, E, cap, dev):
        cache = self.__dict__.setdefault("_cap_offs", {})
        key = (E, cap, str(dev))
        t = cache.get(key)
        if t is None:
            import torch
            if len(cache) >= 8:
                cache.clear()
            t = cache[key] = torch.arange(E + 1, dtype=torch.int64, device=dev) * cap
        return t

    def vicinity_sizes(self, pairs, hop, flags=0):
        import torch
        assert pairs.device.index == self.device, "pairs live on cuda:%s, the graph on cuda:%d" % (pairs.device.index, self.device)
        pairs = pairs.contiguous()
        E = pairs.shape[0]
        n = torch.zeros(max(E, 1), dtype=torch.int32, device=pairs.device)
        m = torch.zeros(max(E, 1), dtype=torch.int32, device=pairs.device)
        rc = _lib.lib().tlc_vicinity_sizes(self._h, _lib.ptr(pairs), C.c_int64(E), C.c_int(hop), C.c_uint32(flags), _lib.ptr(n), _lib.ptr(m),
                                           _lib.stream_ptr(self.device))
        _lib.check(rc, "tlc_vicinity_sizes")
        return n[:E], m[:E]

    def vicinity_filtration(self, pairs, hop, flags=0, cap=None, edge_cap=None, zero=True, offsets=None):
        import torch
        assert pairs.device.index == self.device, "pairs live on cuda:%s, the graph on cuda:%d" % (pairs.device.index, self.device)
        pairs = pairs.contiguous()
        E = pairs.shape[0]
        dev = pairs.device
        mk = torch.zeros if zero else torch.empty
        if offsets is not None:
            offs, eoffs_x, tot_n, tot_m = offsets
            ids = mk(max(int(tot_n), 1), dtype=torch.int32, device=dev)
            f = mk(max(int(tot_n), 1), dtype=torch.float64, device=dev)
            n = torch.zeros(max(E, 1), dtype=torch.int32, device=dev)
            st = torch.zeros(max(E, 1), dtype=torch.uint8, device=dev)
            edges = mk((max(int(tot_m), 1), 2), dtype=torch.int32, device=dev)
            m = torch.zeros(max(E, 1), dtype=torch.int32, device=dev)
            rc = _lib.lib().tlc_vicinity_filtration(self._h, _lib.ptr(pairs), C.c_int64(E), C.c_int(hop), C.c_uint32(flags),
                                                    _lib.ptr(offs), _lib.ptr(ids), _lib.ptr(f), _lib.ptr(n), _lib.ptr(st),
                                                    _lib.ptr(eoffs_x), _lib.ptr(edges), _lib.ptr(m), _lib.stream_ptr(self.device))
            _lib.check(rc, "tlc_vicinity_filtration")
            return offs, ids, f, n[:E], st[:E], eoffs_x, edges, m[:E]
        cap = self.n_nodes if cap is None else int(cap)
        offs = self._capacity_offsets(E, cap, dev)
        ids = mk(max(E * cap, 1), dtype=torch.int32, device=dev)
        f = mk(max(E * cap, 1), dtype=torch.float64, device=dev)
        n = torch.zeros(max(E, 1), dtype=torch.int32, device=dev)
        st = torch.zeros(max(E, 1), dtype=torch.uint8, device=dev)
        eoffs = edges = m = None
        if edge_cap is not None:
            eoffs = self._capacity_offsets(E, int(edge_cap), dev)
            edges = mk((max(E * int(edge_cap), 1), 2), dtype=torch.int32, device=dev)
# ... 279 lines not shown
```

Before: 79.58 million.

## Fold tier binning into extraction kernel to skip separate scan launch

In pipelined plain chunks, the vicinity extraction kernel now bins each pair into its tier and tiny-bin lists itself. It flushes LDS-held batches to global counters and publishes totals to the host through a last-workgroup finish step, so the separate tlc_scan_bin launch is skipped. The tier classification is moved into a shared host/device helper. On bump-arena overflow the host falls back to a full scan. This adds atomics and LDS flushes inside extraction plus extra event waits on the side streams, and it carries a risk of ordering bugs.

Measured after the change: 37.48 million. 52.9% lower.

```diff
diff --git a/include/tlcgnn.h b/include/tlcgnn.h
--- a/include/tlcgnn.h
+++ b/include/tlcgnn.h
@@ -70,6 +70,7 @@
 int tlc_debug_dc_stats(tlc_graph* g, long long* h_out, void* stream);
 int tlc_debug_chunk_counters(tlc_graph* g, long long* h_out, int32_t n, void* stream);
 int tlc_debug_tier_counts(tlc_graph* g, long long* h_out, void* stream);
+int tlc_debug_tier_lists(tlc_graph* g, int32_t* h_lists, int64_t cap, long long* h_counts, void* stream);
 int tlc_debug_phase_profile(tlc_graph* g, int enable, unsigned long long* h_out, int64_t cap_u64, int32_t* n_rows);
 int tlc_debug_pair_times(tlc_graph* g, unsigned long long* h_out, int64_t n_pairs);
 
diff --git a/tlc-gnn_amd/_lib.py b/tlc-gnn_amd/_lib.py
--- a/tlc-gnn_amd/_lib.py
+++ b/tlc-gnn_amd/_lib.py
@@ -26,7 +26,7 @@
     "tlc_nc_curv_bwd_f32", "tlc_spgemm_csr_dense_f32", "tlc_spmm_csr_f32", "tlc_renorm_rows_f32", "tlc_gcn2_encode_f32", "tlc_gcn2_encode_csr_f32",
     "tlc_lp_decode_fused", "tlc_lp_decode_fused_f32", "tlc_gat_layer_fwd", "tlc_gat_layer_tiled_fwd", "tlc_gat_tile_cut", "tlc_csr_by_target", "tlc_pdgnn_forward", "tlc_pdgnn_forward_work_bytes", "tlc_scatter_f32", "tlc_edge_head_fwd",
     "tlc_complement_rows", "tlc_complement_pairs", "tlc_select_rows", "tlc_pack_vicinities", "tlc_stack_batch", "tlc_ollivier_ricci_sinkhorn",
-    "tlc_near_pairs", "tlc_w2_partial_matching", "tlc_w2_inference_matching", "tlc_gat_layer_bwd", "tlc_edge_head_bwd", "tlc_pack_offsets", "tlc_vicinity_sizes", "tlc_debug_dc_stats", "tlc_debug_tier_counts", "tlc_debug_chunk_counters", "tlc_debug_phase_profile", "tlc_debug_set_option", "tlc_debug_pair_times",
+    "tlc_near_pairs", "tlc_w2_partial_matching", "tlc_w2_inference_matching", "tlc_gat_layer_bwd", "tlc_edge_head_bwd", "tlc_pack_offsets", "tlc_vicinity_sizes", "tlc_debug_dc_stats", "tlc_debug_tier_counts", "tlc_debug_tier_lists", "tlc_debug_chunk_counters", "tlc_debug_phase_profile", "tlc_debug_set_option", "tlc_debug_pair_times",
     "tlc_hks_batch", "tlc_hks_batch_work_bytes",
 ]
 
@@ -161,6 +161,7 @@
         L.tlc_debug_dc_stats.argtypes = [C.c_void_p, C.c_void_p, C.c_void_p]
         L.tlc_debug_tier_counts.argtypes = [C.c_void_p, C.c_void_p, C.c_void_p]
         L.tlc_debug_chunk_counters.argtypes = [C.c_void_p, C.c_void_p, C.c_int32, C.c_void_p]
+        L.tlc_debug_tier_lists.argtypes = [C.c_void_p, C.c_void_p, C.c_int64, C.c_void_p, C.c_void_p]
         L.tlc_debug_phase_profile.argtypes = [C.c_void_p, C.c_int, C.c_void_p, C.c_int64, C.c_void_p]
         _lib = L
     return _lib
diff --git a/tlc-gnn_amd/csrc/api.hip b/tlc-gnn_amd/csrc/api.hip
--- a/tlc-gnn_amd/csrc/api.hip
+++ b/tlc-gnn_amd/csrc/api.hip
@@ -36,7 +36,9 @@
 #define TLC_TIMING_RING 64
 #define TLC_X_REGION 4096
 
-#define TLC_CTL_INTS (64 + TLC_SCAN_MAX_BLOCKS + 8 + 8 * 64)
+#define TLC_CTL_SB (64 + TLC_SCAN_MAX_BLOCKS + 8 + 8 * 64)
+static_assert(TLC_CHUNK_PAIRS <= (1 << 20), "the extraction's own binning packs a chunk-local pair index in 20 bits (extract.hip, sb_flush)");
+#define TLC_CTL_INTS (TLC_CTL_SB + TLC_SB_COUNTERS * TLC_SB_STRIDE)
 struct HostSync {
     long long total_entries;
     int tier_count[TLC_N_TIERS];
@@ -58,6 +60,8 @@
 struct ChunkCtx {
     TlcVicParams vp;
     TlcPdParams pp;
+    TlcScanParams sp;
+    bool self_bin;
     hipStream_t s;
     int n_pairs, hop, pi_enabled;
     bool bump, use_x, early, spec, count_only, tiny_bins, pipelined;
@@ -84,6 +88,7 @@
     int* tiny_bins;
     int* big_lists;
     hipEvent_t ev_cls;
+    int last_tc[TLC_N_TIERS], last_tiny[TLC_TINY_BINS], last_early, last_dcm;
     int prev_dcm;
     long long* edge_off;
     int* d_ctl;
@@ -188,6 +193,8 @@
     int opt_x_region, opt_x_bump_min;
     int opt_mh_front_pos;
     int opt_main_beside_early;
+    int opt_self_bin;
+    long long cnt_scans, cnt_self_bin, cnt_sb_fallback;
     int opt_poison;
     long long last_n_hi;
     long long cnt_n_hi, cnt_pipelined, cnt_early, cnt_beyond_spec, cnt_poisoned, cnt_poison_bytes;
@@ -495,7 +502,7 @@
     g->opt_plain_kernels = env_on("TLC_PLAIN_KERNELS") ? 1 : 0;
     g->opt_n_ws = 3;
     g->opt_x_region = TLC_X_REGION; g->opt_x_bump_min = 1 << 20; g->opt_tier_mask = (1 << TLC_N_TIERS) - 1; g->opt_timing_every = 1;
-    g->opt_mh_front_pos = 64; g->opt_main_beside_early = 1;
+    g->opt_mh_front_pos = 64; g->opt_main_beside_early = 1; g->opt_self_bin = 1;
     int rc = TLC_OK;
     auto fail = [&](int code) { tlc_graph_destroy(g); return code; };
 #define CK(e) do { if ((e) != hipSuccess) { tlc_set_error("%s failed: %s", #e, hipGetErrorString(hipGetLastError())); return fail(TLC_ERR_HIP); } } while (0)
@@ -624,6 +631,54 @@
 }
 static const int tslot[TLC_N_TIERS] = {3, 4, 5, 6, 7, 3, 4, 4};
 
+static void front_scan_params(tlc_graph* g, Workspace* ws) {
+    ChunkCtx& c = ws->ctx;
+    TlcVicParams& vp = c.vp;
+    const int n_pairs = c.n_pairs;
+    const bool early = c.early, use_x = c.use_x, plain = c.plain, pipelined = c.pipelined, bump = c.bump;
+    const long long bump_base = c.bump_base;
+    int* d_early_count = ws->d_ctl + 17;
+    unsigned long long* d_bump_top = reinterpret_cast<unsigned long long*>(ws->d_ctl + 20);
+    int* d_bump_overflow = ws->d_ctl + 22;
+
+    const unsigned seq = ++ws->pub_seq;
+    TlcScanParams& sp = c.sp;
+    memset(&sp, 0, sizeof(sp));
+    sp.n_pairs = n_pairs; sp.hdr_n = ws->hdr_n; sp.hdr_m2 = ws->hdr_m2;
+    sp.block_agg = ws->d_block_sums; sp.block_flag = ws->d_ctl + 64; sp.sync = ws->d_ctl + 10; sp.totals = ws->d_totals;
+    sp.edge_off = ws->edge_off; sp.tier_count = ws->d_ctl; sp.tier_list = ws->tier_list; sp.small_arena = use_x ? 0 : 1;
+    const bool mh_split = !pipelined;
+    sp.mh_min_pos = mh_split ? TLC_MH_MIN_POS : 0x7fffffff;
+    c.mh_front = !mh_split && plain && g->opt_mh_front_pos > 0;
+    if (c.mh_front) { sp.mh_min_pos = g->opt_mh_front_pos; sp.mh_compact_only = 1; }
+    sp.tiny_ok = (g->opt_tiny && plain && vp.flags == 0u && vp.res == 5) ? 1 : 0;
+    sp.dcm_count = ws->d_ctl + 44; sp.h_dcm = const_cast<int*>(&ws->h_sync_dev->pub_dcm);
+    static_assert(TLC_TINY_BINS <= 16, "the size-class counters of the TINY list live in d_ctl[48..63]");
+    if (sp.tiny_ok) { sp.tiny_bin_count = ws->d_ctl + 48; sp.tiny_bin_list = ws->tiny_bins; sp.h_tiny_bins = const_cast<int*>(ws->h_sync_dev->pub_tiny); }
+    sp.early_list = early ? ws->d_early_list : nullptr; sp.early_count = d_early_count; sp.early_cap = TLC_EARLY_SLOTS;
+    sp.h_early = const_cast<int*>(&ws->h_sync_dev->pub_early);
+    sp.bump_top = bump ? d_bump_top : nullptr; sp.bump_overflow = d_bump_overflow; sp.bump_base = bump_base;
+    sp.h_overflow = const_cast<int*>(&ws->h_sync_dev->pub_overflow);
+    sp.h_total = const_cast<long long*>(&ws->h_sync_dev->pub_total);
+    sp.h_tier = const_cast<int*>(ws->h_sync_dev->pub_tier);
+    sp.h_seq = const_cast<unsigned*>(&ws->h_sync_dev->pub_seq);
+    sp.seq = seq;
+    c.seq = seq;
+    c.tiny_bins = sp.tiny_bin_count != nullptr;
+}
+
+static int submit_scan(tlc_graph* g, Workspace* ws) {
+    ChunkCtx& c = ws->ctx;
+    hipStream_t s = c.s;
+    const int nb = (c.n_pairs + TLC_SCAN_BLOCK - 1) / TLC_SCAN_BLOCK;
+    T0(1, s);
+    hipLaunchKernelGGL(tlc_scan_bin, dim3(nb), dim3(TLC_SCAN_BLOCK), 0, s, c.sp);
+    T1(1, s);
+    TLC_HIP_CHECK(hipGetLastError());
+    g->cnt_scans += 1;
+    return TLC_OK;
+}
+
 static int front_prepare(tlc_graph* g, Workspace* ws, const int32_t* d_pairs, int n_pairs, int hop, uint32_t flags, int res,
                          double* d_out_pi, uint8_t* d_out_status, const int64_t* d_ids_off, int32_t* d_out_ids,
                          double* d_out_f, int32_t* d_out_n, const int64_t* d_edge_offs, int32_t* d_out_edges, int32_t* d_out_m,
@@ -729,6 +784,19 @@
     c.bump = bump; c.use_x = use_x; c.early = early; c.bump_base = bump_base; c.xgrid = xgrid;
     c.plain = plain; c.fsplit = fsplit; c.xfgrid = xfgrid; c.pipelined = pipelined; c.spec = false;
     c.count_only = g->count_only != 0;
+    if (early && (rc = ensure_early(g, ws, hop, s)) != TLC_OK) return rc;
+    front_scan_params(g, ws);
+    c.self_bin = g->opt_self_bin && pipelined && plain && flags == 0u && use_x && bump && !c.count_only;
+    if (c.self_bin) {
+        TlcSelfBin& sb = vp.sb;
+        const TlcScanParams& sp = c.sp;
+        sb.ctr = ws->d_ctl + TLC_CTL_SB;
+        sb.tier_list = ws->tier_list; sb.tiny_bin_list = ws->tiny_bins;
+        sb.tiny_ok = sp.tiny_ok; sb.mh_min_pos = sp.mh_min_pos; sb.mh_compact_only = sp.mh_compact_only;
+        sb.expected = xgrid + ((early && use_x) ? TLC_EARLY_WG : 0) + xfgrid;
+        sb.h_total = sp.h_total; sb.h_tier = sp.h_tier; sb.h_tiny_bins = const_cast<int*>(ws->h_sync_dev->pub_tiny);
+        sb.h_dcm = sp.h_dcm; sb.h_early = sp.h_early; sb.h_overflow = sp.h_overflow; sb.h_seq = sp.h_seq; sb.seq = sp.seq;
+    }
     return TLC_OK;
 }
 
@@ -873,11 +941,7 @@
     TlcVicParams& vp = c.vp;
     hipStream_t s = c.s;
     const int n_pairs = c.n_pairs, xgrid = c.xgrid, vgrid = c.vgrid;
-    const bool early = c.early, use_x = c.use_x, fsplit = c.fsplit, plain = c.plain, pipelined = c.pipelined, bump = c.bump;
-    const long long bump_base = c.bump_base;
-    int* d_early_count = ws->d_ctl + 17;
-    unsigned long long* d_bump_top = reinterpret_cast<unsigned long long*>(ws->d_ctl + 20);
-    int* d_bump_overflow = ws->d_ctl + 22;
+    const bool early = c.early, use_x = c.use_x, fsplit = c.fsplit, pipelined = c.pipelined;
     vp.work_counter = ws->d_ctl + 64 + TLC_SCAN_MAX_BLOCKS + 8;
     vp.work_chunk = std::max(2, n_pairs / (pipelined ? 4096 : 8192));
     if (fsplit && early) vp.work_chunk = 1;
@@ -890,39 +954,11 @@
     T1(0, s);
     vp.work_counter = nullptr;
     vp.skip_count = nullptr; vp.big_count = nullptr;
+    vp.sb.ctr = nullptr;
     TLC_HIP_CHECK(hipGetLastError());
+    if (c.self_bin) { g->cnt_self_bin += 1; return TLC_OK; }
     if (early) TLC_HIP_CHECK(hipStreamWaitEvent(s, ws->ev_early, 0));
-
-    const int nb = (n_pairs + TLC_SCAN_BLOCK - 1) / TLC_SCAN_BLOCK;
-    T0(1, s);
-    const unsigned seq = ++ws->pub_seq;
-    TlcScanParams sp;
-    memset(&sp, 0, sizeof(sp));
-    sp.n_pairs = n_pairs; sp.hdr_n = ws->hdr_n; sp.hdr_m2 = ws->hdr_m2;
-    sp.block_agg = ws->d_block_sums; sp.block_flag = ws->d_ctl + 64; sp.sync = ws->d_ctl + 10; sp.totals = ws->d_totals;
-    sp.edge_off = ws->edge_off; sp.tier_count = ws->d_ctl; sp.tier_list = ws->tier_list; sp.small_arena = use_x ? 0 : 1;
-    const bool mh_split = !pipelined;
-    sp.mh_min_pos = mh_split ? TLC_MH_MIN_POS : 0x7fffffff;
-    c.mh_front = !mh_split && plain && g->opt_mh_front_pos > 0;
-    if (c.mh_front) { sp.mh_min_pos = g->opt_mh_front_pos; sp.mh_compact_only = 1; }
-    sp.tiny_ok = (g->opt_tiny && plain && vp.flags == 0u && vp.res == 5) ? 1 : 0;
-    sp.dcm_count = ws->d_ctl + 44; sp.h_dcm = const_cast<int*>(&ws->h_sync_dev->pub_dcm);
-    static_assert(TLC_TINY_BINS <= 16, "the size-class counters of the TINY list live in d_ctl[48..63]");
-    if (sp.tiny_ok) { sp.tiny_bin_count = ws->d_ctl + 48; sp.tiny_bin_list = ws->tiny_bins; sp.h_tiny_bins = const_cast<int*>(ws->h_sync_dev->pub_tiny); }
-    sp.early_list = early ? ws->d_early_list : nullptr; sp.early_count = d_early_count; sp.early_cap = TLC_EARLY_SLOTS;
-    sp.h_early = const_cast<int*>(&ws->h_sync_dev->pub_early);
-    sp.bump_top = bump ? d_bump_top : nullptr; sp.bump_overflow = d_bump_overflow; sp.bump_base = bump_base;
-    sp.h_overflow = const_cast<int*>(&ws->h_sync_dev->pub_overflow);
-    sp.h_total = const_cast<long long*>(&ws->h_sync_dev->pub_total);
-    sp.h_tier = const_cast<int*>(ws->h_sync_dev->pub_tier);
-    sp.h_seq = const_cast<unsigned*>(&ws->h_sync_dev->pub_seq);
-    sp.seq = seq;
-    hipLaunchKernelGGL(tlc_scan_bin, dim3(nb), dim3(TLC_SCAN_BLOCK), 0, s, sp);
-    T1(1, s);
-    TLC_HIP_CHECK(hipGetLastError());
-    c.seq = seq;
-    c.tiny_bins = sp.tiny_bin_count != nullptr;
-    return TLC_OK;
+    return submit_scan(g, ws);
 }
 
 static int front_speculative(tlc_graph* g, Workspace* ws) {
@@ -1015,7 +1051,8 @@
         if ((it & 0x3ff) != 0) continue;
         const auto el = std::chrono::steady_clock::now() - t0;
         if (el < std::chrono::microseconds(300)) continue;
-        const hipError_t q = hipStreamQuery(s);
+        hipError_t q = hipStreamQuery(s);
+        if (q == hipSuccess && ws->ctx.self_bin && ws->ctx.early && ws->h_sync->pub_seq != seq) q = hipEventQuery(ws->ev_early);
         if (q == hipSuccess) { seen = (ws->h_sync->pub_seq == seq); break; }
         if (q != hipErrorNotReady) { tlc_set_error(hipGetErrorString(q)); return TLC_ERR_HIP; }
         if (el > std::chrono::seconds(20)) break;
@@ -1038,17 +1075,27 @@
     const int n_pairs = c.n_pairs, hop = c.hop, pi_enabled = c.pi_enabled, xgrid = c.xgrid, vgrid = c.vgrid;
     const bool bump = c.bump, use_x = c.use_x, early = c.early, spec = c.spec;
     const long long bump_base = c.bump_base;
-    const unsigned seq = c.seq;
     size_t (&spec_base)[TLC_N_TIERS] = c.spec_base;
     int (&spec_cap)[TLC_N_TIERS] = c.spec_cap;
     bool (&used)[TLC_N_SIDE] = c.used;
     ws->back_pending = 0;
-    if ((rc = wait_for_sizes(ws, s, seq)) != TLC_OK) return rc;
+    if ((rc = wait_for_sizes(ws, s, c.seq)) != TLC_OK) return rc;
+    if (c.self_bin) {
+        if (early) TLC_HIP_CHECK(hipStreamWaitEvent(s, ws->ev_early, 0));
+        if (ws->h_sync->pub_overflow != 0) {
+            g->cnt_sb_fallback += 1;
+            c.sp.seq = c.seq = ++ws->pub_seq;
+            if ((rc = submit_scan(g, ws)) != TLC_OK) return rc;
+            if ((rc = wait_for_sizes(ws, s, c.seq)) != TLC_OK) return rc;
+        }
+    }
     ht_seen = ht_us();
     std::atomic_thread_fence(std::memory_order_acquire);
     const long long total = ws->h_sync->pub_total;
     int tc[TLC_N_TIERS];
-    for (int t = 0; t < TLC_N_TIERS; ++t) tc[t] = ws->h_sync->pub_tier[t];
+    for (int t = 0; t < TLC_N_TIERS; ++t) ws->last_tc[t] = tc[t] = ws->h_sync->pub_tier[t];
+    for (int b = 0; b < TLC_TINY_BINS; ++b) ws->last_tiny[b] = c.tiny_bins ? ws->h_sync->pub_tiny[b] : 0;
+    ws->last_early = early ? ws->h_sync->pub_early : 0; ws->last_dcm = ws->h_sync->pub_dcm;
     int n_hi = 0;
     if (c.mh_front) { n_hi = tc[TLC_TIER_MEDHI]; tc[TLC_TIER_MEDIUM] += n_hi; tc[TLC_TIER_MEDHI] = 0; }
     g->cnt_n_hi += n_hi;
@@ -1127,6 +1174,7 @@
         auto launch_side = [&](int k, int t, bool behind_s = true) -> int {
             if (bumped && !behind_s) {
                 TLC_HIP_CHECK(hipStreamWaitEvent(ws->side[k], ws->ev_scan, 0));
+                if (c.self_bin && early) TLC_HIP_CHECK(hipStreamWaitEvent(ws->side[k], ws->ev_early, 0));
             } else {
                 TLC_HIP_CHECK(hipEventRecord(ws->ev_fork, s));
                 TLC_HIP_CHECK(hipStreamWaitEvent(ws->side[k], ws->ev_fork, 0));
@@ -1188,7 +1236,10 @@
         }
         auto launch_tiny_small = [&]() -> int {
             if (tc[TLC_TIER_TINY] > 0) {
-                if (bumped) { TLC_HIP_CHECK(hipStreamWaitEvent(ws->side[5], ws->ev_scan, 0)); }
+                if (bumped) {
+                    TLC_HIP_CHECK(hipStreamWaitEvent(ws->side[5], ws->ev_scan, 0));
+                    if (c.self_bin && early) TLC_HIP_CHECK(hipStreamWaitEvent(ws->side[5], ws->ev_early, 0));
+                }
                 else { TLC_HIP_CHECK(hipEventRecord(ws->ev_fork, s)); TLC_HIP_CHECK(hipStreamWaitEvent(ws->side[5], ws->ev_fork, 0)); }
                 pp.tier_list = ws->tier_list + (size_t)TLC_TIER_TINY * n_pairs; pp.tier_count = tc[TLC_TIER_TINY];
                 pp.tiny_bin_list = nullptr;
@@ -1566,6 +1617,7 @@
     else if (!strcmp(name, "x_arena")) { g->opt_x_region = value > 0 ? value : TLC_X_REGION; g->opt_x_bump_min = value > 0 ? value : (1 << 20); }
     else if (!strcmp(name, "mh_front_pos")) g->opt_mh_front_pos = std::max(value, 0);
     else if (!strcmp(name, "main_beside_early")) g->opt_main_beside_early = value != 0;
+    else if (!strcmp(name, "self_bin")) g->opt_self_bin = value != 0;
     else if (!strcmp(name, "poison")) g->opt_poison = value != 0;
     else { tlc_set_error("tlc_debug_set_option: unknown option '%s'", name); return TLC_ERR_INVALID_ARG; }
     return TLC_OK;
@@ -1591,10 +1643,10 @@
     TLC_ON_DEVICE(g->device);
     { int rc_p = finish_pending(g); if (rc_p != TLC_OK) return rc_p; }
     TLC_HIP_CHECK(hipStreamSynchronize((hipStream_t)stream));
-    const long long v[12] = {g->last_n_hi, g->cnt_n_hi, g->cnt_pipelined, g->cnt_early, g->cnt_beyond_spec, g->cnt_poisoned,
+    const long long v[15] = {g->last_n_hi, g->cnt_n_hi, g->cnt_pipelined, g->cnt_early, g->cnt_beyond_spec, g->cnt_poisoned,
                              g->cnt_poison_bytes, g->poison_region[0], g->poison_region[1], g->poison_region[2], g->cnt_deferred,
-                             g->max_busy};
-    for (int k = 0; k < n && k < 12; ++k) h_out[k] = v[k];
+                             g->max_busy, g->cnt_scans, g->cnt_self_bin, g->cnt_sb_fallback};
+    for (int k = 0; k < n && k < 15; ++k) h_out[k] = v[k];
     return TLC_OK;
 }
 
@@ -1604,6 +1656,27 @@
     { int rc_p = finish_pending(g); if (rc_p != TLC_OK) return rc_p; }
     TLC_HIP_CHECK(hipStreamSynchronize((hipStream_t)stream));
     for (int t = 0; t < TLC_N_TIERS; ++t) h_out[t] = g->last_tc[t];
+    return TLC_OK;
+}
+
+extern "C" int tlc_debug_tier_lists(tlc_graph* g, int32_t* h_lists, int64_t cap, long long* h_counts, void* stream) {
+    TLC_REQUIRE(g && h_lists && h_counts && cap >= 0, "null argument");
+    TLC_ON_DEVICE(g->device);
+    { int rc_p = finish_pending(g); if (rc_p != TLC_OK) return rc_p; }
+    TLC_HIP_CHECK(hipStreamSynchronize((hipStream_t)stream));
+    for (int k = 0; k < TLC_N_TIERS + TLC_TINY_BINS + 2; ++k) h_counts[k] = 0;
+    Workspace* ws = g->last_ws;
+    if (!ws) return TLC_OK;
+    if (ws->busy) { TLC_HIP_CHECK(hipEventSynchronize(ws->ev_done)); ws->busy = 0; }
+    for (int k = 0; k < TLC_N_TIERS + TLC_TINY_BINS; ++k) {
+        const int cnt = k < TLC_N_TIERS ? ws->last_tc[k] : ws->last_tiny[k - TLC_N_TIERS];
+        const int* src = k < TLC_N_TIERS ? ws->tier_list + (size_t)k * ws->n_pairs : ws->tiny_bins + (size_t)(k - TLC_N_TIERS) * ws->n_pairs;
+        h_counts[k] = cnt;
+        const size_t take = (size_t)std::min<int64_t>(cnt, cap);
+        if (take) TLC_HIP_CHECK(hipMemcpy(h_lists + (size_t)k * cap, src, take * sizeof(int), hipMemcpyDeviceToHost));
+    }
+    h_counts[TLC_N_TIERS + TLC_TINY_BINS] = ws->last_early;
+    h_counts[TLC_N_TIERS + TLC_TINY_BINS + 1] = ws->last_dcm;
     return TLC_OK;
 }
 
diff --git a/tlc-gnn_amd/csrc/extract.hip b/tlc-gnn_amd/csrc/extract.hip
--- a/tlc-gnn_amd/csrc/extract.hip
+++ b/tlc-gnn_amd/csrc/extract.hip
@@ -17,8 +17,9 @@
 #define TLC_X_UNITS (1024 + TLC_X_H_CAP * TLC_X_H_CAP / 64)
 constexpr int X_STAGE = 128;
 struct XLayout {
-    size_t o_pref, o_sid, o_hvy, o_hl, o_ctl, o_ucnt, o_stage, o_mt, total;
+    size_t o_pref, o_sid, o_hvy, o_hl, o_ctl, o_ucnt, o_stage, o_mt, o_sb, total;
 };
+#define TLC_X_SB_BYTES (2 * 64 * 4)
 #define TLC_X_MT_BYTES ((TLC_BE_CAP / 64) * 16)
 __host__ __device__ __forceinline__ constexpr XLayout x_layout(int nw, int sid_cap, int bw, bool fast = false) {
     XLayout L{};
@@ -30,7 +31,8 @@
         L.o_ucnt = L.o_ctl + 64 + 4 + 16;
         L.o_stage = (L.o_ucnt + 15) & ~(size_t)15;
         L.o_mt = L.o_stage;
-        L.total = L.o_mt + TLC_X_MT_BYTES;
+        L.o_sb = L.o_mt + TLC_X_MT_BYTES;
+        L.total = L.o_sb + TLC_X_SB_BYTES;
         return L;
     }
     L.o_pref = nw4 * 4;
@@ -41,7 +43,8 @@
     L.o_ucnt = L.o_ctl + 64 + (size_t)(bw / 64) * 4 + 16;
     L.o_stage = (L.o_ucnt + (bw > 64 ? (size_t)TLC_X_UNITS * 4 : 0) + 15) & ~(size_t)15;
     L.o_mt = L.o_stage + (size_t)(bw / 64) * X_STAGE * 12;
-    L.total = L.o_mt + TLC_X_MT_BYTES;
+    L.o_sb = L.o_mt + TLC_X_MT_BYTES;
+    L.total = L.o_sb + TLC_X_SB_BYTES;
     return L;
 }
 
@@ -54,6 +57,7 @@
     unsigned char* stage;
     int* ctl;
     int* xw;
+    int* sb;
 };
 
 __device__ __forceinline__ bool x_member(const XState& X, int y, int& ly) {
@@ -424,6 +428,7 @@
     X.xw = X.ctl + 16;
     X.ucnt = (int*)(lds + L.o_ucnt);
     X.stage = lds + L.o_stage;
+    X.sb = (int*)(lds + L.o_sb);
     int tid_ = threadIdx.x;
     asm volatile("" : "+v"(tid_));
     const int tid = tid_;
@@ -683,6 +688,7 @@
     if (m > TLC_MAX_SUBGRAPH_EDGES) {
         x_zero_row<BW>(p, i, TLC_ST_TOO_LARGE, -n, lu, lv);
     } else {
+        bool pre = false;
         if (tid == 0) { p.hdr_n[i] = n; p.hdr_m2[i] = m2; p.hdr_lu[i] = lu; p.hdr_lv[i] = lv; }
         if (at >= 0 && m <= TLC_M_MMAX) {
             if (tid == 0) { p.edge_off[i] = at; cur[0] = at + m2; }
@@ -695,10 +701,20 @@
             if (es < p.early_cap) {
                 sweep(p.early_dir + (size_t)es * (2 * TLC_L_MMAX), p.early_lw + (size_t)es * (2 * TLC_L_MMAX), 2 * TLC_L_MMAX, -1);
                 if (tid == 0) p.early_list[es] = i;
+                pre = true;
             }
         } else if (es >= 0 && es < p.early_cap) {
-            if (m <= TLC_L_MMAX) { if (tid == 0) p.early_list[es] = i; }
+            if (m <= TLC_L_MMAX) { if (tid == 0) p.early_list[es] = i; pre = true; }
             else if (tid == 0) p.early_list[es] = -1;
+        }
+        if (p.sb.ctr && tid == 0) {
+            if (pre) atomicAdd(p.sb.ctr + TLC_SB_EARLY * TLC_SB_STRIDE, 1);
+            else {
+                const int k = X.ctl[12];
+                X.sb[k] = (int)((unsigned)i | ((unsigned)(n < 4095 ? n : 4095) << 20));
+                X.sb[64 + k] = m2;
+                X.ctl[12] = k + 1;
+            }
         }
     }
     if (!FAST && !fast) {
@@ -708,6 +724,73 @@
     }
     XSTAMP(7);
 #undef XSTAMP
+}
+
+__device__ __forceinline__ void sb_rank(int key, int& leader, int& rank, int& cnt) {
+    leader = -1; rank = 0; cnt = 0;
+    unsigned long long left = __ballot(key >= 0);
+    while (left) {
+        const int src = __builtin_ctzll(left);
+        const int k = __builtin_amdgcn_readlane(key, src);
+        const unsigned long long mk = __ballot(key == k);
+        if (key == k) { leader = src; rank = __popcll(mk & tlc_lanemask_lt()); cnt = __popcll(mk); }
+        left &= ~mk;
+    }
+}
+template <class PB>
+__device__ __forceinline__ void sb_flush(const PB& p, int* ctl, const int* sb, int lane) {
+    const int cnt = ctl[12];
+    if (cnt == 0) return;
+    const bool on = lane < cnt;
+    const unsigned a = on ? (unsigned)sb[lane] : 0u;
+    const int m2 = on ? sb[64 + lane] : 0;
+    const int i = (int)(a & 0xfffffu), n = (int)(a >> 20);
+    int tbin = -1, dcm = 0, tier = -1;
+    if (on) tier = tlc_tier_of(n, m2, p.sb.tiny_ok, p.sb.mh_min_pos, p.sb.mh_compact_only, &tbin, &dcm);
+    int tl, tr, tc, bl, br, bc;
+    sb_rank(tier, tl, tr, tc);
+    sb_rank(tbin, bl, br, bc);
+    int tbase = 0, bbase = 0;
+    if (tl == lane) tbase = atomicAdd(p.sb.ctr + tier * TLC_SB_STRIDE, tc);
+    if (bl == lane) bbase = atomicAdd(p.sb.ctr + (TLC_N_TIERS + tbin) * TLC_SB_STRIDE, bc);
+    if (tier == TLC_TIER_LARGE || tier == TLC_TIER_HUGE)
+        p.edge_off[i] = (long long)atomicAdd(reinterpret_cast<unsigned long long*>(p.sb.ctr + TLC_SB_HEAVY * TLC_SB_STRIDE), (unsigned long long)m2);
+    const unsigned long long dk = __ballot(dcm != 0);
+    if (dk && lane == 0) atomicAdd(p.sb.ctr + TLC_SB_DCM * TLC_SB_STRIDE, __popcll(dk));
+    tbase = __shfl(tbase, tl < 0 ? lane : tl);
+    bbase = __shfl(bbase, bl < 0 ? lane : bl);
+    if (tier >= 0) p.sb.tier_list[(size_t)tier * p.n_pairs + tbase + tr] = i;
+    if (tbin >= 0) p.sb.tiny_bin_list[(size_t)tbin * p.n_pairs + bbase + br] = i;
+    if (lane == 0) ctl[12] = 0;
+}
+template <class PB>
+__device__ __forceinline__ void sb_finish(const PB& p, int lane) {
+    int* const ctr = p.sb.ctr;
+    __threadfence();
+    int last = 0;
+    if (lane == 0) last = atomicAdd(ctr + TLC_SB_DONE * TLC_SB_STRIDE, 1) == p.sb.expected - 1 ? 1 : 0;
+    if (!__builtin_amdgcn_readfirstlane(last)) return;
+    __threadfence();
+    auto ld = [&](int k) { return __hip_atomic_load(ctr + k * TLC_SB_STRIDE, __ATOMIC_RELAXED, __HIP_MEMORY_SCOPE_AGENT); };
+    const long long arena_base = p.bump_base + (long long)__hip_atomic_load(p.bump_top, __ATOMIC_RELAXED, __HIP_MEMORY_SCOPE_AGENT);
+    for (int t = TLC_TIER_LARGE; t <= TLC_TIER_HUGE; ++t) {
+        const int c = ld(t);
+        const int* list = p.sb.tier_list + (size_t)t * p.n_pairs;
+        for (int k = lane; k < c; k += TLC_WAVE) {
+            long long* e = p.edge_off + __hip_atomic_load(list + k, __ATOMIC_RELAXED, __HIP_MEMORY_SCOPE_AGENT);
+            *e = arena_base + __hip_atomic_load(e, __ATOMIC_RELAXED, __HIP_MEMORY_SCOPE_AGENT);
+        }
+    }
+    if (lane != 0) return;
+    *p.sb.h_overflow = __hip_atomic_load(p.bump_overflow, __ATOMIC_RELAXED, __HIP_MEMORY_SCOPE_AGENT);
+    *p.sb.h_total = arena_base + (long long)__hip_atomic_load(reinterpret_cast<unsigned long long*>(ctr + TLC_SB_HEAVY * TLC_SB_STRIDE),
+                                                              __ATOMIC_RELAXED, __HIP_MEMORY_SCOPE_AGENT);
+    *p.sb.h_early = ld(TLC_SB_EARLY);
+    for (int t = 0; t < TLC_N_TIERS; ++t) p.sb.h_tier[t] = ld(t);
+    *p.sb.h_dcm = ld(TLC_SB_DCM);
+    for (int b = 0; b < TLC_TINY_BINS; ++b) p.sb.h_tiny_bins[b] = ld(TLC_N_TIERS + b);
+    __threadfence_system();
+    __hip_atomic_store(p.sb.h_seq, p.sb.seq, __ATOMIC_RELEASE, __HIP_MEMORY_SCOPE_SYSTEM);
 }
 
 }
@@ -731,6 +814,7 @@
             const long long b = p.region_base_entries + (long long)(p.region_base_wg + (int)blockIdx.x) * p.region_entries;
             cur[0] = b; cur[1] = b + p.region_entries;
             if (!p.bump_top) cur[1] = cur[0] = 0;
+            ((int*)cur)[4] = 0;
         }
         __syncthreads();
     }
@@ -776,6 +860,16 @@
     const bool dyn = p.work_counter != nullptr;
     const int n_chunks = dyn ? (n_work + p.work_chunk - 1) / p.work_chunk : n_work;
     int ck = (int)(blockIdx.x % TLC_X_COUNTERS), dry = 0;
+    int held = 0;
+    auto bin_held = [&](XParams* q, bool finish) {
+        x_sync<BW>();
+        if (threadIdx.x < TLC_WAVE) {
+            const XLayout SL = x_layout(q->nw, FAST ? TLC_BE_CAP + 8 : XCfg<BW>::SID_CAP, BW, FAST);
+            sb_flush(*q, (int*)(xlds + SL.o_ctl), (const int*)(xlds + SL.o_sb), (int)threadIdx.x);
+            if (finish) sb_finish(*q, (int)threadIdx.x);
+        }
+        x_sync<BW>();
+    };
     for (int c = blockIdx.x; c < n_chunks;) {
         int nxt = 0;
         if (dyn && BW == 64 && threadIdx.x == 0) nxt = atomicAdd(p.work_counter + ck * TLC_X_COUNTER_STRIDE, 1);
@@ -799,6 +893,7 @@
             H.u = u0; H.v = v0;
             bounds_of(q, H);
             extract_pair<BW, FAST>(*q, i0, fr0, H, xlds, slot);
+            if (q->sb.ctr && ++held == 64) { bin_held(q, false); held = 0; }
             i0 = i1; fr0 = fr1; u0 = u1; v0 = v1;
             i1 = i2; fr1 = fr2;
         }
@@ -820,6 +915,11 @@
             c = __builtin_amdgcn_readfirstlane(s_chunk);
             __syncthreads();
         }
+    }
+    {
+        XParams* q = kp;
+        asm volatile("" : "+s"(q));
+        if (q->sb.ctr) bin_held(q, true);
     }
 }
 
diff --git a/tlc-gnn_amd/csrc/tlc_kernels.h b/tlc-gnn_amd/csrc/tlc_kernels.h
--- a/tlc-gnn_amd/csrc/tlc_kernels.h
+++ b/tlc-gnn_amd/csrc/tlc_kernels.h
@@ -57,10 +57,61 @@
 #define TLC_L_THREADS 512
 #define TLC_HUGE_MIN_TABLE 16384
 
+#ifdef __HIPCC__
+#define TLC_HD __host__ __device__
+#else
+#define TLC_HD
+#endif
+TLC_HD inline int tlc_tier_of(int n, int m2, int tiny_ok, int mh_min_pos, int mh_compact_only, int* tiny_bin, int* dcm) {
+    const int m = m2 >> 1;
+    int tier = TLC_TIER_HUGE;
+    *tiny_bin = -1;
+    *dcm = 0;
+    if (tiny_ok && n <= TLC_T_NCUT && m <= TLC_T_MCUT) {
+        tier = TLC_TIER_TINY;
+        const int c = (n + m) / TLC_TINY_BIN_W;
+        *tiny_bin = TLC_TINY_BINS - 1 - (c < TLC_TINY_BINS - 1 ? c : TLC_TINY_BINS - 1);
+    }
+    else if (n <= TLC_S_NMAX && m <= TLC_S_MMAX) tier = TLC_TIER_SMALL;
+    else if (n <= TLC_D_NMAX && m <= TLC_D_MMAX) tier = TLC_TIER_MID;
+    else if (n <= TLC_M_NMAX && m <= TLC_M_MMAX) {
+        const bool wide = n > TLC_C_NMAX || m > TLC_C_MMAX || m - n + 1 >= TLC_DC_MIN_POS_SHARED;
+        const bool split = mh_min_pos != 0x7fffffff;
+        if (split && !mh_compact_only && (wide || m - n + 1 >= mh_min_pos)) tier = TLC_TIER_MEDHI;
+        else if (split && mh_compact_only && !wide && m - n + 1 >= mh_min_pos) tier = TLC_TIER_MEDHI;
+        else tier = wide ? TLC_TIER_MEDWIDE : TLC_TIER_MEDIUM;
+        *dcm = ((tier == TLC_TIER_MEDHI || tier == TLC_TIER_MEDWIDE) && m - n + 1 >= TLC_DC_MIN_POS_SHARED && m <= 8 * 256) ? 1 : 0;
+    }
+    else if (n <= TLC_L_NMAX && m <= TLC_L_MMAX) tier = TLC_TIER_LARGE;
+    return tier;
+}
+
 struct __attribute__((aligned(64))) TlcNodeRec {
     int row_start, deg, hidx, n_in;
     int col[4];
     double w[4];
+};
+
+#define TLC_SB_STRIDE 64
+#define TLC_SB_DCM (TLC_N_TIERS + TLC_TINY_BINS)
+#define TLC_SB_EARLY (TLC_SB_DCM + 1)
+#define TLC_SB_DONE (TLC_SB_DCM + 2)
+#define TLC_SB_HEAVY (TLC_SB_DCM + 3)
+#define TLC_SB_COUNTERS (TLC_SB_DCM + 4)
+struct TlcSelfBin {
+    int* ctr;
+    int* tier_list;
+    int* tiny_bin_list;
+    int tiny_ok, mh_min_pos, mh_compact_only;
+    int expected;
+    long long* h_total;
+    int* h_tier;
+    int* h_tiny_bins;
+    int* h_dcm;
+    int* h_early;
+    int* h_overflow;
+    unsigned* h_seq;
+    unsigned seq;
 };
 
 struct TlcVicParams {
@@ -130,6 +181,7 @@
     const unsigned* bbits;
     int bb_nw;
     int fast_split;
+    TlcSelfBin sb;
     int early_min_ball;
 };
 #define TLC_BE_CAP 512
diff --git a/tlc-gnn_amd/csrc/vicinity.hip b/tlc-gnn_amd/csrc/vicinity.hip
--- a/tlc-gnn_amd/csrc/vicinity.hip
+++ b/tlc-gnn_amd/csrc/vicinity.hip
@@ -102,24 +102,10 @@
         if (lane == 0) s_prefix = acc;
     }
     __syncthreads();
-    int tier = -1;
+    int tier = -1, tbin = -1, dcm = 0;
     if (i < p.n_pairs) {
         if (own > 0 || !bumped) p.edge_off[i] = arena_base + s_prefix + wbase + incl - own;
-        if (n > 0 && !pre) {
-            const int m = m2v >> 1;
-            tier = TLC_TIER_HUGE;
-            if (p.tiny_ok && n <= TLC_T_NCUT && m <= TLC_T_MCUT) tier = TLC_TIER_TINY;
-            else if (n <= TLC_S_NMAX && m <= TLC_S_MMAX) tier = TLC_TIER_SMALL;
-            else if (n <= TLC_D_NMAX && m <= TLC_D_MMAX) tier = TLC_TIER_MID;
-            else if (n <= TLC_M_NMAX && m <= TLC_M_MMAX) {
-                const bool wide = n > TLC_C_NMAX || m > TLC_C_MMAX || m - n + 1 >= TLC_DC_MIN_POS_SHARED;
-                const bool split = p.mh_min_pos != 0x7fffffff;
-                if (split && !p.mh_compact_only && (wide || m - n + 1 >= p.mh_min_pos)) tier = TLC_TIER_MEDHI;
-                else if (split && p.mh_compact_only && !wide && m - n + 1 >= p.mh_min_pos) tier = TLC_TIER_MEDHI;
-                else tier = wide ? TLC_TIER_MEDWIDE : TLC_TIER_MEDIUM;
-            }
-            else if (n <= TLC_L_NMAX && m <= TLC_L_MMAX) tier = TLC_TIER_LARGE;
-        }
+        if (n > 0 && !pre) tier = tlc_tier_of(n, m2v, p.tiny_ok, p.mh_min_pos, p.mh_compact_only, &tbin, &dcm);
     }
     int my_rank = 0;
 #pragma unroll
@@ -137,17 +123,11 @@
     __syncthreads();
     if (tier >= 0) p.tier_list[(size_t)tier * p.n_pairs + s_tbase[tier] + s_tc[tier][wave] + my_rank] = i;
     if (p.dcm_count) {
-        const int mm = m2v >> 1;
-        const bool big = (tier == TLC_TIER_MEDHI || tier == TLC_TIER_MEDWIDE) && mm - n + 1 >= TLC_DC_MIN_POS_SHARED && mm <= 8 * 256;
-        const unsigned long long mk = __ballot(big);
+        const unsigned long long mk = __ballot(dcm != 0);
         if (lane == 0 && mk) atomicAdd(p.dcm_count, __popcll(mk));
     }
     if (p.tiny_bin_count) {
-        int bin = -1;
-        if (tier == TLC_TIER_TINY) {
-            const int c = (n + (m2v >> 1)) / TLC_TINY_BIN_W;
-            bin = TLC_TINY_BINS - 1 - (c < TLC_TINY_BINS - 1 ? c : TLC_TINY_BINS - 1);
-        }
+        const int bin = tbin;
         int brank = 0;
 #pragma unroll
         for (int b = 0; b < TLC_TINY_BINS; ++b) {
diff --git a/tlc-gnn_amd/engine.py b/tlc-gnn_amd/engine.py
--- a/tlc-gnn_amd/engine.py
+++ b/tlc-gnn_amd/engine.py
@@ -81,13 +81,29 @@
 
     CHUNK_COUNTERS = ("front_list_last_call", "front_list", "pipelined_chunks", "early_chunks", "beyond_spec_slots", "poisoned_chunks",
                       "poison_bytes", "poison_arena_bytes", "poison_early_bytes", "poison_small_bytes", "deferred_second_halves",
-                      "max_busy_workspaces")
+                      "max_busy_workspaces", "scan_launches", "self_bin_chunks", "self_bin_fallbacks")
 
     def chunk_counters(self):
         out = (C.c_longlong * len(self.CHUNK_COUNTERS))()
         _lib.check(_lib.lib().tlc_debug_chunk_counters(self._h, C.cast(out, C.c_void_p), C.c_int32(len(out)), _lib.stream_ptr(self.device)),
                    "tlc_debug_chunk_counters")
         return dict(zip(self.CHUNK_COUNTERS, (int(v) for v in out)))
+
+    TIER_NAMES = ("small", "medium", "large", "huge", "mid", "tiny", "medium_many_pos", "medium_wide")
+
+    def tier_lists(self, cap):
+        import numpy as np
+        nl = len(self.TIER_NAMES) + 8
+        lists = np.zeros((nl, max(int(cap), 1)), dtype=np.int32)
+        counts = (C.c_longlong * (nl + 2))()
+        _lib.check(_lib.lib().tlc_debug_tier_lists(self._h, C.c_void_p(lists.ctypes.data), C.c_int64(lists.shape[1]), C.cast(counts, C.c_void_p),
+                                                   _lib.stream_ptr(self.device)), "tlc_debug_tier_lists")
+        names = list(self.TIER_NAMES) + ["tiny_bin_%d" % b for b in range(8)]
+        out = {}
+        for k, name in enumerate(names):
+            assert counts[k] <= lists.shape[1], "cap is smaller than the list"
+            out[name] = np.sort(lists[k, :int(counts[k])])
+        return out, {"early": int(counts[nl]), "dcm": int(counts[nl + 1])}
 
     def front_list_count(self):
         return self.chunk_counters()["front_list_last_call"]
```
